# hugolatendresse/FlexFlow

Measured on AMD Instinct MI355X. Metric: decoded tokens/s (LLaMA-7B SpecInfer, LLaMA-68M SSM), higher is better.
Workload: dtype f16; 1 GPU; llama7b_specinfer_llama68m_b8_p128_d128; model=LLaMA-7B (random init), ssm=LLaMA-68M (random init), global_batch=8, prefill=128, decode=128, seq_len=256, parallelism=tp1, layers=32

## Files before the change

### flexflow_amd/csrc/api.cpp

```cpp
#include <rccl/rccl.h>
#include <stdio.h>
#include <stdlib.h>
#include <string.h>

#include <chrono>
#include <cmath>
#include <condition_variable>
#include <memory>
#include <mutex>
#include <string>
#include <vector>

#include <algorithm>
#include <climits>

#include "ffmi_internal.h"
#include "collective.h"

static thread_local std::string g_last_error;

void ffmi_set_last_error(const char *msg, const char *file, int line) {
  char buf[512];
  snprintf(buf, sizeof(buf), "%s (%s:%d)", msg, file, line);
  g_last_error = buf;
// ... 221 lines not shown
}

extern "C" ffmi_status ffmi_attn_create(const ffmi_attn_cfg *cfg, ffmi_attn **out) {
  FFMI_CHECK(cfg && out, FFMI_ERR_INVALID);
  FFMI_CHECK(cfg->head_dim == 64 || cfg->head_dim == 128 ||
                 (cfg->head_dim == 32 && cfg->mode == FFMI_ATTN_INC),
             FFMI_ERR_UNSUPPORTED);
  FFMI_CHECK(cfg->num_heads > 0 && cfg->max_requests > 0 && cfg->max_seq_len > 0 &&
                 cfg->max_tokens > 0,
             FFMI_ERR_INVALID);
  FFMI_CHECK(cfg->out_layout == 0 || cfg->out_layout == 1, FFMI_ERR_INVALID);
  FFMI_CHECK(cfg->out_layout == 0 || (cfg->num_heads * cfg->head_dim) % 32 == 0,
             FFMI_ERR_UNSUPPORTED);
  ffmi_attn *h = new ffmi_attn();
  h->cfg = *cfg;
  h->slots = (cfg->max_seq_len + cfg->max_tree_tokens + 31) & ~31;
  const size_t Hl = (size_t)cfg->num_heads * cfg->head_dim;
  const size_t kv = (size_t)cfg->max_requests * cfg->num_heads * h->slots * cfg->head_dim;
  const bool f32 = cfg->full_precision != 0;
  if (f32 && (cfg->out_layout != 0 || (size_t)(cfg->head_dim + 256 + h->slots) * 4 > 64 * 1024)) {
    delete h;
    ffmi_set_last_error("full precision: out_layout 0 and (head_dim + 256 + slots) * 4 <= 64 KiB",
                        __FILE__, __LINE__);
    return FFMI_ERR_UNSUPPORTED;
  }
  const size_t es = f32 ? 4 : 2, stage_halves = f32 ? 1 : 2;
  bool ok = hipMalloc((void **)&h->kc, kv * es) == hipSuccess &&
            hipMalloc((void **)&h->vc, kv * es) == hipSuccess &&
            hipMalloc((void **)&h->qbuf, (size_t)cfg->max_tokens * Hl * es) == hipSuccess;
  if (ok && cfg->mode == FFMI_ATTN_TREE)
    ok = hipMalloc((void **)&h->stage, (size_t)cfg->max_tokens * 2 * Hl * es * stage_halves) ==
         hipSuccess;
  std::vector<float> tab;
  rope_table(tab, h->slots, cfg->head_dim, cfg);
  if (ok) ok = hipMalloc((void **)&h->rope, tab.size() * sizeof(float)) == hipSuccess;
  if (!ok) {
    ffmi_attn_destroy(h);
    ffmi_set_last_error("attention cache alloc", __FILE__, __LINE__);
    return FFMI_ERR_OOM;
  }
  FFMI_HIP(hipMemset(h->kc, 0, kv * es));
  FFMI_HIP(hipMemset(h->vc, 0, kv * es));
  if (h->stage)
    FFMI_HIP(hipMemset(h->stage, 0, (size_t)cfg->max_tokens * 2 * Hl * es * stage_halves));
  FFMI_HIP(hipMemcpy(h->rope, tab.data(), tab.size() * sizeof(float), hipMemcpyHostToDevice));
  *out = h;
  return FFMI_OK;
}

namespace ffmi {
ffmi_status attn_rope_fault(ffmi_attn *h, int from_pos) {
  FFMI_CHECK(h, FFMI_ERR_INVALID);
  std::vector<float> tab;
  rope_table(tab, h->slots + 1, h->cfg.head_dim, &h->cfg);
  const size_t row = (size_t)h->cfg.head_dim;
  if (from_pos >= 0)
    for (int p = from_pos; p < h->slots; ++p)
      memcpy(&tab[(size_t)p * row], &tab[(size_t)(p + 1) * row], row * sizeof(float));
  FFMI_HIP(hipMemcpy(h->rope, tab.data(), (size_t)h->slots * row * sizeof(float),
                     hipMemcpyHostToDevice));
  return FFMI_OK;
}
}

extern "C" void ffmi_attn_destroy(ffmi_attn *h) {
  if (!h) return;
  (void)hipFree(h->kc);
  (void)hipFree(h->vc);
  (void)hipFree(h->qbuf);
  (void)hipFree(h->stage);
  (void)hipFree(h->rope);
  delete h;
}

extern "C" ffmi_status ffmi_attn_kv_ptrs(ffmi_attn *h, void **k, void **v, int *slots) {
  FFMI_CHECK(h, FFMI_ERR_INVALID);
  if (k) *k = h->kc;
  if (v) *v = h->vc;
  if (slots) *slots = h->slots;
  return FFMI_OK;
}

namespace ffmi {
ffmi_status attn_forward(ffmi_attn *h, const ffmi_batch_dev *b, const void *qkv, Partials qkvp,
                         void *out, ffmi_stream stream, int parity, OprojArgs *opa) {
  FFMI_CHECK(h && b && (qkv || qkvp.S > 0) && out, FFMI_ERR_INVALID);
  if (opa) opa->done = false;
  FFMI_CHECK(b->num_tokens <= h->cfg.max_tokens, FFMI_ERR_INVALID);
  const bool tree = h->cfg.mode == FFMI_ATTN_TREE;
  const hipStream_t s = (hipStream_t)stream;
  const int heads = h->cfg.num_heads, d = h->cfg.head_dim;
  if (h->cfg.full_precision) {
    FFMI_CHECK(qkv && qkvp.S == 0 && !(opa && opa->wo), FFMI_ERR_INVALID);
    FFMI_HIP(ffmi::launch_kv_update_f32(b->dev, b->num_tokens, tree ? b->num_commits : 0,
                                        (const float *)qkv, h->rope, h->slots, (float *)h->qbuf,
                                        (float *)h->kc, (float *)h->vc,
                                        tree ? (float *)h->stage : nullptr, heads, d, h->slots, s));
    FFMI_HIP(ffmi::launch_attention_f32(b->dev, b->num_tokens, (const float *)h->qbuf,
                                        (const float *)h->kc, (const float *)h->vc, (float *)out,
                                        heads, d, h->slots, h->cfg.qk_scale, s));
    return FFMI_OK;
  }
  uint16_t *stage_wr = nullptr, *stage_rd = nullptr;
  int C = 0;
  if (tree) {
    if (parity < 0) parity = h->parity, h->parity ^= 1;
    const size_t half = (size_t)h->cfg.max_tokens * 2 * heads * d;
    stage_wr = h->stage + (parity ? half : 0);
    stage_rd = h->stage + (parity ? 0 : half);
    C = b->num_commits;
  }
  const bool no_fuse = getenv("FFMI_ATTN_NO_FUSE") != nullptr;
  const bool fused = b->one_item_per_req && b->lds_tail && !no_fuse;
  if (C > 0 && b->commit_overlap) {
    FFMI_HIP(ffmi::launch_commit(b->dev, C, stage_rd, h->kc, h->vc, heads, d, h->slots, s));
    C = 0;
  }
  if (!fused) {
    FFMI_HIP(ffmi::launch_kv_update(b->dev, b->num_tokens, b->num_work, C,
                                    (const uint16_t *)qkv, qkvp, h->qbuf, h->kc, h->vc, stage_wr,
                                    stage_rd, h->rope, heads, d, h->slots, h->slots, s));
    C = 0;
  }
  const bool oproj = opa && opa->wo && opa->slab && fused && d == 64 && b->max_q <= 16 &&
                     opa->N % 16 == 0 && opa->N <= 1024 && b->num_tokens <= opa->max_T;
  FFMI_HIP(ffmi::launch_attention(b->dev, b->num_work, b->max_q, h->qbuf, h->kc, h->vc,
                                  (uint16_t *)out, heads, d, h->slots, h->cfg.qk_scale, s,
                                  h->cfg.out_layout == 1, fused, b->num_tokens, C,
                                  (const uint16_t *)qkv, qkvp, stage_wr, stage_rd, h->rope,
                                  h->slots, oproj ? opa : nullptr));
  if (oproj) opa->done = true;
  return FFMI_OK;
}
}

static ffmi_status attn_run(ffmi_attn *h, const ffmi_batch_dev *b, const void *qkv, void *out,
                            ffmi_stream stream, int mode) {
  FFMI_CHECK(h && qkv, FFMI_ERR_INVALID);
  FFMI_CHECK(h->cfg.mode == mode, FFMI_ERR_INVALID);
  return ffmi::attn_forward(h, b, qkv, ffmi::Partials(), out, stream);
}

extern "C" ffmi_status ffmi_attn_inc(ffmi_attn *h, const ffmi_batch_dev *b, const void *qkv,
                                     void *out, ffmi_stream stream) {
  return attn_run(h, b, qkv, out, stream, FFMI_ATTN_INC);
}
extern "C" ffmi_status ffmi_attn_spec(ffmi_attn *h, const ffmi_batch_dev *b, const void *qkv,
                                      void *out, ffmi_stream stream) {
  return attn_run(h, b, qkv, out, stream, FFMI_ATTN_SPEC);
}
extern "C" ffmi_status ffmi_attn_tree(ffmi_attn *h, const ffmi_batch_dev *b, const void *qkv,
                                      void *out, ffmi_stream stream) {
  FFMI_CHECK(h && h->stage, FFMI_ERR_INVALID);
  return attn_run(h, b, qkv, out, stream, FFMI_ATTN_TREE);
}

extern "C" size_t ffmi_linear_packed_bytes(int out_dim, int in_dim) {
  const size_t nt = (size_t)(out_dim + 15) / 16, kt = (size_t)(in_dim + 31) / 32;
  return nt * kt * 512 * 2;
}

extern "C" ffmi_status ffmi_linear_pack_weight(const void *W, int out_dim, int in_dim,
                                               void *W_packed, ffmi_stream stream) {
  FFMI_CHECK(W && W_packed && out_dim > 0 && in_dim > 0, FFMI_ERR_INVALID);
  FFMI_HIP(ffmi::launch_pack_weight((const uint16_t *)W, in_dim, 0, 0, out_dim, in_dim,
                                    (uint16_t *)W_packed, 1, 0, (out_dim + 15) / 16,
                                    (hipStream_t)stream));
  return FFMI_OK;
}

extern "C" ffmi_status ffmi_linear_pack_gate_up(const void *Wg, const void *Wu, int out_dim,
                                                int in_dim, void *W_packed, ffmi_stream stream) {
  FFMI_CHECK(Wg && Wu && W_packed && out_dim > 0 && in_dim > 0, FFMI_ERR_INVALID);
  const int pitch = 2 * ((out_dim + 15) / 16);
  FFMI_HIP(ffmi::launch_pack_weight((const uint16_t *)Wg, in_dim, 0, 0, out_dim, in_dim,
                                    (uint16_t *)W_packed, 2, 0, pitch, (hipStream_t)stream));
  FFMI_HIP(ffmi::launch_pack_weight((const uint16_t *)Wu, in_dim, 0, 0, out_dim, in_dim,
                                    (uint16_t *)W_packed, 2, 1, pitch, (hipStream_t)stream));
  return FFMI_OK;
}

extern "C" size_t ffmi_linear_workspace_bytes(int T, int out_dim, int in_dim, int epilogue) {
  if (T <= 0 || out_dim <= 0 || in_dim <= 0) return 0;
  return ffmi::gemm_workspace_bytes(T, out_dim, in_dim, epilogue);
}

extern "C" ffmi_status ffmi_linear_ws(const void *X, const void *W_packed, void *Y, int T,
                                      int out_dim, int in_dim, int epilogue, void *workspace,
                                      size_t workspace_bytes, ffmi_stream stream) {
  FFMI_CHECK(X && W_packed && Y && T >= 0 && out_dim > 0, FFMI_ERR_INVALID);
  FFMI_CHECK(in_dim > 0 && in_dim % 32 == 0, FFMI_ERR_UNSUPPORTED);
  const int epi = epilogue & ~(FFMI_X_PACKED | FFMI_W_STREAM);
  const int epi_base = epi & ~FFMI_Y_PACKED;
  FFMI_CHECK(epi_base == FFMI_EPI_NONE || epi_base == FFMI_EPI_SILU_MUL, FFMI_ERR_INVALID);
  FFMI_CHECK(!(epilogue & FFMI_Y_PACKED) || out_dim % 32 == 0, FFMI_ERR_UNSUPPORTED);
  FFMI_HIP(ffmi::launch_gemm((const uint16_t *)X, (const uint16_t *)W_packed, (uint16_t *)Y,
                             (float *)workspace, workspace_bytes, T, out_dim, in_dim, epilogue,
                             (hipStream_t)stream));
  return FFMI_OK;
}

static std::mutex g_ws_mu;
static void *g_ws = nullptr;
static size_t g_ws_bytes = 0;

extern "C" ffmi_status ffmi_linear(const void *X, const void *W_packed, void *Y, int T,
                                   int out_dim, int in_dim, int epilogue, ffmi_stream stream) {
  FFMI_CHECK(X && W_packed && Y && T >= 0 && out_dim > 0, FFMI_ERR_INVALID);
  FFMI_CHECK(in_dim > 0 && in_dim % 32 == 0, FFMI_ERR_UNSUPPORTED);
  const size_t need = ffmi_linear_workspace_bytes(T, out_dim, in_dim, epilogue);
  void *ws = nullptr;
  {
    std::lock_guard<std::mutex> lk(g_ws_mu);
    if (need > g_ws_bytes) {
      if (g_ws) {
        FFMI_HIP(hipDeviceSynchronize());
        (void)hipFree(g_ws);
        g_ws = nullptr;
        g_ws_bytes = 0;
      }
      if (hipMalloc(&g_ws, need) != hipSuccess) return FFMI_ERR_OOM;
      g_ws_bytes = need;
    }
    ws = g_ws;
  }
  return ffmi_linear_ws(X, W_packed, Y, T, out_dim, in_dim, epilogue, ws, g_ws_bytes, stream);
}

extern "C" ffmi_status ffmi_rmsnorm(const void *x, const void *w, void *out, int T, int H,
                                    float eps, ffmi_stream stream) {
  FFMI_CHECK(x && w && out && H % 8 == 0 && H <= 16384, FFMI_ERR_INVALID);
  FFMI_HIP(ffmi::launch_rmsnorm((const uint16_t *)x, nullptr, (const uint16_t *)w, nullptr,
                                (uint16_t *)out, T, H, eps, (hipStream_t)stream));
  return FFMI_OK;
}

extern "C" ffmi_status ffmi_residual_rmsnorm(const void *x1, const void *x2, const void *w,
                                             void *residual_out, void *out, int T, int H,
                                             float eps, ffmi_stream stream) {
  FFMI_CHECK(x1 && x2 && w && residual_out && out && H % 8 == 0 && H <= 16384, FFMI_ERR_INVALID);
  FFMI_HIP(ffmi::launch_rmsnorm((const uint16_t *)x1, (const uint16_t *)x2, (const uint16_t *)w,
                                (uint16_t *)residual_out, (uint16_t *)out, T, H, eps,
                                (hipStream_t)stream));
  return FFMI_OK;
}

extern "C" ffmi_status ffmi_rmsnorm_ex(const void *x1, const void *x2, const void *w,
                                       void *residual_out, void *out, int T, int H, float eps,
                                       int flags, ffmi_stream stream) {
  FFMI_CHECK(x1 && w && out && T >= 0 && H > 0 && H % 8 == 0, FFMI_ERR_INVALID);
  FFMI_CHECK(!x2 || residual_out, FFMI_ERR_INVALID);
  FFMI_CHECK((flags & ~FFMI_Y_PACKED) == 0, FFMI_ERR_INVALID);
  const bool packed = (flags & FFMI_Y_PACKED) != 0;
  FFMI_CHECK(!packed || H % 32 == 0, FFMI_ERR_UNSUPPORTED);
  FFMI_HIP(ffmi::launch_rmsnorm((const uint16_t *)x1, (const uint16_t *)x2, (const uint16_t *)w,
                                (uint16_t *)residual_out, (uint16_t *)out, T, H, eps,
                                (hipStream_t)stream, packed));
  return FFMI_OK;
}

extern "C" ffmi_status ffmi_embedding(const ffmi_batch_dev *b, const void *table, void *out,
                                      int H, ffmi_stream stream) {
  FFMI_CHECK(b && table && out && H % 8 == 0, FFMI_ERR_INVALID);
  FFMI_HIP(ffmi::launch_embedding(b->dev, b->num_tokens, (const uint16_t *)table,
                                  (uint16_t *)out, H, (hipStream_t)stream));
  return FFMI_OK;
}

extern "C" ffmi_status ffmi_silu_mul(const void *a, const void *b, void *out, size_t n,
                                     ffmi_stream stream) {
  FFMI_CHECK(a && b && out, FFMI_ERR_INVALID);
  FFMI_HIP(ffmi::launch_silu_mul((const uint16_t *)a, (const uint16_t *)b, (uint16_t *)out, n,
                                 (hipStream_t)stream));
  return FFMI_OK;
}

extern "C" ffmi_status ffmi_argmax(const void *logits, int T, int V, int32_t *ids, float *probs,
                                   ffmi_stream stream) {
  FFMI_CHECK(logits && ids && V > 0, FFMI_ERR_INVALID);
  FFMI_HIP(ffmi::launch_argmax((const uint16_t *)logits, T, V, 1, ids, probs,
                               (hipStream_t)stream));
  return FFMI_OK;
}

extern "C" ffmi_status ffmi_arg_topk(const void *logits, int T, int V, int k, int32_t *ids,
                                     float *probs, ffmi_stream stream) {
  FFMI_CHECK(logits && ids && V > 0 && k >= 1 && k <= 4 && k <= V, FFMI_ERR_INVALID);
  FFMI_HIP(ffmi::launch_argmax((const uint16_t *)logits, T, V, k, ids, probs,
                               (hipStream_t)stream));
  return FFMI_OK;
}

extern "C" size_t ffmi_arg_topk_workspace_bytes(int T) { return ffmi::argmax_workspace_bytes(T); }

extern "C" ffmi_status ffmi_arg_topk_ws(const void *logits, int T, int V, int k, int32_t *ids,
                                        float *probs, void *workspace, size_t workspace_bytes,
                                        ffmi_stream stream) {
  FFMI_CHECK(logits && ids && V > 0 && k >= 1 && k <= 4 && k <= V, FFMI_ERR_INVALID);
  FFMI_HIP(ffmi::launch_argmax((const uint16_t *)logits, T, V, k, ids, probs,
                               (hipStream_t)stream, workspace, workspace_bytes));
  return FFMI_OK;
}

extern "C" ffmi_status ffmi_debug_fused_residual_linear(const void *X, const void *W_packed,
                                                        void *residual, float *ss_out, int T,
                                                        int out_dim, int in_dim,
                                                        ffmi_stream stream) {
  FFMI_CHECK(X && W_packed && residual && ss_out && T > 0 && T <= 32, FFMI_ERR_INVALID);
  ffmi::FuseArgs fz;
  fz.kind = 1;
  fz.res_in = (const uint16_t *)residual;
  fz.ss_out = ss_out;
  FFMI_HIP(ffmi::launch_gemm((const uint16_t *)X, (const uint16_t *)W_packed, (uint16_t *)residual,
                             nullptr, 0, T, out_dim, in_dim, FFMI_EPI_NONE, (hipStream_t)stream,
                             nullptr, 0, &fz));
  return FFMI_OK;
}

extern "C" ffmi_status ffmi_debug_fused_norm_linear(const void *residual, const float *ss_in,
                                                    const void *norm_w, float eps,
                                                    const void *W_packed, void *Y, int T,
                                                    int out_dim, int in_dim, int epilogue,
                                                    ffmi_stream stream) {
  FFMI_CHECK(residual && ss_in && norm_w && W_packed && Y && T > 0 && T <= 32 &&
                 (epilogue == FFMI_EPI_NONE || epilogue == FFMI_EPI_SILU_MUL),
             FFMI_ERR_INVALID);
  ffmi::FuseArgs fz;
  fz.kind = 2;
  fz.ss_in = ss_in;
  fz.nss = in_dim / 16;
  fz.wnorm = (const uint16_t *)norm_w;
  fz.eps = eps;
  FFMI_HIP(ffmi::launch_gemm((const uint16_t *)residual, (const uint16_t *)W_packed, (uint16_t *)Y,
                             nullptr, 0, T, out_dim, in_dim, epilogue, (hipStream_t)stream,
                             nullptr, 0, &fz));
  return FFMI_OK;
}

extern "C" ffmi_status ffmi_fill_weight(void *dst_f16, size_t n, const char *name, uint64_t seed,
                                        int kind, ffmi_stream stream) {
  FFMI_CHECK(dst_f16 && name, FFMI_ERR_INVALID);
  FFMI_HIP(ffmi::launch_fill_weight((uint16_t *)dst_f16, n, ffmi::weight_key(name, seed), kind,
                                    (hipStream_t)stream));
  return FFMI_OK;
}

struct LocalGroup {
  int n = 0;
  ffmi_status sum_status = FFMI_OK;
  std::mutex mu;
  std::condition_variable cv;
  int arrived = 0;
  long gen = 0;
  bool broken = false;
  std::vector<const void *> bufs;
  void *tmp = nullptr;
  size_t tmp_bytes = 0;
  ~LocalGroup() {
    if (tmp) (void)hipFree(tmp);
  }
  bool barrier() {
    std::unique_lock<std::mutex> lk(mu);
    if (broken) return false;
    const long g = gen;
    if (++arrived == n) {
      arrived = 0;
      ++gen;
      cv.notify_all();
      return true;
    }
    if (!cv.wait_for(lk, std::chrono::seconds(120), [&] { return gen != g || broken; }) || broken) {
      broken = true;
      cv.notify_all();
      return false;
    }
    return true;
  }
};

struct PeerState {
  size_t cap = 0;
  char *own = nullptr;
  char *base[ffmi::kMaxPeers] = {};
  std::vector<void *> opened;
  int *err_h = nullptr, *err_d = nullptr;
  bool attached = false;
  uint64_t timeout_ticks = 1000000000ull;
  size_t two_shot_min = 256 << 10;
  ~PeerState() {
    for (void *p : opened) (void)hipIpcCloseMemHandle(p);
    if (own) (void)hipFree(own);
    if (err_h) (void)hipHostFree(err_h);
  }
};

struct ffmi_comm {
  ncclComm_t comm = nullptr;
  int nranks = 1, rank = 0;
  std::shared_ptr<LocalGroup> local;
  std::unique_ptr<PeerState> peer;
  float *xg = nullptr;
  size_t xg_cap = 0;
  hipStream_t xg_stream = nullptr;
};

extern "C" ffmi_status ffmi_comm_create_local(int nranks, ffmi_comm **out) {
  FFMI_CHECK(out && nranks >= 1 && nranks <= 8, FFMI_ERR_INVALID);
  auto g = std::make_shared<LocalGroup>();
  g->n = nranks;
  g->bufs.assign(nranks, nullptr);
  for (int r = 0; r < nranks; ++r) {
    out[r] = new ffmi_comm();
    out[r]->nranks = nranks;
    out[r]->rank = r;
    out[r]->local = g;
  }
  return FFMI_OK;
}

static ffmi_status local_allreduce(ffmi_comm *c, const void *in, void *out, size_t count,
                                   int dtype, hipStream_t s) {
  LocalGroup &g = *c->local;
  const size_t bytes = count * (dtype == FFMI_F16 ? 2 : 4);
  g.bufs[c->rank] = in;
  FFMI_HIP(hipStreamSynchronize(s));
  FFMI_CHECK(g.barrier(), FFMI_ERR_NCCL);
  ffmi_status st = FFMI_OK;
  if (c->rank == 0) {
    if (g.tmp_bytes < bytes) {
      if (g.tmp) (void)hipFree(g.tmp);
      g.tmp = nullptr;
      g.tmp_bytes = 0;
      if (hipMalloc(&g.tmp, bytes) == hipSuccess) g.tmp_bytes = bytes;
    }
    if (!g.tmp) {
      st = FFMI_ERR_OOM;
    } else if (ffmi::launch_group_sum(g.bufs.data(), g.n, g.tmp, count, dtype, s) != hipSuccess ||
               hipStreamSynchronize(s) != hipSuccess) {
      st = FFMI_ERR_HIP;
    }
  }
  if (c->rank == 0) g.sum_status = st;
  if (!g.barrier() || g.sum_status != FFMI_OK) {
    std::lock_guard<std::mutex> lk(g.mu);
    g.broken = true;
    g.cv.notify_all();
    return g.sum_status != FFMI_OK ? g.sum_status : FFMI_ERR_NCCL;
  }
  FFMI_HIP(hipMemcpyAsync(out, g.tmp, bytes, hipMemcpyDeviceToDevice, s));
  FFMI_HIP(hipStreamSynchronize(s));
  FFMI_CHECK(g.barrier(), FFMI_ERR_NCCL);
  return FFMI_OK;
}

extern "C" ffmi_status ffmi_comm_unique_id(void *id_out) {
  FFMI_CHECK(id_out, FFMI_ERR_INVALID);
  static_assert(sizeof(ncclUniqueId) == FFMI_UNIQUE_ID_BYTES, "unique id size");
  ncclUniqueId id;
  if (ncclGetUniqueId(&id) != ncclSuccess) return FFMI_ERR_NCCL;
  memcpy(id_out, &id, sizeof(id));
  return FFMI_OK;
}

extern "C" ffmi_status ffmi_comm_create(const void *id, int nranks, int rank, ffmi_comm **out) {
  FFMI_CHECK(id && out && nranks >= 1 && rank >= 0 && rank < nranks, FFMI_ERR_INVALID);
  ffmi_comm *c = new ffmi_comm();
  c->nranks = nranks;
  c->rank = rank;
  ncclUniqueId uid;
  memcpy(&uid, id, sizeof(uid));
  ncclResult_t r = ncclCommInitRank(&c->comm, nranks, uid, rank);
  if (r != ncclSuccess) {
    ffmi_set_last_error(ncclGetErrorString(r), __FILE__, __LINE__);
    delete c;
    return FFMI_ERR_NCCL;
  }
  *out = c;
  return FFMI_OK;
}

extern "C" void ffmi_comm_destroy(ffmi_comm *c) {
  if (!c) return;
  if (c->xg_stream) (void)hipStreamSynchronize(c->xg_stream);
  if (c->xg) (void)hipFree(c->xg);
  if (c->xg_stream) (void)hipStreamDestroy(c->xg_stream);
  if (c->comm) ncclCommDestroy(c->comm);
  delete c;
}

extern "C" ffmi_status ffmi_comm_allgather(ffmi_comm *c, const void *mine, size_t bytes,
                                           void *all) {
  FFMI_CHECK(c && (mine || !bytes) && (all || !bytes), FFMI_ERR_INVALID);
  const int n = c->nranks;
  if (n == 1) {
    if (bytes) memcpy(all, mine, bytes);
    return FFMI_OK;
  }
  const size_t words = (bytes + 1) / 2;
  const size_t count = words * n;
  if (c->xg_cap < count) {
    if (c->xg) FFMI_HIP(hipFree(c->xg));
    c->xg = nullptr;
    c->xg_cap = 0;
    FFMI_HIP(hipMalloc((void **)&c->xg, count * sizeof(float)));
    c->xg_cap = count;
  }
  if (!c->xg_stream) FFMI_HIP(hipStreamCreateWithFlags(&c->xg_stream, hipStreamNonBlocking));
  std::vector<float> h(count, 0.0f);
  std::vector<uint16_t> w(words, 0);
  memcpy(w.data(), mine, bytes);
  for (size_t i = 0; i < words; ++i) h[(size_t)c->rank * words + i] = (float)w[i];
  FFMI_HIP(hipMemcpyAsync(c->xg, h.data(), count * sizeof(float), hipMemcpyHostToDevice,
                          c->xg_stream));
  ffmi_status st = ffmi_allreduce(c, c->xg, c->xg, count, FFMI_F32, (ffmi_stream)c->xg_stream);
  if (st != FFMI_OK) return st;
  FFMI_HIP(hipMemcpyAsync(h.data(), c->xg, count * sizeof(float), hipMemcpyDeviceToHost,
                          c->xg_stream));
  FFMI_HIP(hipStreamSynchronize(c->xg_stream));
  if (c->peer && c->peer->attached) {
    st = ffmi_comm_peer_status(c);
    if (st != FFMI_OK) return st;
  }
  std::vector<uint16_t> out(words);
  for (int r = 0; r < n; ++r) {
    for (size_t i = 0; i < words; ++i) {
      const float v = h[(size_t)r * words + i];
      if (!(v >= 0.0f && v <= 65535.0f && v == (float)(uint16_t)v)) return FFMI_ERR_NCCL;
      out[i] = (uint16_t)v;
    }
    memcpy(static_cast<char *>(all) + (size_t)r * bytes, out.data(), bytes);
  }
  return FFMI_OK;
}

extern "C" ffmi_status ffmi_comm_create_peer(int nranks, int rank, ffmi_comm **out) {
  FFMI_CHECK(out && nranks >= 1 && nranks <= ffmi::kMaxPeers && rank >= 0 && rank < nranks,
             FFMI_ERR_INVALID);
  ffmi_comm *c = new ffmi_comm();
  c->nranks = nranks;
  c->rank = rank;
  *out = c;
  return FFMI_OK;
}

extern "C" ffmi_status ffmi_comm_peer_export(ffmi_comm *c, size_t max_bytes, void *handle_out) {
  FFMI_CHECK(c && handle_out && max_bytes > 0 && !c->local, FFMI_ERR_INVALID);
  FFMI_CHECK(c->nranks <= ffmi::kMaxPeers && !c->peer, FFMI_ERR_INVALID);
  static_assert(sizeof(hipIpcMemHandle_t) == FFMI_PEER_HANDLE_BYTES, "IPC handle size");
  auto p = std::make_unique<PeerState>();
  p->cap = (max_bytes + 255) & ~(size_t)255;
  if (const char *e = getenv("FFMI_PEER_TIMEOUT_S")) p->timeout_ticks = (uint64_t)(atof(e) * 1e8);
  if (c->nranks <= 2) p->two_shot_min = (size_t)-1;
  if (const char *e = getenv("FFMI_PEER_TWO_SHOT_MIN")) p->two_shot_min = (size_t)atoll(e);
  const size_t bytes = ffmi::peer_buffer_bytes(p->cap);
  const char *uc = getenv("FFMI_PEER_UNCACHED");
  if (uc && !atoi(uc)) FFMI_HIP(hipMalloc((void **)&p->own, bytes));
  else FFMI_HIP(hipExtMallocWithFlags((void **)&p->own, bytes, hipDeviceMallocUncached));
  FFMI_HIP(hipMemset(p->own, 0, ffmi::kDataOff));
  FFMI_HIP(hipDeviceSynchronize());
  FFMI_HIP(hipHostMalloc((void **)&p->err_h, sizeof(int), hipHostMallocMapped));
  *p->err_h = 0;
  FFMI_HIP(hipHostGetDevicePointer((void **)&p->err_d, p->err_h, 0));
  hipIpcMemHandle_t h;
  FFMI_HIP(hipIpcGetMemHandle(&h, p->own));
  memcpy(handle_out, &h, sizeof(h));
  c->peer = std::move(p);
  return FFMI_OK;
}

static ffmi_status peer_run(ffmi_comm *c, const void *in, void *out, size_t rows, size_t cols,
                            size_t ld, size_t col0, int dtype, hipStream_t s,
                            const ffmi::Partials *slabs = nullptr, int rs_row0 = -1,
                            int rs_row1 = -1, const ffmi::PeerNormArgs *norm = nullptr,
                            int two_shot = -1) {
  PeerState &p = *c->peer;
  const size_t esz = dtype == FFMI_F16 ? 2 : 4;
  const size_t bytes = rows * cols * esz;
  FFMI_CHECK(bytes <= p.cap, FFMI_ERR_INVALID);
  FFMI_CHECK((cols * esz) % 16 == 0 && ((size_t)in & 15) == 0 && ((size_t)out & 15) == 0 &&
                 (ld * esz) % 16 == 0 && (col0 * esz) % 16 == 0,
             FFMI_ERR_UNSUPPORTED);
  if (slabs && slabs->S > 0)
    FFMI_CHECK(dtype == FFMI_F16 && slabs->S <= 8 && slabs->NP >= (int)cols && slabs->NP % 4 == 0 &&
                   ((size_t)slabs->p & 15) == 0,
               FFMI_ERR_UNSUPPORTED);
  ffmi::PeerArgs a;
  for (int r = 0; r < ffmi::kMaxPeers; ++r) a.base[r] = p.base[r];
  a.nranks = c->nranks;
  a.rank = c->rank;
  a.cap = p.cap;
  a.in = in;
  a.out = out;
  a.nvec = bytes / 16;
  a.vec_elems = 16 / esz;
  a.cols = cols;
  a.ld = ld;
  a.col0 = col0;
  a.esz = esz;
  a.err = p.err_d;
  a.timeout_ticks = p.timeout_ticks;
  if (slabs && slabs->S > 0) a.slabs = slabs->p, a.S = slabs->S, a.NP = slabs->NP, a.rows = rows;
  const bool ts = two_shot >= 0 ? two_shot != 0 : bytes >= p.two_shot_min;
  if (norm) FFMI_HIP(ffmi::launch_peer_allreduce_norm(a, *norm, ts, s));
  else FFMI_HIP(ffmi::launch_peer_allreduce(a, ts, s, rs_row0, rs_row1));
  return FFMI_OK;
}
// ... 233 lines not shown
```

### flexflow_amd/csrc/ffmi_internal.h

```cpp
#pragma once
#include <hip/hip_runtime.h>
#include <hip/hip_fp16.h>
#include <stdint.h>

#include "../../include/ffmi.h"
#include "kernels/gemm_plan.h"

#define FFMI_HIP(expr)                                   \
  do {                                                   \
    hipError_t e_ = (expr);                              \
    if (e_ != hipSuccess) {                              \
      ffmi_set_last_error(hipGetErrorString(e_), __FILE__, __LINE__); \
      (void)hipGetLastError();  \
      return FFMI_ERR_HIP;                               \
    }                                                    \
  } while (0)

#define FFMI_CHECK(cond, code)                                         \
  do {                                                                 \
    if (!(cond)) {                                                     \
      ffmi_set_last_error(#cond, __FILE__, __LINE__);                  \
      return (code);                                                   \
    }                                                                  \
  } while (0)

void ffmi_set_last_error(const char *msg, const char *file, int line);

namespace ffmi {

typedef _Float16 h8 __attribute__((ext_vector_type(8)));
typedef _Float16 h4 __attribute__((ext_vector_type(4)));
typedef float f4 __attribute__((ext_vector_type(4)));

template <bool NT>
__device__ __forceinline__ h8 ld_weight(const uint16_t *p) {
  if constexpr (NT) return __builtin_nontemporal_load(reinterpret_cast<const h8 *>(p));
  else return *reinterpret_cast<const h8 *>(p);
}

__host__ __device__ __forceinline__ size_t act_packed_off(int m, int n, int K) {
  return ((((size_t)(m >> 4) * (size_t)(K >> 5) + (size_t)(n >> 5)) * 64 + (m & 15) +
           16 * ((n >> 3) & 3))
          << 3) +
         (n & 7);
}

struct BatchHeader {
  int32_t num_tokens, num_work, num_commits, num_mask_reqs;
  int32_t off_tokens, off_work, off_commits, off_masks;
};
constexpr int kBlobWorkOffset = 32;
static_assert(sizeof(BatchHeader) == kBlobWorkOffset, "work array follows the header");

constexpr int kTailSlots = 128;
constexpr int kItemCommits = 8;

struct WorkDev {
  ffmi_attn_work w;
  int32_t clean;
  int32_t tail0;
  int32_t ncommit;
  int32_t told;
  int16_t rope_pos[FFMI_ATTN_QTILE];
  int16_t cm_src[kItemCommits], cm_depth[kItemCommits];
};
static_assert(sizeof(WorkDev) % 16 == 0, "16-B aligned work items");

struct BatchView {
  const BatchHeader *hdr;
  const ffmi_token_info *tokens;
  const WorkDev *work;
  const ffmi_commit_info *commits;
  const uint64_t *masks;
};

__device__ __forceinline__ BatchView batch_view(const char *blob) {
  BatchView v;
  v.hdr = reinterpret_cast<const BatchHeader *>(blob);
  v.work = reinterpret_cast<const WorkDev *>(blob + kBlobWorkOffset);
  v.tokens = reinterpret_cast<const ffmi_token_info *>(blob + v.hdr->off_tokens);
  v.commits = reinterpret_cast<const ffmi_commit_info *>(blob + v.hdr->off_commits);
  v.masks = reinterpret_cast<const uint64_t *>(blob + v.hdr->off_masks);
  return v;
}

struct Partials {
  const float *p = nullptr;
  int S = 0, NP = 0;
};
__device__ __forceinline__ float partials_value(const float *p, int S, int NP, int T, int t,
                                                int n) {
  const size_t slab = (size_t)T * NP;
  const float *q = p + (size_t)t * NP + n;
  float acc = q[0];
  for (int s = 1; s < S; ++s) acc += q[s * slab];
  return __half2float(__float2half_rn(acc));
}

__host__ __device__ __forceinline__ void mid_xcd_map(int bx, int by, int nblk, int S, int &cb,
                                                     int &ks) {
  cb = bx, ks = by;
  if (S <= 1) return;
  const int l = bx + nblk * by, P = nblk * S;
  const int x = l & 7, q = P >> 3, r = P & 7;
  const int L = (x < r ? x * (q + 1) : r * (q + 1) + (x - r) * q) + (l >> 3);
  ks = L / nblk, cb = L - ks * nblk;
}

hipError_t launch_fill_weight(uint16_t *dst, size_t n, uint64_t key, int kind, hipStream_t s,
                              int cols = 0, uint64_t pa = 1, uint64_t pb = 0, float scale = 1.0f);
hipError_t launch_fill_weight_f32(float *dst, size_t n, uint64_t key, int kind, hipStream_t s,
                                  int cols = 0, uint64_t pa = 1, uint64_t pb = 0,
                                  float scale = 1.0f);
float weight_amp(int kind);
hipError_t launch_gemm_f32(const float *X, const float *W, float *Y, int T, int N, int K,
                           hipStream_t s);
hipError_t launch_rmsnorm_f32(const float *x1, const float *x2, const float *w, float *res_out,
                              float *out, int T, int H, float eps, hipStream_t s,
                              const char *gather = nullptr);
hipError_t launch_silu_mul_f32(const float *A, const float *B, float *out, int T, int F,
                               size_t lda, size_t ldb, hipStream_t s);
hipError_t launch_kv_update_f32(const char *blob, int T, int C, const float *qkv, const float *rope,
                                int max_rope_pos, float *qbuf, float *kc, float *vc,
                                float *stage, int heads, int d, int slots, hipStream_t s);
hipError_t launch_attention_f32(const char *blob, int T, const float *qbuf, const float *kc,
                                const float *vc, float *out, int heads, int d, int slots,
                                float scale, hipStream_t s);
hipError_t launch_softmax_topk_f32(const float *logits, int T, int V, int k, int32_t *ids,
                                   float *probs, hipStream_t s);
ffmi_status attn_rope_fault(ffmi_attn *h, int from_pos);
bool weights_kmajor();
inline size_t w_tile_stride(int KT) { return weights_kmajor() ? 512 : (size_t)KT * 512; }
inline size_t w_k_stride(int pitch) { return weights_kmajor() ? (size_t)pitch * 512 : 512; }
hipError_t launch_pack_weight(const uint16_t *src, int ld, int row0, int col0,
                              int N, int K, uint16_t *dst, int tile_step,
                              int tile_offset, int pitch, hipStream_t s);
struct FuseArgs {
  int kind = 0;
  const uint16_t *res_in = nullptr;
  float *ss_out = nullptr;
  const float *ss_in = nullptr;
  int nss = 0;
  const uint16_t *wnorm = nullptr;
  float eps = 0.f;
};
hipError_t launch_gemm(const uint16_t *X, const uint16_t *Wp, uint16_t *Y, float *ws,
                       size_t ws_bytes, int T, int N, int K, int epilogue, hipStream_t s,
                       Partials *defer = nullptr, int wpitch = 0, const FuseArgs *fuse = nullptr);
hipError_t launch_partials_reduce(const Partials &p, uint16_t *Y, int T, int N, hipStream_t s);
long attn_debug_stamps(long long *dst, long max_waves);
hipError_t launch_marker(int i, hipStream_t s);
void attn_stamp_gate(bool open);
long debug_markers(long long *dst, long n);
long gemm_debug_stamps(long long *dst, long max_waves);
size_t packed_act_bytes(int T, int K);
hipError_t launch_pack_act(const uint16_t *X, uint16_t *Xp, int T, int K, hipStream_t s);
hipError_t launch_rmsnorm(const uint16_t *x1, const uint16_t *x2, const uint16_t *w,
                          uint16_t *res_out, uint16_t *out, int T, int H, float eps,
                          hipStream_t s, bool out_packed = false, Partials x2p = {}, const char *gather = nullptr,
                          char *blob_dst = nullptr, size_t blob_bytes = 0,
                          const int32_t *gather_prev = nullptr);
void set_norm_fault(bool on);
hipError_t launch_embedding(const char *blob, int T, const uint16_t *table,
                            uint16_t *out, int H, hipStream_t s);
hipError_t launch_silu_mul(const uint16_t *a, const uint16_t *b, uint16_t *out,
                           size_t n, hipStream_t s);
hipError_t launch_argmax(const uint16_t *logits, int T, int V, int k, int32_t *ids,
                         float *probs, hipStream_t s, void *ws = nullptr, size_t ws_bytes = 0,
                         int32_t *ids2 = nullptr);
size_t argmax_workspace_bytes(int T);
hipError_t launch_vshard(const uint16_t *logits, int T, int Vl, int P, int rank, int k,
                         int phase, float *xch, int W, int32_t *ids, float *probs,
                         hipStream_t s);
hipError_t launch_group_sum(const void *const *bufs, int n, void *out, size_t count, int dtype,
                            hipStream_t s);

hipError_t launch_kv_update(const char *blob, int T, int W, int C, const uint16_t *qkv,
                            Partials qkvp, uint16_t *qbuf, uint16_t *kc, uint16_t *vc,
                            uint16_t *stage_wr, const uint16_t *stage_rd, const float *rope,
                            int heads, int d, int slots, int max_rope_pos, hipStream_t s);
hipError_t launch_commit(const char *blob, int C, const uint16_t *stage,
                         uint16_t *kc, uint16_t *vc, int heads, int d, int slots,
                         hipStream_t s);
struct OprojArgs {
  const uint16_t *wo = nullptr;
  float *slab = nullptr;
  int N = 0, max_T = 0;
  size_t wts = 0, wks = 0;
  bool done = false;
};
hipError_t launch_attention(const char *blob, int W, int max_q, uint16_t *qbuf, uint16_t *kc,
                            uint16_t *vc, uint16_t *out, int heads, int d, int slots, float scale,
                            hipStream_t s, bool out_packed, bool fused, int T, int C,
                            const uint16_t *qkv, Partials qkvp, uint16_t *stage_wr,
                            const uint16_t *stage_rd, const float *rope, int max_rope_pos,
                            const OprojArgs *opa = nullptr);

uint64_t weight_key(const char *name, uint64_t seed);

}

struct ffmi_batch_dev {
  char *host = nullptr;
  char *dev = nullptr;
  size_t cap = 0;
  int max_tokens = 0, max_requests = 0;
  int num_tokens = 0, num_work = 0, num_commits = 0, num_mask_reqs = 0;
  bool commit_overlap = false;
  bool one_item_per_req = false;
  bool lds_tail = false;
  int max_q = 0;
  hipEvent_t uploaded = nullptr;
};

namespace ffmi {
ffmi_status batch_stage(ffmi_batch_dev *b, const ffmi_batch_desc *d, size_t *bytes);
ffmi_status batch_copy(ffmi_batch_dev *b, size_t bytes, hipStream_t s, bool record_event);
bool comm_has_peer(const ffmi_comm *c, size_t bytes);
int comm_size(const ffmi_comm *c);
int comm_rank(const ffmi_comm *c);
bool comm_peer_attached(const ffmi_comm *c);
bool comm_has_fallback(const ffmi_comm *c);
bool comm_is_rccl(const ffmi_comm *c);
ffmi_status comm_allreduce_cols(ffmi_comm *c, const void *in, void *out, int rows, int cols,
                                int ld, int col0, int dtype, hipStream_t s,
                                const Partials *slabs = nullptr);
bool comm_two_shot(const ffmi_comm *c, size_t bytes);
ffmi_status comm_reduce_rows(ffmi_comm *c, const void *in, void *out, int rows, int cols, int ld,
                             int col0, int row0, int row1, hipStream_t s,
                             const Partials *slabs = nullptr);
ffmi_status comm_allreduce_norm(ffmi_comm *c, const void *in, int T, int H, int col0,
                                const uint16_t *prev, uint16_t *res, const uint16_t *w, float eps,
                                uint16_t *h, bool packed, bool two_shot, hipStream_t s,
                                const Partials *slabs = nullptr);
ffmi_status comm_status(ffmi_comm *c);
ffmi_status attn_forward(ffmi_attn *h, const ffmi_batch_dev *b, const void *qkv, Partials qkvp,
                         void *out, ffmi_stream stream, int parity = -1,
                         OprojArgs *opa = nullptr);
}
```

### flexflow_amd/csrc/kernels/norm.hip

```cpp
#include <algorithm>

#include "../ffmi_internal.h"
#include "expf_ref.h"

namespace ffmi {

__device__ __forceinline__ float h2f_(uint16_t v) { return __half2float(__ushort_as_half(v)); }
__device__ __forceinline__ uint16_t f2h_(float v) { return __half_as_ushort(__float2half_rn(v)); }

template <int NW, typename T>
__device__ __forceinline__ T block_sum(T v, T *scratch) {
#pragma unroll
  for (int o = 32; o > 0; o >>= 1) v += __shfl_xor(v, o);
  const int wave = threadIdx.x >> 6;
  if ((threadIdx.x & 63) == 0) scratch[wave] = v;
  __syncthreads();
  T r = scratch[0];
#pragma unroll
  for (int q = 1; q < NW; ++q) r += scratch[q];
  return r;
}

template <int NT, int MAXC, int MAXS, int SRC>
__global__ __launch_bounds__(NT) void rmsnorm_kernel(
    const uint16_t *__restrict__ x1, const uint16_t *__restrict__ x2,
    const uint16_t *__restrict__ w, uint16_t *__restrict__ res_out,
    uint16_t *__restrict__ out, int H, float eps, int out_packed,
    const float *__restrict__ x2p, int pS, int pNP, const char *__restrict__ gather,
    uint4 *__restrict__ blob_dst, int blob_n16, const int32_t *__restrict__ gprev) {
  __shared__ double scratch[NT / 64];
  const int row = blockIdx.x;
  const int T = gridDim.x;
  const int nchunk = H >> 3;
  constexpr bool FAULT = SRC >= 4;
  constexpr int S = FAULT ? SRC - 3 : SRC;
  int gid = 0;
  if (S == 3) {
    gid = batch_view(gather).tokens[row].token_id;
    if (gid < 0) gid = gprev[-1 - gid];
  }
  const uint16_t *a = S == 3 ? x1 + (size_t)gid * H : x1 + (size_t)row * H;
  if (S == 3 && blob_dst) {
    const uint4 *src = reinterpret_cast<const uint4 *>(gather);
    for (int i = row * NT + threadIdx.x; i < blob_n16; i += T * NT) blob_dst[i] = src[i];
  }
  uint4 v[MAXC], wv[MAXC];
  uint4 xb[MAXC];
  f4 slo[MAXS], shi[MAXS];
  auto fold = [&]() {
    f4 lo = slo[0], hi = shi[0];
#pragma unroll
    for (int sl = 1; sl < MAXS; ++sl)
      if (sl < pS) lo += slo[sl], hi += shi[sl];
    uint16_t hb[8];
#pragma unroll
    for (int q4 = 0; q4 < 4; ++q4) {
      hb[q4] = f2h_(lo[q4]);
      hb[q4 + 4] = f2h_(hi[q4]);
    }
    return *reinterpret_cast<uint4 *>(hb);
  };
#pragma unroll
  for (int c = 0; c < MAXC; ++c) {
    const int ch = min((int)threadIdx.x + c * NT, nchunk - 1);
    if (S == 2) {
      const float *q = x2p + (size_t)row * pNP + ch * 8;
#pragma unroll
      for (int sl = 0; sl < MAXS; ++sl) {
        const float *qs = q + (size_t)min(sl, pS - 1) * T * pNP;
        slo[sl] = *reinterpret_cast<const f4 *>(qs);
        shi[sl] = *reinterpret_cast<const f4 *>(qs + 4);
      }
    }
    if (S == 1) xb[c] = *reinterpret_cast<const uint4 *>(x2 + (size_t)row * H + ch * 8);
    v[c] = *reinterpret_cast<const uint4 *>(a + ch * 8);
    wv[c] = *reinterpret_cast<const uint4 *>(w + ch * 8);
    if (S == 2 && MAXC > 1) xb[c] = fold();
  }
  if (S == 2 && MAXC == 1) xb[0] = fold();
  double ss = 0.0;
#pragma unroll
  for (int c = 0; c < MAXC; ++c) {
    const int ch = threadIdx.x + c * NT;
    if (ch < nchunk) {
      uint4 xa = v[c];
      if (S == 1 || S == 2) {
        const uint4 xbb = xb[c];
        const __half2 *pa = reinterpret_cast<const __half2 *>(&xa);
        const __half2 *pb = reinterpret_cast<const __half2 *>(&xbb);
        if (FAULT) {
          const uint16_t *ea = reinterpret_cast<const uint16_t *>(&xa);
          const uint16_t *eb = reinterpret_cast<const uint16_t *>(&xbb);
#pragma unroll
          for (int q = 0; q < 8; ++q) {
            const float f = h2f_(ea[q]) + h2f_(eb[q]);
            ss += (double)f * (double)f;
          }
        }
        __half2 r[4];
#pragma unroll
        for (int q = 0; q < 4; ++q) r[q] = __hadd2(pa[q], pb[q]);
        xa = *reinterpret_cast<uint4 *>(r);
        *reinterpret_cast<uint4 *>(res_out + (size_t)row * H + ch * 8) = xa;
      } else if (S == 3) {
        *reinterpret_cast<uint4 *>(res_out + (size_t)row * H + ch * 8) = xa;
      }
      v[c] = xa;
      const uint16_t *e = reinterpret_cast<const uint16_t *>(&xa);
      if (!FAULT) {
#pragma unroll
        for (int q = 0; q < 8; ++q) {
          const float f = h2f_(e[q]);
          ss += (double)f * (double)f;
        }
      }
    }
  }
  const float sum = (float)block_sum<NT / 64>(ss, scratch);
  const float rms_f = __fdiv_rn(1.0f, sqrtf(__fadd_rn(__fdiv_rn(sum, (float)H), eps)));
  const float rms = h2f_(f2h_(rms_f));
#pragma unroll
  for (int c = 0; c < MAXC; ++c) {
    const int ch = threadIdx.x + c * NT;
    if (ch < nchunk) {
      const uint16_t *e = reinterpret_cast<const uint16_t *>(&v[c]);
      const uint16_t *we = reinterpret_cast<const uint16_t *>(&wv[c]);
      uint16_t o8[8];
#pragma unroll
      for (int q = 0; q < 8; ++q) {
        float y = h2f_(f2h_(__fmul_rn(h2f_(e[q]), rms)));
        o8[q] = f2h_(__fmul_rn(y, h2f_(we[q])));
      }
      uint16_t *dst = out_packed ? out + act_packed_off(row, ch * 8, H) : out + (size_t)row * H + ch * 8;
      *reinterpret_cast<uint4 *>(dst) = *reinterpret_cast<uint4 *>(o8);
    }
  }
}

static bool g_norm_fault = false;
void set_norm_fault(bool on) { g_norm_fault = on; }

hipError_t launch_rmsnorm(const uint16_t *x1, const uint16_t *x2, const uint16_t *w,
                          uint16_t *res_out, uint16_t *out, int T, int H, float eps,
                          hipStream_t s, bool out_packed, Partials x2p, const char *gather,
                          char *blob_dst, size_t blob_bytes, const int32_t *gather_prev) {
  if (gather && (x2 || x2p.S > 0 || !res_out)) return hipErrorInvalidValue;
  if (blob_dst && (!gather || blob_bytes > (size_t)1 << 30 || (uintptr_t)gather % 16 ||
                   (uintptr_t)blob_dst % 16))
    return hipErrorInvalidValue;
  const int blob_n16 = blob_dst ? (int)((blob_bytes + 15) / 16) : 0;
  if (T <= 0) return hipSuccess;
  if (out_packed && H % 32) return hipErrorInvalidValue;
  const int op = out_packed ? 1 : 0;
  const int nchunk = H / 8;
  if (nchunk > 4096) return hipErrorInvalidValue;
  const float *pp = x2p.S > 0 ? x2p.p : nullptr;
  if (pp && (x2p.S > 16 || (x2p.S > 8 && nchunk > 128))) return hipErrorInvalidValue;
  if ((x2 || pp) && !res_out) return hipErrorInvalidValue;
  if (pp && nchunk > 1024) return hipErrorInvalidValue;
  const int src = gather ? 3 : pp ? 2 : x2 ? 1 : 0;
  const int ms = !pp || x2p.S <= 1 ? 1 : x2p.S <= 2 ? 2 : x2p.S <= 4 ? 4 : x2p.S <= 8 ? 8
               : x2p.S <= 12 ? 12 : 16;
#define FFMI_RMS3(NT, MC, MS, SR)                                                              \
  hipLaunchKernelGGL((rmsnorm_kernel<NT, MC, MS, SR>), dim3(T), dim3(NT), 0, s, x1, x2, w,    \
                     res_out, out, H, eps, op, pp, x2p.S, x2p.NP, gather,               \
                     reinterpret_cast<uint4 *>(blob_dst), blob_n16, gather_prev)
#define FFMI_RMS(NT, MC)                                   \
  do {                                                     \
    if (src == 0) FFMI_RMS3(NT, MC, 1, 0);                 \
    else if (src == 1) FFMI_RMS3(NT, MC, 1, 1);            \
    else if (src == 3) FFMI_RMS3(NT, MC, 1, 3);            \
    else if (ms == 1) FFMI_RMS3(NT, MC, 1, 2);             \
    else if (ms == 2) FFMI_RMS3(NT, MC, 2, 2);             \
    else if (ms == 4) FFMI_RMS3(NT, MC, 4, 2);             \
    else FFMI_RMS3(NT, MC, 8, 2);                          \
  } while (0)
#define FFMI_RMS_NOSLAB(NT, MC)                            \
  do {                                                     \
    if (src == 0) FFMI_RMS3(NT, MC, 1, 0);                 \
    else if (src == 1) FFMI_RMS3(NT, MC, 1, 1);            \
    else FFMI_RMS3(NT, MC, 1, 3);                          \
  } while (0)
  if (g_norm_fault && (src == 1 || src == 2)) {
#define FFMI_RMSF(NT)                                      \
  do {                                                     \
    if (src == 1) FFMI_RMS3(NT, 1, 1, 4);                  \
    else if (ms == 1) FFMI_RMS3(NT, 1, 1, 5);              \
    else if (ms == 2) FFMI_RMS3(NT, 1, 2, 5);              \
    else if (ms == 4) FFMI_RMS3(NT, 1, 4, 5);              \
    else if (ms == 8) FFMI_RMS3(NT, 1, 8, 5);              \
    else return hipErrorInvalidValue;                      \
  } while (0)
    if (nchunk <= 128) FFMI_RMSF(128);
    else if (nchunk <= 256) FFMI_RMSF(256);
    else if (nchunk <= 512) FFMI_RMSF(512);
    else if (nchunk <= 1024) FFMI_RMSF(1024);
    else return hipErrorInvalidValue;
#undef FFMI_RMSF
    return hipGetLastError();
  }
  if (nchunk <= 128 && ms == 12) FFMI_RMS3(128, 1, 12, 2);
  else if (nchunk <= 128 && ms == 16) FFMI_RMS3(128, 1, 16, 2);
  else if (nchunk <= 128) FFMI_RMS(128, 1);
  else if (nchunk <= 256) FFMI_RMS(256, 1);
  else if (nchunk <= 512) FFMI_RMS(512, 1);
  else if (nchunk <= 1024) FFMI_RMS(1024, 1);
  else if (nchunk <= 2048) FFMI_RMS_NOSLAB(1024, 2);
  else FFMI_RMS_NOSLAB(1024, 4);
#undef FFMI_RMS_NOSLAB
#undef FFMI_RMS
#undef FFMI_RMS3
  return hipGetLastError();
}

__global__ void embedding_kernel(const char *__restrict__ blob,
                                 const uint16_t *__restrict__ table,
                                 uint16_t *__restrict__ out, int H) {
  const BatchView bv = batch_view(blob);
  const int t = blockIdx.x;
  const int tok = bv.tokens[t].token_id;
  const uint4 *src = reinterpret_cast<const uint4 *>(table + (size_t)tok * H);
  uint4 *dst = reinterpret_cast<uint4 *>(out + (size_t)t * H);
  for (int c = threadIdx.x; c < H / 8; c += blockDim.x) dst[c] = src[c];
}

hipError_t launch_embedding(const char *blob, int T, const uint16_t *table, uint16_t *out,
                            int H, hipStream_t s) {
  if (T <= 0) return hipSuccess;
  if (H % 8 != 0) return hipErrorInvalidValue;
  hipLaunchKernelGGL(embedding_kernel, dim3(T), dim3(256), 0, s, blob, table, out, H);
  return hipGetLastError();
}

__global__ void silu_mul_kernel(const uint16_t *__restrict__ a, const uint16_t *__restrict__ b,
                                uint16_t *__restrict__ out, size_t n) {
  for (size_t i = blockIdx.x * (size_t)blockDim.x + threadIdx.x; i < n;
       i += (size_t)gridDim.x * blockDim.x) {
    const float g = h2f_(a[i]);
    const float sg = __fdiv_rn(1.0f, __fadd_rn(1.0f, expf(-g)));
    const float t = h2f_(f2h_(__fmul_rn(g, h2f_(f2h_(sg)))));
    out[i] = f2h_(__fmul_rn(t, h2f_(b[i])));
  }
}

hipError_t launch_silu_mul(const uint16_t *a, const uint16_t *b, uint16_t *out, size_t n,
                           hipStream_t s) {
  if (n == 0) return hipSuccess;
  size_t blocks = (n + 255) / 256;
  if (blocks > 16384) blocks = 16384;
  hipLaunchKernelGGL(silu_mul_kernel, dim3((unsigned)blocks), dim3(256), 0, s, a, b, out, n);
  return hipGetLastError();
}

extern "C" __device__ float __ockl_wfred_max_f32(float);
extern "C" __device__ double __ockl_wfred_add_f64(double);
extern "C" __device__ unsigned long long __ockl_wfred_max_u64(unsigned long long);

template <int TPB, int NV, int G>
__global__ __launch_bounds__(TPB) void softmax_topk_reg_kernel(
    const uint16_t *__restrict__ logits, int V, int k, int32_t *__restrict__ ids,
    float *__restrict__ probs, double *__restrict__ part, unsigned *__restrict__ cnt,
    int32_t *__restrict__ ids2) {
  constexpr int NW = TPB / 64;
  constexpr int kCand = 128;
  static_assert(G == 1 || ((NV * 8) % G == 0 && NV * 8 / G >= 2),
                "split: whole dwords of a thread's elements per workgroup");
  constexpr int E = NV * 8 / G;
  __shared__ double sh[NW + 2];
  __shared__ unsigned long long cand[kCand];
  __shared__ unsigned ncand;
  __shared__ int last_arrival;
  float *fsh = reinterpret_cast<float *>(sh);
  unsigned long long *ksh = reinterpret_cast<unsigned long long *>(sh);
  const int row = G == 1 ? blockIdx.x : blockIdx.y, chunk = G == 1 ? 0 : blockIdx.x;
  const int tid = threadIdx.x, lane = tid & 63, wv = tid >> 6;
  const int nvec = V >> 3;
  const uint4 *x = reinterpret_cast<const uint4 *>(logits + (size_t)row * V);
  constexpr int EPV = E < 8 ? 8 / E : 1;
  const int vrot = G == 1 ? 0 : (E >= 8 ? chunk * (E / 8) : chunk / EPV);
  const int eo = E >= 8 ? 0 : (chunk % EPV) * E;
  auto gv = [&](int v) -> int { return (G == 1 ? v : (v + vrot) % NV) * TPB + tid; };
  uint4 r[NV];
#pragma unroll
  for (int v = 0; v < NV; ++v) {
    const int i = gv(v);
    r[v] = i < nvec ? x[i] : make_uint4(0xfc00fc00u, 0xfc00fc00u, 0xfc00fc00u, 0xfc00fc00u);
  }
  if (tid == 0) ncand = 0;
  auto elem = [&](int v, int e) -> float {
    const uint32_t w = (&r[v].x)[e >> 1];
    return h2f_((uint16_t)((e & 1) ? (w >> 16) : (w & 0xffffu)));
  };
  float mx = -INFINITY;
#pragma unroll
  for (int v = 0; v < NV; ++v)
#pragma unroll
    for (int e = 0; e < 8; ++e) mx = fmaxf(mx, elem(v, e));
  mx = __ockl_wfred_max_f32(mx);
  if (lane == 0) fsh[wv] = mx;
  __syncthreads();
  float wmax[NW];
#pragma unroll
  for (int q = 0; q < NW; ++q) wmax[q] = fsh[q];
  __syncthreads();
  float M = wmax[0];
#pragma unroll
  for (int q = 1; q < NW; ++q) M = fmaxf(M, wmax[q]);
  float L = -INFINITY;
  {
    float top[4] = {-INFINITY, -INFINITY, -INFINITY, -INFINITY};
#pragma unroll
    for (int q = 0; q < NW; ++q) {
      float v = wmax[q];
#pragma unroll
      for (int j = 0; j < 4; ++j) {
        const float hi = fmaxf(top[j], v), lo = fminf(top[j], v);
        top[j] = hi, v = lo;
      }
    }
#pragma unroll
    for (int j = 0; j < 4; ++j)
      if (j == k - 1) L = top[j];
  }
  double se = 0.0;
  if constexpr (E >= 8) {
#pragma unroll
    for (int v = 0; v < E / 8; ++v)
      if (gv(v) < nvec)
#pragma unroll
        for (int e = 0; e < 8; ++e) se += (double)expf_ref(elem(v, e) - M);
  } else {
    const int d0 = eo >> 1;
    auto dw = [&](int d) -> uint32_t {
      const uint32_t lo = (d & 1) ? r[0].y : r[0].x, hi = (d & 1) ? r[0].w : r[0].z;
      return (d & 2) ? hi : lo;
    };
    if (gv(0) < nvec)
#pragma unroll
      for (int q = 0; q < E / 2; ++q) {
        const uint32_t w = dw(d0 + q);
        se += (double)expf_ref(h2f_((uint16_t)(w & 0xffffu)) - M);
        se += (double)expf_ref(h2f_((uint16_t)(w >> 16)) - M);
      }
  }
  se = __ockl_wfred_add_f64(se);
  if (lane == 0) sh[wv] = se;
  __syncthreads();
  double sd = 0.0;
#pragma unroll
  for (int q = 0; q < NW; ++q) sd += sh[q];
  if constexpr (G > 1) {
    if (wv == 0) {
      unsigned before = 0;
      if (lane == 0) {
        __hip_atomic_store(&part[(size_t)row * G + chunk], sd, __ATOMIC_RELAXED,
                           __HIP_MEMORY_SCOPE_AGENT);
        asm volatile("s_waitcnt vmcnt(0)" ::: "memory");
        before = __hip_atomic_fetch_add(&cnt[row], 1u, __ATOMIC_RELAXED, __HIP_MEMORY_SCOPE_AGENT);
      }
      const int last = __shfl(before, 0) == (unsigned)(G - 1);
      if (last) {
        double pq = 0.0;
        if (lane < G)
          pq = __hip_atomic_load(&part[(size_t)row * G + lane], __ATOMIC_RELAXED,
                                 __HIP_MEMORY_SCOPE_AGENT);
        double tot = 0.0;
#pragma unroll
        for (int q = 0; q < G; ++q) tot += __shfl(pq, q);
        if (lane == 0) {
          __hip_atomic_store(&cnt[row], 0u, __ATOMIC_RELAXED, __HIP_MEMORY_SCOPE_AGENT);
          sh[NW] = tot;
        }
      }
      if (lane == 0) last_arrival = last;
    }
    __syncthreads();
    if (!last_arrival) return;
    sd = sh[NW];
  }
  const float S = (float)sd;
  float thr = -3.402823466e38f;
  {
    const uint16_t pL = f2h_(__fdiv_rn(expf_ref(L - M), S));
    if (pL > 1) {
      const float lo = 0.5f * (h2f_(pL) + h2f_((uint16_t)(pL - 1)));
      thr = M + logf(lo * S) - 0.0009765625f * fmaxf(1.0f, fabsf(M));
    }
  }
  auto key_of = [&](float xv, unsigned i) -> unsigned long long {
    const uint16_t p = f2h_(__fdiv_rn(expf_ref(xv - M), S));
    return ((unsigned long long)(p + 1u) << 32) | (unsigned long long)(0xffffffffu - i);
  };
  auto emit = [&](int rd, unsigned long long b) {
    ids[(size_t)row * k + rd] = (int)(0xffffffffu - (unsigned)(b & 0xffffffffu));
    if (ids2) ids2[(size_t)row * k + rd] = (int)(0xffffffffu - (unsigned)(b & 0xffffffffu));
    if (probs) probs[(size_t)row * k + rd] = h2f_((uint16_t)((b >> 32) - 1u));
  };
#pragma unroll
  for (int v = 0; v < NV; ++v)
#pragma unroll
    for (int e = 0; e < 8; ++e) {
      const float xv = elem(v, e);
      const unsigned i = (unsigned)(gv(v) * 8 + e);
      if (xv >= thr && (int)i < V) {
        const unsigned slot = atomicAdd(&ncand, 1u);
        if (slot < (unsigned)kCand) cand[slot] = key_of(xv, i);
      }
    }
  __syncthreads();
  const unsigned n = ncand;
  if (n <= (unsigned)kCand) {
    if (wv == 0) {
      unsigned long long a = (unsigned)lane < n ? cand[lane] : 0ull;
      unsigned long long b = (unsigned)(lane + 64) < n ? cand[lane + 64] : 0ull;
      for (int rd = 0; rd < k; ++rd) {
        const unsigned long long best = __ockl_wfred_max_u64(a > b ? a : b);
        if (lane == 0) emit(rd, best);
        if (a == best) a = 0ull;
        if (b == best) b = 0ull;
      }
    }
    return;
  }
  for (int rd = 0; rd < k; ++rd) {
    unsigned long long best = 0;
#pragma unroll
    for (int v = 0; v < NV; ++v)
#pragma unroll
      for (int e = 0; e < 8; ++e) {
        const float xv = elem(v, e);
        const unsigned i = (unsigned)(gv(v) * 8 + e);
        if (xv >= thr && (int)i < V) {
          const unsigned long long key = key_of(xv, i);
          best = key > best ? key : best;
        }
      }
    best = __ockl_wfred_max_u64(best);
    if (lane == 0) ksh[wv] = best;
    __syncthreads();
    unsigned long long b = ksh[0];
#pragma unroll
    for (int q = 1; q < NW; ++q) b = ksh[q] > b ? ksh[q] : b;
    __syncthreads();
    const unsigned idx = 0xffffffffu - (unsigned)(b & 0xffffffffu);
    if (tid == 0) emit(rd, b);
    if (rd + 1 < k && (idx >> 3) % TPB == (unsigned)tid) {
#pragma unroll
      for (int v = 0; v < NV; ++v)
        if ((unsigned)gv(v) == (idx >> 3)) {
#pragma unroll
          for (int e = 0; e < 8; ++e) {
            uint32_t &w = (&r[v].x)[e >> 1];
            const uint32_t m = (e & 1) ? 0xffff0000u : 0x0000ffffu;
            if ((unsigned)e == (idx & 7)) w = (w & ~m) | (0xfc00fc00u & m);
          }
        }
    }
  }
}

template <int TPB>
__global__ __launch_bounds__(TPB) void softmax_topk_kernel(
    const uint16_t *__restrict__ logits, int V, int k, int32_t *__restrict__ ids,
    float *__restrict__ probs, int32_t *__restrict__ ids2) {
  constexpr int NW = TPB / 64;
  constexpr int kCand = 128;
  __shared__ double sh[NW + 2];
  __shared__ unsigned long long cand[kCand];
  __shared__ unsigned ncand;
  float *fsh = reinterpret_cast<float *>(sh);
  unsigned long long *ksh = reinterpret_cast<unsigned long long *>(sh);
  const int row = blockIdx.x, tid = threadIdx.x, lane = tid & 63, wv = tid >> 6;
  const uint16_t *x = logits + (size_t)row * V;
  if (tid == 0) ncand = 0;
  float mx = -INFINITY;
  for (int i = tid; i < V; i += TPB) mx = fmaxf(mx, h2f_(x[i]));
  mx = __ockl_wfred_max_f32(mx);
  if (lane == 0) fsh[wv] = mx;
  __syncthreads();
  float wmax[NW];
#pragma unroll
  for (int q = 0; q < NW; ++q) wmax[q] = fsh[q];
  __syncthreads();
  float M = wmax[0];
#pragma unroll
  for (int q = 1; q < NW; ++q) M = fmaxf(M, wmax[q]);
  float L = -INFINITY;
  {
    float top[4] = {-INFINITY, -INFINITY, -INFINITY, -INFINITY};
#pragma unroll
    for (int q = 0; q < NW; ++q) {
      float v = wmax[q];
#pragma unroll
      for (int j = 0; j < 4; ++j) {
        const float hi = fmaxf(top[j], v), lo = fminf(top[j], v);
        top[j] = hi, v = lo;
      }
    }
#pragma unroll
    for (int j = 0; j < 4; ++j)
      if (j == k - 1) L = top[j];
  }
  double se = 0.0;
  for (int i = tid; i < V; i += TPB) se += (double)expf_ref(h2f_(x[i]) - M);
  se = __ockl_wfred_add_f64(se);
  if (lane == 0) sh[wv] = se;
  __syncthreads();
  double sd = 0.0;
#pragma unroll
  for (int q = 0; q < NW; ++q) sd += sh[q];
  const float S = (float)sd;
  float thr = -3.402823466e38f;
  {
    const uint16_t pL = f2h_(__fdiv_rn(expf_ref(L - M), S));
    if (pL > 1) {
      const float lo = 0.5f * (h2f_(pL) + h2f_((uint16_t)(pL - 1)));
      thr = M + logf(lo * S) - 0.0009765625f * fmaxf(1.0f, fabsf(M));
    }
  }
  auto key_of = [&](float xv, unsigned i) -> unsigned long long {
    const uint16_t p = f2h_(__fdiv_rn(expf_ref(xv - M), S));
    return ((unsigned long long)(p + 1u) << 32) | (unsigned long long)(0xffffffffu - i);
  };
  auto emit = [&](int rd, unsigned long long b) {
    ids[(size_t)row * k + rd] = (int)(0xffffffffu - (unsigned)(b & 0xffffffffu));
    if (ids2) ids2[(size_t)row * k + rd] = (int)(0xffffffffu - (unsigned)(b & 0xffffffffu));
    if (probs) probs[(size_t)row * k + rd] = h2f_((uint16_t)((b >> 32) - 1u));
  };
  for (int i = tid; i < V; i += TPB) {
    const float xv = h2f_(x[i]);
    if (xv >= thr) {
      const unsigned slot = atomicAdd(&ncand, 1u);
      if (slot < (unsigned)kCand) cand[slot] = key_of(xv, (unsigned)i);
    }
  }
  __syncthreads();
  const unsigned n = ncand;
  if (n <= (unsigned)kCand) {
    if (wv == 0) {
      unsigned long long a = (unsigned)lane < n ? cand[lane] : 0ull;
      unsigned long long b = (unsigned)(lane + 64) < n ? cand[lane + 64] : 0ull;
      for (int rd = 0; rd < k; ++rd) {
        const unsigned long long best = __ockl_wfred_max_u64(a > b ? a : b);
        if (lane == 0) emit(rd, best);
        if (a == best) a = 0ull;
        if (b == best) b = 0ull;
      }
    }
    return;
  }
  int chosen[4] = {-1, -1, -1, -1};
  for (int rd = 0; rd < k; ++rd) {
    unsigned long long best = 0;
    for (int i = tid; i < V; i += TPB) {
      const float xv = h2f_(x[i]);
      if (xv < thr) continue;
      bool taken = false;
#pragma unroll
      for (int q = 0; q < 4; ++q) taken |= (q < rd && chosen[q] == i);
      if (taken) continue;
      const unsigned long long key = key_of(xv, (unsigned)i);
      best = key > best ? key : best;
    }
    best = __ockl_wfred_max_u64(best);
    if (lane == 0) ksh[wv] = best;
    __syncthreads();
    unsigned long long b = ksh[0];
#pragma unroll
    for (int q = 1; q < NW; ++q) b = ksh[q] > b ? ksh[q] : b;
    __syncthreads();
    chosen[rd] = (int)(0xffffffffu - (unsigned)(b & 0xffffffffu));
    if (tid == 0) emit(rd, b);
  }
}

constexpr int kSplitRows = 256;
constexpr size_t kSplitPartOff = kSplitRows * 4;
size_t argmax_workspace_bytes(int T) {
  return T <= 0 ? 0 : kSplitPartOff + (size_t)std::min(T, kSplitRows) * 16 * 8;
}

hipError_t launch_argmax(const uint16_t *logits, int T, int V, int k, int32_t *ids,
                         float *probs, hipStream_t s, void *ws, size_t ws_bytes, int32_t *ids2) {
  if (T <= 0) return hipSuccess;
  if (k < 1 || k > 4) return hipErrorInvalidValue;
  static const int split_env = getenv("FFMI_TOPK_SPLIT") ? atoi(getenv("FFMI_TOPK_SPLIT")) : -1;
  static const bool split2 = getenv("FFMI_TOPK_SPLIT2") && atoi(getenv("FFMI_TOPK_SPLIT2"));
  int G = T <= 32 ? 8 : T <= 64 ? 4 : T <= 128 ? 2 : (T <= kSplitRows && split2) ? 2 : 1;
  if (split_env >= 0) G = split_env;
  if (!ws || ws_bytes < argmax_workspace_bytes(T) || T > kSplitRows) G = 1;
  unsigned *cnt = reinterpret_cast<unsigned *>(ws);
  double *part = ws ? reinterpret_cast<double *>(static_cast<char *>(ws) + kSplitPartOff) : nullptr;
  static const int tpb = [] {
    const char *e = getenv("FFMI_TOPK_TPB");
    const int v = e ? atoi(e) : 1024;
    return v == 256 || v == 512 ? v : 1024;
  }();
  const int nv = (V / 8 + tpb - 1) / tpb;
  if (V % 8 == 0 && ((uintptr_t)logits & 15) == 0 && nv * tpb <= 4096) {
#define FFMI_SMR(TPB, NV)                                                                  \
  hipLaunchKernelGGL((softmax_topk_reg_kernel<TPB, NV, 1>), dim3(T), dim3(TPB), 0, s, logits, V, \
                     k, ids, probs, nullptr, nullptr, ids2)
#define FFMI_SMG(NV, GG)                                                                     \
  hipLaunchKernelGGL((softmax_topk_reg_kernel<1024, NV, GG>), dim3(GG, T), dim3(1024), 0, s, \
                     logits, V, k, ids, probs, part, cnt, ids2)
    const int gmax = 4 * std::max(1, nv);
    while (G > 1 && (G > gmax || (G & (G - 1)))) G >>= 1;
    if (tpb == 1024 && G > 1) {
      if (nv <= 1) {
        if (G >= 4) FFMI_SMG(1, 4);
        else FFMI_SMG(1, 2);
      } else if (nv <= 2) {
        if (G >= 8) FFMI_SMG(2, 8);
        else if (G == 4) FFMI_SMG(2, 4);
        else FFMI_SMG(2, 2);
      } else {
        if (G >= 16) FFMI_SMG(4, 16);
        else if (G == 8) FFMI_SMG(4, 8);
        else if (G == 4) FFMI_SMG(4, 4);
        else FFMI_SMG(4, 2);
      }
    } else if (tpb == 256) {
      if (nv <= 4) FFMI_SMR(256, 4);
      else if (nv <= 8) FFMI_SMR(256, 8);
      else FFMI_SMR(256, 16);
    } else if (tpb == 512) {
      if (nv <= 2) FFMI_SMR(512, 2);
      else if (nv <= 4) FFMI_SMR(512, 4);
      else FFMI_SMR(512, 8);
    } else {
      if (nv <= 1) FFMI_SMR(1024, 1);
      else if (nv <= 2) FFMI_SMR(1024, 2);
      else FFMI_SMR(1024, 4);
    }
#undef FFMI_SMR
#undef FFMI_SMG
  } else {
    hipLaunchKernelGGL(softmax_topk_kernel<1024>, dim3(T), dim3(1024), 0, s, logits, V, k, ids, probs,
                       ids2);
  }
  return hipGetLastError();
}

template <int TPB>
__global__ __launch_bounds__(TPB) void vshard_kernel(const uint16_t *__restrict__ logits, int T,
                                                      int Vl, int P, int rank, int k, int phase,
                                                      float *__restrict__ xch, int W,
                                                      int32_t *__restrict__ ids,
                                                      float *__restrict__ probs) {
  constexpr int NW = TPB / 64;
  constexpr int kCand = 128;
  __shared__ double dsh[NW];
  __shared__ float fsh[NW];
  __shared__ unsigned long long ksh[NW];
  __shared__ unsigned long long cand[kCand];
  __shared__ unsigned ncand;
  const int t = blockIdx.x, tid = threadIdx.x, lane = tid & 63, wv = tid >> 6;
  const uint16_t *x = logits + (size_t)t * Vl;
  auto slot = [&](int r) { return xch + ((size_t)r * T + t) * W; };
  if (phase == 3) {
    if (tid == 0) {
      int taken[4] = {-1, -1, -1, -1};
      for (int rd = 0; rd < k; ++rd) {
        unsigned long long best = 0;
        int bq = -1;
        for (int r = 0; r < P; ++r)
          for (int j = 0; j < k; ++j) {
            const float pv = slot(r)[2 * j], iv = slot(r)[2 * j + 1];
            if (iv < 0.f) continue;
            const int q = r * k + j;
            bool used = false;
            for (int z = 0; z < rd; ++z) used |= taken[z] == q;
            if (used) continue;
            const unsigned long long key =
                ((unsigned long long)(f2h_(pv) + 1u) << 32) |
                (unsigned long long)(0xffffffffu - (unsigned)iv);
            if (key > best) best = key, bq = q;
          }
        taken[rd] = bq;
        ids[(size_t)t * k + rd] = (int)(0xffffffffu - (unsigned)(best & 0xffffffffu));
        if (probs) probs[(size_t)t * k + rd] = h2f_((uint16_t)((best >> 32) - 1u));
      }
    }
    return;
  }
  float *own = slot(rank);
  if (phase == 0) {
    float m = -INFINITY;
    for (int i = tid; i < Vl; i += TPB) m = fmaxf(m, h2f_(x[i]));
    m = __ockl_wfred_max_f32(m);
    if (lane == 0) fsh[wv] = m;
    __syncthreads();
#pragma unroll
    for (int q = 0; q < NW; ++q) m = fmaxf(m, fsh[q]);
    if (tid < P * W) {
      const int r = tid / W, w = tid % W;
      slot(r)[w] = (r == rank && w == 0) ? m : 0.f;
    }
    return;
  }
  float M = -INFINITY;
  for (int r = 0; r < P; ++r) M = fmaxf(M, xch[((size_t)r * T + t) * W]);
  if (phase == 1) {
    double se = 0.0;
    for (int i = tid; i < Vl; i += TPB) se += (double)expf_ref(h2f_(x[i]) - M);
    se = __ockl_wfred_add_f64(se);
    if (lane == 0) dsh[wv] = se;
    __syncthreads();
    se = 0.0;
#pragma unroll
    for (int q = 0; q < NW; ++q) se += dsh[q];
    if (tid < P * W) {
      const int r = tid / W, w = tid % W;
      const float hi = (float)se, lo = (float)(se - (double)hi);
      slot(r)[w] = r != rank ? 0.f : (w == 0 ? M : w == 1 ? hi : w == 2 ? lo : 0.f);
    }
    return;
  }
  double sd = 0.0;
  for (int r = 0; r < P; ++r) {
    const float *q = xch + ((size_t)r * T + t) * W;
    sd += (double)q[1] + (double)q[2];
  }
  const float S = (float)sd;
  if (tid == 0) ncand = 0;
  float wm = -INFINITY;
  for (int i = tid; i < Vl; i += TPB) wm = fmaxf(wm, h2f_(x[i]));
  wm = __ockl_wfred_max_f32(wm);
  if (lane == 0) fsh[wv] = wm;
  __syncthreads();
  float L = -INFINITY;
  {
    float top[4] = {-INFINITY, -INFINITY, -INFINITY, -INFINITY};
#pragma unroll
    for (int q = 0; q < NW; ++q) {
      float v = fsh[q];
#pragma unroll
      for (int j = 0; j < 4; ++j) {
        const float hi = fmaxf(top[j], v), lo = fminf(top[j], v);
        top[j] = hi, v = lo;
      }
    }
#pragma unroll
    for (int j = 0; j < 4; ++j)
      if (j == k - 1) L = top[j];
  }
  float thr = -3.402823466e38f;
  {
    const uint16_t pL = f2h_(__fdiv_rn(expf_ref(L - M), S));
    if (pL > 1) {
      const float lo = 0.5f * (h2f_(pL) + h2f_((uint16_t)(pL - 1)));
      thr = M + logf(lo * S) - 0.0009765625f * fmaxf(1.0f, fabsf(M));
    }
  }
  auto key_of = [&](float xv, int i) -> unsigned long long {
    const uint16_t p = f2h_(__fdiv_rn(expf_ref(xv - M), S));
    const unsigned gi = (unsigned)(rank * Vl + i);
    return ((unsigned long long)(p + 1u) << 32) | (unsigned long long)(0xffffffffu - gi);
  };
  auto emit = [&](int rd, unsigned long long b) {
    own[2 * rd] = b ? h2f_((uint16_t)((b >> 32) - 1u)) : 0.f;
    own[2 * rd + 1] = b ? (float)(0xffffffffu - (unsigned)(b & 0xffffffffu)) : -1.f;
  };
  for (int i = tid; i < Vl; i += TPB) {
    const float xv = h2f_(x[i]);
    if (xv >= thr) {
      const unsigned sl = atomicAdd(&ncand, 1u);
      if (sl < (unsigned)kCand) cand[sl] = key_of(xv, i);
    }
  }
  __syncthreads();
  const unsigned n = ncand;
  if (n <= (unsigned)kCand) {
    if (wv == 0) {
      unsigned long long a = (unsigned)lane < n ? cand[lane] : 0ull;
      unsigned long long b = (unsigned)(lane + 64) < n ? cand[lane + 64] : 0ull;
      for (int rd = 0; rd < k; ++rd) {
        const unsigned long long best = __ockl_wfred_max_u64(a > b ? a : b);
        if (lane == 0) emit(rd, best);
        if (best) {
          if (a == best) a = 0ull;
          if (b == best) b = 0ull;
        }
      }
    }
  } else {
    int chosen[4] = {-1, -1, -1, -1};
    for (int rd = 0; rd < k; ++rd) {
      unsigned long long best = 0;
      for (int i = tid; i < Vl; i += TPB) {
        const float xv = h2f_(x[i]);
        if (xv < thr) continue;
        bool used = false;
#pragma unroll
        for (int z = 0; z < 4; ++z) used |= (z < rd && chosen[z] == i);
        if (used) continue;
        const unsigned long long key = key_of(xv, i);
        best = key > best ? key : best;
      }
      best = __ockl_wfred_max_u64(best);
      if (lane == 0) ksh[wv] = best;
      __syncthreads();
      unsigned long long b = ksh[0];
#pragma unroll
      for (int q = 1; q < NW; ++q) b = ksh[q] > b ? ksh[q] : b;
      __syncthreads();
      chosen[rd] = b ? (int)(0xffffffffu - (unsigned)(b & 0xffffffffu)) - rank * Vl : -1;
      if (tid == 0) emit(rd, b);
    }
  }
  if (tid < P * W) {
    const int r = tid / W, w = tid % W;
    if (r != rank) slot(r)[w] = 0.f;
    else if (w >= 2 * k) own[w] = 0.f;
  }
}

hipError_t launch_vshard(const uint16_t *logits, int T, int Vl, int P, int rank, int k,
                         int phase, float *xch, int W, int32_t *ids, float *probs,
                         hipStream_t s) {
  if (T <= 0) return hipSuccess;
  if (k < 1 || k > 4 || P * W > 256 || W < 2 * k || W < 4) return hipErrorInvalidValue;
  hipLaunchKernelGGL((vshard_kernel<1024>), dim3(T), dim3(1024), 0, s, logits, T, Vl, P, rank, k,
                     phase, xch, W, ids, probs);
  return hipGetLastError();
}

struct GroupBufs {
  const void *p[8];
};
__global__ void group_sum_kernel(GroupBufs b, int n, void *__restrict__ out, size_t count,
                                 int dtype) {
  for (size_t i = blockIdx.x * (size_t)blockDim.x + threadIdx.x; i < count;
       i += (size_t)gridDim.x * blockDim.x) {
    if (dtype == FFMI_F16) {
      float a = 0.f;
      for (int r = 0; r < n; ++r) a += h2f_(reinterpret_cast<const uint16_t *>(b.p[r])[i]);
      reinterpret_cast<uint16_t *>(out)[i] = f2h_(a);
    } else if (dtype == FFMI_F32) {
      float a = 0.f;
      for (int r = 0; r < n; ++r) a += reinterpret_cast<const float *>(b.p[r])[i];
      reinterpret_cast<float *>(out)[i] = a;
    } else {
      int a = 0;
      for (int r = 0; r < n; ++r) a += reinterpret_cast<const int *>(b.p[r])[i];
      reinterpret_cast<int *>(out)[i] = a;
    }
  }
}

hipError_t launch_group_sum(const void *const *bufs, int n, void *out, size_t count, int dtype,
                            hipStream_t s) {
  if (n < 1 || n > 8) return hipErrorInvalidValue;
  if (count == 0) return hipSuccess;
  GroupBufs b;
  for (int r = 0; r < 8; ++r) b.p[r] = bufs[r < n ? r : 0];
  size_t blocks = (count + 255) / 256;
  if (blocks > 4096) blocks = 4096;
  hipLaunchKernelGGL(group_sum_kernel, dim3((unsigned)blocks), dim3(256), 0, s, b, n, out, count,
                     dtype);
  return hipGetLastError();
}

}
```

### flexflow_amd/csrc/runtime/llama_gpu.cpp

```cpp
#include <stdio.h>
#include <string.h>

#include <algorithm>
#include <cmath>

#include <string>
#include <map>
#include <tuple>
#include <vector>

#include "model.h"
#include "request_manager.h"

namespace ffmi {

namespace {

struct Layer {
  uint16_t *in_norm = nullptr, *post_norm = nullptr;
  uint16_t *wqkv = nullptr, *wo = nullptr, *wgu = nullptr, *wd = nullptr;
  ffmi_attn *attn = nullptr;
};

struct LlamaGPU : public ffmi_model {
  ffmi_llama_config c{};
  ffmi_model_opts o{};
  int token_capacity() const override { return o.max_tokens; }
  bool uses_collectives() const override { return o.tp_size > 1; }
  std::string weights_folder;
  int Hl = 0, Fl = 0, d = 0, heads_l = 0, slots = 0;
  bool packed = false;
  int wstream = 0;
  hipStream_t stream = nullptr;
  std::vector<Layer> layers;
  uint16_t *embed = nullptr, *final_norm = nullptr, *lm = nullptr;
  uint16_t *res = nullptr, *h = nullptr, *qkv = nullptr, *att = nullptr, *proj = nullptr,
           *mlp = nullptr, *logits = nullptr;
  int32_t *ids_d = nullptr;
  void *topk_ws = nullptr;
  size_t topk_ws_bytes = 0;
  int Vl = 0;
  float *xch = nullptr;
  bool peer = false;
  bool rccl = false;
  bool solo = false;
  int fuse_norms = getenv("FFMI_FUSE_NORM") ? atoi(getenv("FFMI_FUSE_NORM")) : 1;
  float *ss_o = nullptr, *ss_d = nullptr;
  bool fuse_ao = false;
  float *oslab = nullptr;
  int oslab_T = 0;
  int tp_fuse_norm = getenv("FFMI_TP_FUSED_NORM") ? atoi(getenv("FFMI_TP_FUSED_NORM")) : 1;
  int tp_chunks = 1;
  hipStream_t comm_stream = nullptr;
  uint16_t *chunk_buf = nullptr;
  std::vector<hipEvent_t> ev_chunk;
  hipEvent_t ev_comm_done = nullptr;
  float *ws = nullptr;
  size_t ws_bytes = 0;
  size_t ws_chunk = 0;
  bool ar_slabs = !getenv("FFMI_AR_SLABS") || atoi(getenv("FFMI_AR_SLABS")) != 0;
  int32_t *ids_h = nullptr;
  static constexpr int kChain = BeamSearchBatchConfig::MAX_BEAM_DEPTH;
  ffmi_batch_dev *chain_batch[kChain] = {};
  int32_t *ids_dev = nullptr;
  int cur_slot = 0;
  size_t slot_results[kChain] = {};
  std::vector<int> slot_map[kChain];
  hipEvent_t slot_ev[kChain] = {};
  hipEvent_t chain_t0 = nullptr;
  bool slot_ev_live[kChain] = {};
  int last_slot = -1;
  bool chain_ok = !getenv("FFMI_SSM_CHAIN") || atoi(getenv("FFMI_SSM_CHAIN")) != 0;
  size_t slot_ints() const { return (size_t)((o.max_tokens + 15) & ~15) * 4 * 2; }
  bool result_copy = getenv("FFMI_RESULT_COPY") && atoi(getenv("FFMI_RESULT_COPY")) != 0;
  float *probs_h = nullptr;
  ffmi_batch_dev *batch = nullptr;
  PackedStep ps;
  std::vector<void *> allocs;

  enum Cat { GEMM_QKV, GEMM_O, GEMM_GATE_UP, GEMM_DOWN, GEMM_LM_HEAD, ATTENTION, NORM,
             ALLREDUCE, SAMPLING, EMBED, NCAT };
  struct ProfRec {
    int cat;
    hipEvent_t a, b;
    double bytes, flops;
  };
  struct OpStat {
    long launches = 0;
    double ms = 0, bytes = 0, flops = 0;
  };
  int prof_level = 0;
  int prof_every = getenv("FFMI_PROF_EVERY") ? std::max(1, atoi(getenv("FFMI_PROF_EVERY"))) : 4;
  long prof_steps = 0;
  bool prof_this_step = true;
  std::vector<hipEvent_t> ev_pool;
  size_t ev_used = 0;
  std::vector<ProfRec> recs;
  OpStat opstat[NCAT];

  hipEvent_t next_event() {
    if (ev_used == ev_pool.size()) {
      hipEvent_t e;
      (void)hipEventCreate(&e);
      ev_pool.push_back(e);
    }
    return ev_pool[ev_used++];
  }
  bool prof_on(int layer, int T) const {
    if (prof_level == 2) return true;
    if (prof_level == 1)
      return prof_this_step && T <= 256 && (layer == 0 || layer == c.num_layers / 2);
    return false;
  }
  int prof_begin(bool on) {
    if (!on) return -1;
    ProfRec r;
    r.a = next_event();
    r.b = next_event();
    (void)hipEventRecord(r.a, stream);
    recs.push_back(r);
    return (int)recs.size() - 1;
  }
  void prof_end(int idx, int cat, double bytes, double flops) {
    if (idx < 0) return;
    ProfRec &r = recs[idx];
    r.cat = cat;
    r.bytes = bytes;
    r.flops = flops;
    (void)hipEventRecord(r.b, stream);
  }
  void prof_collect() {
    for (auto &r : recs) {
      float ms = 0;
      if (hipEventElapsedTime(&ms, r.a, r.b) != hipSuccess) continue;
      OpStat &o = opstat[r.cat];
      o.launches++;
      o.ms += ms;
      o.bytes += r.bytes;
      o.flops += r.flops;
    }
    recs.clear();
    ev_used = 0;
  }
  ffmi_status set_profiling(int level) override {
    prof_level = level;
    prof_steps = 0;
    for (auto &o : opstat) o = OpStat();
    return FFMI_OK;
  }
  int op_stats(ffmi_op_stat *out, int cap) override {
    static const char *names[NCAT] = {"gemm_qkv", "gemm_o_proj", "gemm_gate_up_silu",
                                      "gemm_down", "gemm_lm_head", "attention", "rmsnorm",
                                      "rowpar_gemm_allreduce", "softmax_argmax", "embedding"};
    int n = 0;
    for (int i = 0; i < NCAT; ++i) {
      if (opstat[i].launches == 0) continue;
      if (out && n < cap) {
        snprintf(out[n].name, sizeof(out[n].name), "%s", names[i]);
        out[n].launches = opstat[i].launches;
        out[n].total_ms = opstat[i].ms;
        out[n].bytes = opstat[i].bytes;
        out[n].flops = opstat[i].flops;
      }
      ++n;
    }
    return n;
  }
  static double gemm_bytes(int T, int N_w, int N_out, int K) {
    return 2.0 * ((double)N_w * K + (double)T * K + (double)T * N_out);
  }
  double attn_bytes() const {
    std::vector<int> kv(o.max_requests, 0);
    for (const auto &w : ps.work) kv[w.req] = std::max(kv[w.req], w.kv_len);
    double b = 0;
    for (int r : kv) b += (double)r * Hl * 2 * 2;
    return b + (double)ps.tokens.size() * (3 * Hl + Hl) * 2;
  }

  static constexpr int kDbgKinds = 10;
  int dbg = 0;
  uint16_t *dbg_buf = nullptr;
  size_t dbg_off[kDbgKinds] = {};
  int dbg_T = -1;
  long debug_width(int k) const override {
    switch (k) {
      case FFMI_DBG_LOGITS: return Vl;
      case FFMI_DBG_QKV: return 3L * Hl;
      case FFMI_DBG_ATTN_OUT: return Hl;
      case FFMI_DBG_MLP_ACT: return Fl;
      case FFMI_DBG_HIDDEN: case FFMI_DBG_ATTN_NORM: case FFMI_DBG_O_PROJ:
      case FFMI_DBG_FFN_NORM: case FFMI_DBG_DOWN: case FFMI_DBG_EMBED: return c.hidden;
    }
    return -1;
  }
  int dbg_layers(int k) const {
    return k == FFMI_DBG_LOGITS ? 0 : k == FFMI_DBG_EMBED ? 1
                                    : k == FFMI_DBG_HIDDEN ? c.num_layers + 1 : c.num_layers;
  }
  bool dbg_is_packed(int k, int layer) const {
    if (!packed) return false;
    return k == FFMI_DBG_ATTN_NORM || k == FFMI_DBG_FFN_NORM || k == FFMI_DBG_ATTN_OUT ||
           k == FFMI_DBG_MLP_ACT || (k == FFMI_DBG_HIDDEN && layer == c.num_layers);
  }
  size_t dbg_tm() const { return (size_t)((o.max_tokens + 15) & ~15); }
  ffmi_status set_debug(int enable) override {
    if (enable && !dbg_buf) {
      size_t total = 0;
      for (int k = 0; k < kDbgKinds; ++k) {
        dbg_off[k] = total;
        total += (size_t)dbg_layers(k) * dbg_tm() * std::max(0L, debug_width(k));
      }
      if (alloc(&dbg_buf, total) != FFMI_OK) return FFMI_ERR_OOM;
    }
    dbg = enable ? 1 : 0;
    dbg_T = -1;
    return FFMI_OK;
  }
  uint16_t *dbg_slot(int k, int l) const {
    return dbg_buf + dbg_off[k] + (size_t)l * dbg_tm() * debug_width(k);
  }
  ffmi_status dbg_copy(int k, int l, const uint16_t *src, int T) {
    const size_t rows = dbg_is_packed(k, l) ? (size_t)((T + 15) & ~15) : (size_t)T;
    FFMI_HIP(hipMemcpyAsync(dbg_slot(k, l), src, rows * debug_width(k) * 2,
                            hipMemcpyDeviceToDevice, stream));
    return FFMI_OK;
  }
  ffmi_status dbg_gemm_out(int k, int l, const uint16_t *Y, const ffmi::Partials &p, int T) {
    if (p.S > 0) {
      FFMI_HIP(ffmi::launch_partials_reduce(p, dbg_slot(k, l), T, (int)debug_width(k), stream));
      return FFMI_OK;
    }
    return dbg_copy(k, l, Y, T);
  }
  long debug_tensor(int which, int layer, float *out, long cap) override {
    if (dbg_T < 0 || (stream && hipStreamSynchronize(stream) != hipSuccess)) return -1;
    if (which < 0 || which >= kDbgKinds) return -1;
    const int T = dbg_T;
    const long width = debug_width(which);
    if (which != FFMI_DBG_LOGITS && (layer < 0 || layer >= dbg_layers(which))) return -1;
    if (cap < (long)T * width) return -1;
    const uint16_t *src = which == FFMI_DBG_LOGITS ? logits : dbg_slot(which, layer);
    const bool pk = which != FFMI_DBG_LOGITS && dbg_is_packed(which, layer);
    const size_t n = (size_t)(pk ? (T + 15) & ~15 : T) * width;
    std::vector<uint16_t> raw(n);
    if (hipMemcpy(raw.data(), src, n * 2, hipMemcpyDeviceToHost) != hipSuccess) return -1;
    for (int t = 0; t < T; ++t)
      for (long j = 0; j < width; ++j) {
        const uint16_t b = raw[pk ? act_packed_off(t, (int)j, (int)width) : (size_t)t * width + j];
        _Float16 v;
        memcpy(&v, &b, 2);
        out[(size_t)t * width + j] = (float)v;
      }
    return T;
  }

  int ar_drop_layer = -1, ar_drop_which = 0;
  bool ar_drop_now = false;
  std::vector<int> head_swapped;

  ffmi_status pack_q_heads(int l, bool swap) {
    const int H = c.hidden, s = o.tp_rank;
    uint16_t *tmp = nullptr;
    FFMI_HIP(hipMalloc((void **)&tmp, (size_t)H * H * 2));
    const std::string p = "model.layers." + std::to_string(l) + ".self_attn.q_proj.weight";
    ffmi_status st = FFMI_OK;
    if (!weights_folder.empty()) {
      st = load_tensor(tmp, (size_t)H * H, p);
    } else if (launch_fill_weight(tmp, (size_t)H * H, ffmi::weight_key(p.c_str(), o.weight_seed),
                                  0, stream) != hipSuccess) {
      st = FFMI_ERR_HIP;
    }
    if (st == FFMI_OK) {
      const int pitch = 3 * (Hl / 16);
      const hipError_t e0 = launch_pack_weight(tmp, H, s * Hl + (swap ? d : 0), 0, d, H,
                                               layers[l].wqkv, 1, 0, pitch, stream);
      const hipError_t e1 = launch_pack_weight(tmp, H, s * Hl + (swap ? 0 : d), 0, d, H,
                                               layers[l].wqkv, 1, d / 16, pitch, stream);
      if (e0 != hipSuccess || e1 != hipSuccess || hipStreamSynchronize(stream) != hipSuccess)
        st = FFMI_ERR_HIP;
    }
    (void)hipFree(tmp);
    return st;
  }

  ffmi_status debug_fault(int kind, int layer, int arg) override {
    if (stream) FFMI_HIP(hipStreamSynchronize(stream));
    if (kind == FFMI_FAULT_TP_HEAD_SWAP) {
      FFMI_CHECK(layer >= -1 && layer < c.num_layers && heads_l >= 2 && d % 16 == 0,
                 FFMI_ERR_INVALID);
      for (int l = 0; l < c.num_layers; ++l)
        if ((layer < 0 || l == layer) &&
            std::find(head_swapped.begin(), head_swapped.end(), l) == head_swapped.end()) {
          ffmi_status st = pack_q_heads(l, true);
          if (st != FFMI_OK) return st;
          head_swapped.push_back(l);
        }
      clear_graphs();
      return FFMI_OK;
    }
    if (kind == FFMI_FAULT_TP_AR_DROP) {
      FFMI_CHECK(o.tp_size > 1 && layer >= 0 && layer < c.num_layers && (arg == 0 || arg == 1),
                 FFMI_ERR_INVALID);
      ar_drop_layer = layer;
      ar_drop_which = arg;
      clear_graphs();
      return FFMI_OK;
    }
    if (kind == FFMI_FAULT_NONE) {
      for (int l : head_swapped) {
        ffmi_status st = pack_q_heads(l, false);
        if (st != FFMI_OK) return st;
      }
      head_swapped.clear();
      ar_drop_layer = -1;
      clear_graphs();
    }
    if (kind == FFMI_FAULT_RESID_ROUND || kind == FFMI_FAULT_NONE) {
      ffmi::set_norm_fault(kind == FFMI_FAULT_RESID_ROUND);
      clear_graphs();
      if (kind == FFMI_FAULT_RESID_ROUND) return FFMI_OK;
    }
    if (kind == FFMI_FAULT_NONE) {
      for (auto &L : layers) {
        ffmi_status st = ffmi::attn_rope_fault(L.attn, -1);
        if (st != FFMI_OK) return st;
      }
      return FFMI_OK;
    }
    FFMI_CHECK(kind == FFMI_FAULT_ROPE_POS && layer >= -1 && layer < c.num_layers,
               FFMI_ERR_INVALID);
    for (int l = 0; l < c.num_layers; ++l)
      if (layer < 0 || l == layer) {
        ffmi_status st = ffmi::attn_rope_fault(layers[l].attn, arg);
        if (st != FFMI_OK) return st;
      }
    return FFMI_OK;
  }

  ~LlamaGPU() override {
    if (stream) (void)hipStreamSynchronize(stream);
    for (auto &kv : st_sum) {
      if (kv.first < 0) {
        fprintf(stderr, "[ffmi step timing] H=%d chain of %d steps: %ld chains, gpu span %.1f us "
                "(%.1f us per step)\n", c.hidden, -kv.first, kv.second.n,
                kv.second.gpu / kv.second.n, kv.second.gpu / kv.second.n / -kv.first);
        continue;
      }
      fprintf(stderr, "[ffmi step timing] H=%d T=%d steps=%ld launch=%.1f gpu=%.1f wait=%.1f total=%.1f us\n",
              c.hidden, kv.first, kv.second.n, kv.second.launch / kv.second.n, kv.second.gpu / kv.second.n,
              kv.second.wait / kv.second.n, kv.second.total / kv.second.n);
    }
    for (auto e : st_ev)
      if (e) (void)hipEventDestroy(e);
    for (auto e : slot_ev)
      if (e) (void)hipEventDestroy(e);
    if (chain_t0) (void)hipEventDestroy(chain_t0);
    clear_graphs();
    for (auto &L : layers) ffmi_attn_destroy(L.attn);
    for (auto e : ev_pool) (void)hipEventDestroy(e);
    for (auto e : ev_chunk) (void)hipEventDestroy(e);
    if (ev_comm_done) (void)hipEventDestroy(ev_comm_done);
    if (comm_stream) (void)hipStreamDestroy(comm_stream);
    for (void *p : allocs) (void)hipFree(p);
    if (ids_h) (void)hipHostFree(ids_h);
    for (int i = 1; i < kChain; ++i) ffmi_batch_destroy(chain_batch[i]);
    ffmi_batch_destroy(batch);
    if (stream) (void)hipStreamDestroy(stream);
  }

  template <typename T>
  ffmi_status alloc(T **p, size_t elems) {
    if (hipMalloc((void **)p, elems * sizeof(T)) != hipSuccess) {
      ffmi_set_last_error("model alloc", __FILE__, __LINE__);
      return FFMI_ERR_OOM;
    }
    allocs.push_back(*p);
    return FFMI_OK;
  }

  ffmi_status load_tensor(uint16_t *dst, size_t n, const std::string &hf_name) {
    std::string file = hf_name.rfind("model.", 0) == 0 ? hf_name.substr(6) : hf_name;
    const bool kv = file.find("self_attn.k_proj") != std::string::npos ||
                    file.find("self_attn.v_proj") != std::string::npos;
    const int group = kv ? c.num_heads / c.num_kv_heads : 1;
    const size_t n_file = n / group;
    const std::string path = weights_folder + "/" + file;
    FILE *f = fopen(path.c_str(), "rb");
    if (!f) {
      ffmi_set_last_error(("weight file not found: " + path).c_str(), __FILE__, __LINE__);
      return FFMI_ERR_INVALID;
    }
    fseek(f, 0, SEEK_END);
    const long bytes = ftell(f);
    fseek(f, 0, SEEK_SET);
    std::vector<uint16_t> h16(n_file);
    bool ok = false;
    if (bytes == (long)(n_file * 2)) {
      ok = fread(h16.data(), 2, n_file, f) == n_file;
    } else if (bytes == (long)(n_file * 4)) {
      std::vector<float> h32(n_file);
      ok = fread(h32.data(), 4, n_file, f) == n_file;
      for (size_t i = 0; ok && i < n_file; ++i) {
        const _Float16 v = (_Float16)h32[i];
        memcpy(&h16[i], &v, 2);
      }
    }
    fclose(f);
    if (!ok) {
      ffmi_set_last_error(("weight file has the wrong size: " + path).c_str(), __FILE__, __LINE__);
      return FFMI_ERR_INVALID;
    }
    if (group > 1) {
      const size_t row_block = n_file / c.num_kv_heads;
      std::vector<uint16_t> rep(n);
      for (int i = 0; i < c.num_heads; ++i)
        memcpy(rep.data() + (size_t)i * row_block, h16.data() + (size_t)(i / group) * row_block,
               row_block * 2);
      h16.swap(rep);
    }
    FFMI_HIP(hipMemcpy(dst, h16.data(), n * 2, hipMemcpyHostToDevice));
    return FFMI_OK;
  }

  ffmi_status init() {
    const int H = c.hidden, F = c.intermediate, V = c.vocab_size, P = o.tp_size;
    FFMI_CHECK(c.num_kv_heads == c.num_heads ||
                   (!weights_folder.empty() && c.num_kv_heads > 0 &&
                    c.num_heads % c.num_kv_heads == 0),
               FFMI_ERR_UNSUPPORTED);
    FFMI_CHECK(H % c.num_heads == 0 && c.num_heads % P == 0 && F % P == 0, FFMI_ERR_INVALID);
    d = H / c.num_heads;
    FFMI_CHECK(d == 64 || d == 128 || (d == 32 && mode == FFMI_MODEL_INC), FFMI_ERR_UNSUPPORTED);
    heads_l = c.num_heads / P;
    Hl = heads_l * d;
    Fl = F / P;
    FFMI_CHECK(H % 32 == 0 && Hl % 32 == 0 && Fl % 32 == 0, FFMI_ERR_UNSUPPORTED);
    FFMI_HIP(hipStreamCreateWithFlags(&stream, hipStreamNonBlocking));
    const int Tm = (o.max_tokens + 15) & ~15;
    packed = H % 32 == 0 && Hl % 32 == 0 && Fl % 32 == 0;
    {
      const double wbytes = 2.0 * c.num_layers * ((double)4 * Hl * H + 3.0 * Fl * H) +
                            2.0 * V * H;
      wstream = wbytes > 192.0 * (1 << 20) ? FFMI_W_STREAM : 0;
      if (const char *e = getenv("FFMI_W_STREAM"))
        wstream = atoi(e) ? FFMI_W_STREAM : 0;
    }
    ffmi_status st;
#define TRY(x) \
  do { if ((st = (x)) != FFMI_OK) return st; } while (0)
    TRY(ffmi_batch_create(Tm, o.max_requests, &batch));
    TRY(alloc(&res, (size_t)Tm * H));
    TRY(alloc(&h, (size_t)Tm * H));
    TRY(alloc(&qkv, (size_t)Tm * 3 * Hl));
    TRY(alloc(&att, (size_t)Tm * Hl));
    TRY(alloc(&proj, (size_t)Tm * H));
    TRY(alloc(&ss_o, (size_t)2 * 32 * (H / 16)));
    ss_d = ss_o + (size_t)32 * (H / 16);
    TRY(alloc(&mlp, (size_t)Tm * Fl));
    fuse_ao = P == 1 && d == 64 && H <= 1024 && H % 16 == 0 &&
              !(getenv("FFMI_FUSE_AO") && atoi(getenv("FFMI_FUSE_AO")) == 0);
    if (fuse_ao) {
      oslab_T = std::min(Tm, 64);
      TRY(alloc(&oslab, (size_t)heads_l * oslab_T * H));
    }
    Vl = P > 1 && V % P == 0 && (V / P) % 16 == 0 ? V / P : V;
    if (const char *e = getenv("FFMI_VOCAB_SHARD"))
      if (!atoi(e)) Vl = V;
    TRY(alloc(&logits, (size_t)Tm * Vl));
    if (Vl != V) TRY(alloc(&xch, (ffmi_vocab_shard_scratch_bytes(P, Tm) + 3) / 4));
    TRY(alloc(&ids_d, (size_t)Tm * 4 * 2));
    topk_ws_bytes = ffmi::argmax_workspace_bytes(std::min(Tm, 256));
    TRY(alloc((char **)&topk_ws, topk_ws_bytes));
    FFMI_HIP(hipMemsetAsync(topk_ws, 0, topk_ws_bytes, stream));
    peer = P > 1 && ffmi::comm_has_peer(o.comm, (size_t)Tm * H * 2);
    if (P > 1 && !peer && ffmi::comm_peer_attached(o.comm) && !ffmi::comm_has_fallback(o.comm)) {
      ffmi_set_last_error("xGMI exchange buffer smaller than max_tokens x hidden fp16 and no "
                          "RCCL communicator", __FILE__, __LINE__);
      return FFMI_ERR_INVALID;
    }
    rccl = P > 1 && !peer && ffmi::comm_is_rccl(o.comm);
    solo = P > 1 && !peer && !rccl && ffmi::comm_size(o.comm) == 1;
    if (peer || rccl) {
      tp_chunks = 2;
      if (const char *e = getenv("FFMI_TP_OVERLAP")) tp_chunks = atoi(e) ? 2 : 1;
      if ((H / tp_chunks) % 32 != 0) tp_chunks = 1;
      FFMI_HIP(hipStreamCreateWithFlags(&comm_stream, hipStreamNonBlocking));
      ev_chunk.resize(tp_chunks);
      for (auto &e : ev_chunk) FFMI_HIP(hipEventCreateWithFlags(&e, hipEventDisableTiming));
      FFMI_HIP(hipEventCreateWithFlags(&ev_comm_done, hipEventDisableTiming));
      if (tp_chunks > 1) TRY(alloc(&chunk_buf, (size_t)Tm * H));
    }
    {
      for (int t = 16; t <= Tm; t += 16) {
        const size_t w1 = ffmi_linear_workspace_bytes(t, 3 * Hl, H, FFMI_EPI_NONE);
        const size_t w2 = ffmi_linear_workspace_bytes(t, H, Hl, FFMI_EPI_NONE);
        const size_t w3 = ffmi_linear_workspace_bytes(t, Fl, H, FFMI_EPI_SILU_MUL);
        const size_t w4 = ffmi_linear_workspace_bytes(t, H, Fl, FFMI_EPI_NONE);
        const size_t w5 = ffmi_linear_workspace_bytes(t, Vl, H, FFMI_EPI_NONE);
        ws_bytes = std::max(ws_bytes, std::max(std::max(std::max(w1, w2), std::max(w3, w4)), w5));
      }
      if (peer && ar_slabs && tp_chunks > 1) {
        const int Hc = H / tp_chunks;
        for (int t = 16; t <= Tm; t += 16)
          ws_chunk = std::max(ws_chunk, std::max(ffmi_linear_workspace_bytes(t, Hc, Hl, FFMI_EPI_NONE),
                                                 ffmi_linear_workspace_bytes(t, Hc, Fl, FFMI_EPI_NONE)));
        ws_chunk = (ws_chunk + 255) & ~(size_t)255;
        ws_bytes = std::max(ws_bytes, ws_chunk * tp_chunks);
      }
      if (ws_bytes) TRY(alloc(&ws, (ws_bytes + 3) / 4));
    }
    FFMI_HIP(hipHostMalloc((void **)&ids_h, (size_t)kChain * Tm * 4 * 2 * sizeof(int32_t),
                           hipHostMallocCoherent | hipHostMallocMapped));
    if (mode == FFMI_MODEL_BEAM) TRY(alloc(&ids_dev, (size_t)kChain * Tm * 4));
    chain_batch[0] = batch;
    if (mode == FFMI_MODEL_BEAM && o.tp_size == 1)
      for (int i = 1; i < kChain; ++i)
        TRY(ffmi_batch_create((o.max_tokens + 15) & ~15, o.max_requests, &chain_batch[i]));
    uint16_t *tmp = nullptr;
    size_t tmp_elems = std::max((size_t)V * H, std::max((size_t)F * H, (size_t)H * H));
    TRY(alloc(&tmp, tmp_elems));
    FFMI_CHECK(o.weight_init >= 0 && o.weight_init <= 2, FFMI_ERR_INVALID);
    const int kres = o.weight_init == 1 ? (FFMI_WKIND_DEPTH | c.num_layers) : 0;
    auto fill = [&](uint16_t *dst, size_t n, const std::string &name, int kind, int cols = 0,
                    uint64_t pa = 1, float scale = 1.0f) -> ffmi_status {
      if (!weights_folder.empty()) return load_tensor(dst, n, name);
      FFMI_CHECK(dst, FFMI_ERR_INVALID);
      FFMI_HIP(ffmi::launch_fill_weight(dst, n, ffmi::weight_key(name.c_str(), o.weight_seed), kind,
                                        stream, cols, pa, 17, scale));
      return FFMI_OK;
    };
    const bool chain = o.weight_init == 2 && weights_folder.empty();
    float chain_scale = 128.0f;
    for (long long f2 = 1; f2 * 32LL * (4096 + 2 * 11008) <
                           (long long)c.num_layers * (c.hidden + 2LL * c.intermediate);
         f2 *= 4)
      chain_scale *= 2.0f;
    TRY(alloc(&embed, (size_t)V * H));
    TRY(fill(embed, (size_t)V * H, "model.embed_tokens.weight", 0, 0, 1, chain ? chain_scale : 1.0f));
    TRY(alloc(&final_norm, H));
    TRY(fill(final_norm, H, "model.norm.weight", 1));
    TRY(alloc(&lm, ffmi_linear_packed_bytes(Vl, H) / 2));
    if (chain)
      TRY(fill(tmp, (size_t)V * H, "model.embed_tokens.weight", 0, H, 7919));
    else
      TRY(fill(tmp, (size_t)V * H, "lm_head.weight", 0));
    FFMI_HIP(launch_pack_weight(tmp, H, Vl == V ? 0 : o.tp_rank * Vl, 0, Vl, H, lm, 1, 0,
                                (Vl + 15) / 16, stream));
    slots = 0;
    layers.resize(c.num_layers);
    const int s = o.tp_rank;
    for (int l = 0; l < c.num_layers; ++l) {
      Layer &L = layers[l];
      const std::string p = "model.layers." + std::to_string(l) + ".";
      TRY(alloc(&L.in_norm, H));
      TRY(fill(L.in_norm, H, p + "input_layernorm.weight", 1));
      TRY(alloc(&L.post_norm, H));
      TRY(fill(L.post_norm, H, p + "post_attention_layernorm.weight", 1));
      const size_t qkv_tiles_bytes = ffmi_linear_packed_bytes(Hl, H);
      TRY(alloc(&L.wqkv, 3 * qkv_tiles_bytes / 2));
      const char *names[3] = {"self_attn.q_proj.weight", "self_attn.k_proj.weight",
                              "self_attn.v_proj.weight"};
      for (int q = 0; q < 3; ++q) {
        TRY(fill(tmp, (size_t)H * H, p + names[q], 0));
        FFMI_HIP(launch_pack_weight(tmp, H, s * Hl, 0, Hl, H, L.wqkv, 1, q * (Hl / 16),
                                    3 * (Hl / 16), stream));
      }
      TRY(alloc(&L.wo, ffmi_linear_packed_bytes(H, Hl) / 2));
      TRY(fill(tmp, (size_t)H * H, p + "self_attn.o_proj.weight", kres));
      FFMI_HIP(launch_pack_weight(tmp, H, 0, s * Hl, H, Hl, L.wo, 1, 0, H / 16, stream));
      TRY(alloc(&L.wgu, 2 * ffmi_linear_packed_bytes(Fl, H) / 2));
      TRY(fill(tmp, (size_t)F * H, p + "mlp.gate_proj.weight", 0));
      FFMI_HIP(launch_pack_weight(tmp, H, s * Fl, 0, Fl, H, L.wgu, 2, 0, 2 * ((Fl + 15) / 16),
                                  stream));
      TRY(fill(tmp, (size_t)F * H, p + "mlp.up_proj.weight", 0));
      FFMI_HIP(launch_pack_weight(tmp, H, s * Fl, 0, Fl, H, L.wgu, 2, 1, 2 * ((Fl + 15) / 16),
                                  stream));
      TRY(alloc(&L.wd, ffmi_linear_packed_bytes(H, Fl) / 2));
      TRY(fill(tmp, (size_t)H * F, p + "mlp.down_proj.weight", kres));
      FFMI_HIP(launch_pack_weight(tmp, F, 0, s * Fl, H, Fl, L.wd, 1, 0, H / 16, stream));
      ffmi_attn_cfg ac{};
      ac.mode = mode == FFMI_MODEL_TREE ? FFMI_ATTN_TREE
                                        : (mode == FFMI_MODEL_BEAM ? FFMI_ATTN_SPEC : FFMI_ATTN_INC);
      ac.num_heads = heads_l;
      ac.head_dim = d;
      ac.max_requests = o.max_requests;
      ac.max_seq_len = o.max_seq_len;
      ac.max_tree_tokens = mode == FFMI_MODEL_INC ? 0 : o.max_tree_tokens;
      ac.max_tokens = Tm;
      ac.qk_scale = 1.0f / sqrtf((float)d);
      ac.rope_theta = c.rope_theta;
      ac.rope_llama3 = c.rope_llama3;
      ac.rope_factor = c.rope_factor;
      ac.rope_low_freq_factor = c.rope_low_freq_factor;
      ac.rope_high_freq_factor = c.rope_high_freq_factor;
      ac.rope_original_max_pos = c.rope_original_max_pos;
      ac.out_layout = packed ? 1 : 0;
      TRY(ffmi_attn_create(&ac, &L.attn));
      int sl = 0;
      ffmi_attn_kv_ptrs(L.attn, nullptr, nullptr, &sl);
      slots = sl;
    }
    FFMI_HIP(hipStreamSynchronize(stream));
    for (auto it = allocs.begin(); it != allocs.end(); ++it)
      if (*it == tmp) {
        (void)hipFree(tmp);
        allocs.erase(it);
        break;
      }
#undef TRY
    return FFMI_OK;
  }

  ffmi_status allreduce(uint16_t *buf, size_t n) {
    if (o.tp_size <= 1) return FFMI_OK;
    return ffmi_allreduce(o.comm, buf, buf, n, FFMI_F16, (ffmi_stream)stream);
  }

  ffmi_status rowpar_gemm_allreduce(const uint16_t *X, const uint16_t *W, int K, uint16_t *out,
                                    int T, int XP) {
    const int H = c.hidden;
    const bool drop = ar_drop_now;
    if (!(peer || rccl) || tp_chunks == 1) {
      ffmi::Partials part;
      FFMI_HIP(ffmi::launch_gemm(X, W, out, ws, ws_bytes, T, H, K, XP, stream,
                                 peer && ar_slabs && !drop ? &part : nullptr));
      if (drop) FFMI_HIP(hipMemsetAsync(out, 0, (size_t)T * H * 2, stream));
      if (peer)
        return ffmi::comm_allreduce_cols(o.comm, out, out, T, H, H, 0, FFMI_F16, stream,
                                         part.S > 0 ? &part : nullptr);
      return allreduce(out, (size_t)T * H);
    }
    const int Hc = H / tp_chunks;
    const size_t tiles = (size_t)(Hc / 16) * ffmi::w_tile_stride((K + 31) / 32);
    for (int ch = 0; ch < tp_chunks; ++ch) {
      uint16_t *cb = chunk_buf + (size_t)ch * T * Hc;
      ffmi::Partials part;
      const bool def = peer && ar_slabs && !drop;
      FFMI_HIP(ffmi::launch_gemm(X, W + ch * tiles, cb,
                                 def ? (float *)((char *)ws + ch * ws_chunk) : ws,
                                 def ? ws_chunk : ws_bytes, T, Hc, K, XP, stream,
                                 def ? &part : nullptr, H / 16));
      if (drop) FFMI_HIP(hipMemsetAsync(cb, 0, (size_t)T * Hc * 2, stream));
      FFMI_HIP(hipEventRecord(ev_chunk[ch], stream));
      FFMI_HIP(hipStreamWaitEvent(comm_stream, ev_chunk[ch], 0));
      if (peer) {
        ffmi_status st = ffmi::comm_allreduce_cols(o.comm, cb, out, T, Hc, H, ch * Hc, FFMI_F16,
                                                   comm_stream, part.S > 0 ? &part : nullptr);
        if (st != FFMI_OK) return st;
      } else {
        ffmi_status st = ffmi_allreduce(o.comm, cb, cb, (size_t)T * Hc, FFMI_F16,
                                        (ffmi_stream)comm_stream);
        if (st != FFMI_OK) return st;
        FFMI_HIP(hipMemcpy2DAsync(out + (size_t)ch * Hc, (size_t)H * 2, cb, (size_t)Hc * 2,
                                  (size_t)Hc * 2, T, hipMemcpyDeviceToDevice, comm_stream));
      }
    }
    FFMI_HIP(hipEventRecord(ev_comm_done, comm_stream));
    FFMI_HIP(hipStreamWaitEvent(stream, ev_comm_done, 0));
    return FFMI_OK;
  }

  ffmi_status rowpar_gemm_allreduce_norm(const uint16_t *X, const uint16_t *W, int K, int T, int XP,
                                         const uint16_t *wnorm) {
    const int H = c.hidden;
    const float eps = c.rms_eps;
    const bool drop = ar_drop_now;
    const bool two = ffmi::comm_two_shot(o.comm, (size_t)T * H * 2);
    if (tp_chunks == 1) {
      ffmi::Partials part;
      FFMI_HIP(ffmi::launch_gemm(X, W, proj, ws, ws_bytes, T, H, K, XP, stream,
                                 ar_slabs && !drop ? &part : nullptr));
      if (drop) FFMI_HIP(hipMemsetAsync(proj, 0, (size_t)T * H * 2, stream));
      return ffmi::comm_allreduce_norm(o.comm, proj, T, H, 0, nullptr, res, wnorm, eps, h, packed,
                                       two, stream, part.S > 0 ? &part : nullptr);
    }
    const int Hc = H / tp_chunks;
    const size_t tiles = (size_t)(Hc / 16) * ffmi::w_tile_stride((K + 31) / 32);
    const int nr = ffmi::comm_size(o.comm), rk = ffmi::comm_rank(o.comm);
    for (int ch = 0; ch < tp_chunks; ++ch) {
      uint16_t *cb = chunk_buf + (size_t)ch * T * Hc;
      ffmi::Partials part;
      const bool def = ar_slabs && !drop;
      FFMI_HIP(ffmi::launch_gemm(X, W + ch * tiles, cb,
                                 def ? (float *)((char *)ws + ch * ws_chunk) : ws,
                                 def ? ws_chunk : ws_bytes, T, Hc, K, XP, stream,
                                 def ? &part : nullptr, H / 16));
      if (drop) FFMI_HIP(hipMemsetAsync(cb, 0, (size_t)T * Hc * 2, stream));
      FFMI_HIP(hipEventRecord(ev_chunk[ch], stream));
      FFMI_HIP(hipStreamWaitEvent(comm_stream, ev_chunk[ch], 0));
      const ffmi::Partials *sl = part.S > 0 ? &part : nullptr;
      ffmi_status st;
      if (ch + 1 < tp_chunks) {
        st = two ? ffmi::comm_reduce_rows(o.comm, cb, proj, T, Hc, H, ch * Hc,
                                          (int)((long)T * rk / nr), (int)((long)T * (rk + 1) / nr),
                                          comm_stream, sl)
                 : ffmi::comm_allreduce_cols(o.comm, cb, proj, T, Hc, H, ch * Hc, FFMI_F16,
                                             comm_stream, sl);
      } else {
        st = ffmi::comm_allreduce_norm(o.comm, cb, T, H, ch * Hc, proj, res, wnorm, eps, h, packed,
                                       two, comm_stream, sl);
      }
      if (st != FFMI_OK) return st;
    }
    FFMI_HIP(hipEventRecord(ev_comm_done, comm_stream));
    FFMI_HIP(hipStreamWaitEvent(stream, ev_comm_done, 0));
    return FFMI_OK;
  }

  struct GraphKey {
    int T, W, C, k, parity, overlap, fused, max_q, slot;
    size_t bytes;
    bool operator<(const GraphKey &o) const {
      return std::tie(T, W, C, k, parity, overlap, fused, max_q, slot, bytes) <
             std::tie(o.T, o.W, o.C, o.k, o.parity, o.overlap, o.fused, o.max_q, o.slot, o.bytes);
    }
  };
  int tree_parity = 0;
  std::map<GraphKey, hipGraphExec_t> graphs;
  int chain_group = getenv("FFMI_CHAIN_GROUP") ? atoi(getenv("FFMI_CHAIN_GROUP")) : kChain - 2;
  struct PendingSlot {
    int slot, T, k;
    size_t bytes;
    GraphKey key;
  };
  std::vector<PendingSlot> pend;
  std::map<std::vector<GraphKey>, hipGraphExec_t> group_graphs;
  bool use_graphs = getenv("FFMI_NO_GRAPHS") == nullptr;
  bool blob_fetch = !getenv("FFMI_BLOB_FETCH") || atoi(getenv("FFMI_BLOB_FETCH")) != 0;
  int graph_max_t = getenv("FFMI_GRAPH_MAXT") ? atoi(getenv("FFMI_GRAPH_MAXT")) : 1024;

  bool inflight = false;
  bool step_timing = getenv("FFMI_STEP_TIMING") && atoi(getenv("FFMI_STEP_TIMING")) != 0;
  hipEvent_t st_ev[2] = {nullptr, nullptr};
  double st_t0 = 0, st_t1 = 0;
  struct StepTime { long n = 0; double launch = 0, gpu = 0, wait = 0, total = 0; };
  std::map<int, StepTime> st_sum;
  int st_T = 0;
  ffmi_status forward(int k) {
    ffmi_status st = forward_launch(k);
    if (st != FFMI_OK) return st;
    return forward_finish();
  }

  ffmi_status forward_launch(int k) {
    inflight = false;
    const int T = (int)ps.tokens.size();
    if (step_timing) {
      if (!st_ev[0]) {
        FFMI_HIP(hipEventCreate(&st_ev[0]));
        FFMI_HIP(hipEventCreate(&st_ev[1]));
      }
      st_t0 = now_us();
      st_T = T;
    }
    prof_this_step = prof_level == 1 && (prof_steps++ % prof_every) == 0;
    ffmi_batch_desc desc;
    ps.desc(&desc);
    const long prev_n = cur_slot > 0 ? (long)slot_results[cur_slot - 1] : 0;
    for (int t = 0; t < T; ++t)
      FFMI_CHECK((desc.tokens[t].token_id >= 0 && desc.tokens[t].token_id < c.vocab_size) ||
                     (desc.tokens[t].token_id < 0 && -1L - desc.tokens[t].token_id < prev_n),
                 FFMI_ERR_INVALID);
    size_t bytes = 0;
    ffmi_status st = ffmi::batch_stage(batch, &desc, &bytes);
    if (st != FFMI_OK) return st;
    if (T == 0) return FFMI_OK;
    probs_h = reinterpret_cast<float *>(ids_h + cur_slot * slot_ints() + (size_t)T * k);
    const bool graph = use_graphs && !dbg && (T <= 64 || (batch->one_item_per_req && T <= graph_max_t)) &&
                       (o.tp_size == 1 || peer || rccl || ffmi::comm_size(o.comm) == 1) &&
                       !prof_on(0, T) &&
                       !prof_on(c.num_layers / 2, T);
    if (graph) {
      const GraphKey key{T, batch->num_work, batch->num_commits, k, tree_parity,
                         batch->commit_overlap ? 1 : 0,
                         (batch->one_item_per_req ? 1 : 0) | (batch->lds_tail ? 2 : 0),
                         batch->max_q, cur_slot, bytes};
      auto it = graphs.find(key);
      if (it == graphs.end()) {
        if (graphs.size() >= 512) clear_graphs();
        hipGraph_t g = nullptr;
        FFMI_HIP(hipStreamBeginCapture(stream, hipStreamCaptureModeThreadLocal));
        st = enqueue(k, bytes, false, T);
        const hipError_t ce = hipStreamEndCapture(stream, &g);
        if (st != FFMI_OK || ce != hipSuccess) {
          if (g) (void)hipGraphDestroy(g);
          if (st != FFMI_OK) return st;
          FFMI_HIP(ce);
        }
        hipGraphExec_t ex = nullptr;
        const hipError_t ie = hipGraphInstantiate(&ex, g, nullptr, nullptr, 0);
        (void)hipGraphDestroy(g);
        FFMI_HIP(ie);
        it = graphs.emplace(key, ex).first;
      }
      if (step_timing) FFMI_HIP(hipEventRecord(st_ev[0], stream));
      FFMI_HIP(hipGraphLaunch(it->second, stream));
    } else {
      if (step_timing) FFMI_HIP(hipEventRecord(st_ev[0], stream));
      st = enqueue(k, bytes, true, T);
      if (st != FFMI_OK) return st;
    }
    if (step_timing) {
      FFMI_HIP(hipEventRecord(st_ev[1], stream));
      st_t1 = now_us();
    }
    inflight = true;
    return FFMI_OK;
  }

  ffmi_status stage_pending(int k, int slot) {
    const int T = (int)ps.tokens.size();
    ffmi_batch_desc desc;
    ps.desc(&desc);
    const long prev_n = slot > 0 ? (long)slot_results[slot - 1] : 0;
    for (int t = 0; t < T; ++t)
      FFMI_CHECK((desc.tokens[t].token_id >= 0 && desc.tokens[t].token_id < c.vocab_size) ||
                     (desc.tokens[t].token_id < 0 && -1L - desc.tokens[t].token_id < prev_n),
                 FFMI_ERR_INVALID);
    size_t bytes = 0;
    ffmi_status st = ffmi::batch_stage(batch, &desc, &bytes);
    if (st != FFMI_OK) return st;
    pend.push_back({slot, T, k, bytes,
                    GraphKey{T, batch->num_work, batch->num_commits, k, tree_parity,
                             batch->commit_overlap ? 1 : 0,
                             (batch->one_item_per_req ? 1 : 0) | (batch->lds_tail ? 2 : 0),
                             batch->max_q, slot, bytes}});
    return FFMI_OK;
  }
  ffmi_status flush_pending() {
    if (pend.empty()) return FFMI_OK;
    std::vector<GraphKey> keys;
    for (const auto &q : pend) keys.push_back(q.key);
    auto it = group_graphs.find(keys);
    if (it == group_graphs.end()) {
      if (group_graphs.size() >= 256) clear_graphs();
      hipGraph_t g = nullptr;
      ffmi_status st = FFMI_OK;
      FFMI_HIP(hipStreamBeginCapture(stream, hipStreamCaptureModeThreadLocal));
      for (const auto &q : pend) {
        cur_slot = q.slot;
        batch = chain_batch[q.slot];
        st = enqueue(q.k, q.bytes, false, q.T);
        if (st != FFMI_OK) break;
      }
      cur_slot = 0;
      batch = chain_batch[0];
      const hipError_t ce = hipStreamEndCapture(stream, &g);
      if (st != FFMI_OK || ce != hipSuccess) {
        if (g) (void)hipGraphDestroy(g);
        pend.clear();
        if (st != FFMI_OK) return st;
        FFMI_HIP(ce);
      }
      hipGraphExec_t ex = nullptr;
      const hipError_t ie = hipGraphInstantiate(&ex, g, nullptr, nullptr, 0);
      (void)hipGraphDestroy(g);
      if (ie != hipSuccess) pend.clear();
      FFMI_HIP(ie);
      it = group_graphs.emplace(keys, ex).first;
    }
    pend.clear();
    FFMI_HIP(hipGraphLaunch(it->second, stream));
    inflight = true;
    return FFMI_OK;
  }

  ffmi_status forward_finish() {
    if (!inflight) return FFMI_OK;
    inflight = false;
    ffmi_status st;
    const double tw = step_timing ? now_us() : 0;
    FFMI_HIP(hipStreamSynchronize(stream));
    if (step_timing) {
      const double te = now_us();
      float ms = 0;
      (void)hipEventElapsedTime(&ms, st_ev[0], st_ev[1]);
      StepTime &q = st_sum[st_T];
      q.n++;
      q.launch += st_t1 - st_t0;
      q.gpu += ms * 1e3;
      q.wait += te - tw;
      q.total += te - st_t0;
    }
    if ((peer || (o.comm && ffmi::comm_peer_attached(o.comm))) &&
        (st = ffmi::comm_status(o.comm)) != FFMI_OK)
      return st;
    if (mode == FFMI_MODEL_TREE) tree_parity ^= 1;
    if (!recs.empty()) prof_collect();
    return FFMI_OK;
  }

  void clear_graphs() {
    for (auto &kv : graphs) (void)hipGraphExecDestroy(kv.second);
    graphs.clear();
    for (auto &kv : group_graphs) (void)hipGraphExecDestroy(kv.second);
    group_graphs.clear();
  }

  ffmi_status enqueue(int k, size_t blob_bytes, bool record_upload, int T) {
    const int H = c.hidden, V = c.vocab_size;
    const float eps = c.rms_eps;
    const ffmi_stream s = (ffmi_stream)stream;
    ffmi_status st;
#define TRY(x) \
  do { if ((st = (x)) != FFMI_OK) return st; } while (0)
    if (!blob_fetch) TRY(ffmi::batch_copy(batch, blob_bytes, stream, record_upload));
    const bool ptail = prof_on(0, T);
    int pr = 0;
    ffmi::Partials down_part;
    static const int marker_h = getenv("FFMI_MARKERS") ? atoi(getenv("FFMI_MARKERS")) : 0;
    static const int marker_t = getenv("FFMI_MARKERS_T") ? atoi(getenv("FFMI_MARKERS_T")) : 0;
    int mark_i = 0;
    const bool fuse = (fuse_norms == 2 || (fuse_norms == 1 && H >= 2048)) && !dbg &&
                      o.tp_size == 1 && T <= 32 && H % 32 == 0 && Hl % 32 == 0 && H <= 4096;
    const bool arn = peer && !solo && o.tp_size > 1 && (tp_fuse_norm == 2 || (tp_fuse_norm == 1 && !dbg));
    for (int l = 0; l < c.num_layers; ++l) {
      Layer &L = layers[l];
      const bool on = prof_on(l, T);
      const bool mark_on = marker_h == c.hidden && l == c.num_layers - 1 && (!marker_t || T == marker_t);
      if (marker_h) ffmi::attn_stamp_gate(mark_on);
      auto mk = [&]() {
        if (mark_on) (void)ffmi::launch_marker(mark_i++, stream);
      };
      if (marker_h && l == 0 && record_upload) (void)ffmi::launch_marker(63, stream);
      mk();
      const int XP = (packed ? FFMI_X_PACKED : 0) | wstream;
      const bool fz_in = fuse && l > 0;
      ffmi::FuseArgs fz_qkv, fz_o, fz_gu, fz_d;
      if (fuse) {
        fz_o.kind = fz_d.kind = 1;
        fz_o.res_in = fz_d.res_in = res;
        fz_o.ss_out = ss_o, fz_d.ss_out = ss_d;
        fz_qkv.kind = fz_gu.kind = 2;
        fz_qkv.ss_in = ss_d, fz_gu.ss_in = ss_o;
        fz_qkv.nss = fz_gu.nss = H / 16;
        fz_qkv.wnorm = L.in_norm, fz_gu.wnorm = L.post_norm;
        fz_qkv.eps = fz_gu.eps = eps;
      }
      if (!fz_in && !(arn && l > 0)) {
        pr = prof_begin(on);
        FFMI_HIP(ffmi::launch_rmsnorm(l == 0 ? embed : res, l == 0 ? nullptr : proj, L.in_norm, res,
                                      h, T, H, eps, stream, packed,
                                      l == 0 ? ffmi::Partials() : down_part,
                                      l == 0 ? (blob_fetch ? batch->host : batch->dev) : nullptr,
                                      l == 0 && blob_fetch ? batch->dev : nullptr, blob_bytes,
                                      cur_slot > 0 ? ids_dev + (size_t)(cur_slot - 1) * (slot_ints() / 2)
                                                   : nullptr));
        if (l == 0 && blob_fetch && record_upload) FFMI_HIP(hipEventRecord(batch->uploaded, stream));
        prof_end(pr, NORM, (double)T * H * 2 * (l == 0 ? 3 : 4), 0);
        mk();
      }
      if (dbg) {
        if (l == 0 || !arn) TRY(dbg_copy(l == 0 ? FFMI_DBG_EMBED : FFMI_DBG_HIDDEN, l == 0 ? 0 : l - 1, res, T));
        TRY(dbg_copy(FFMI_DBG_ATTN_NORM, l, h, T));
      }
      pr = prof_begin(on);
      ffmi::Partials qkv_part;
      FFMI_HIP(ffmi::launch_gemm(fz_in ? res : h, L.wqkv, qkv, (float *)ws, ws_bytes, T, 3 * Hl, H,
                                 fz_in ? wstream : XP, stream, &qkv_part, 0,
                                 fz_in ? &fz_qkv : nullptr));
      prof_end(pr, GEMM_QKV, gemm_bytes(T, 3 * Hl, 3 * Hl, H), 2.0 * T * 3 * Hl * H);
      mk();
      if (dbg) TRY(dbg_gemm_out(FFMI_DBG_QKV, l, qkv, qkv_part, T));
      pr = prof_begin(on);
      ffmi::OprojArgs oa;
      if (fuse_ao && !fuse) {
        oa.wo = L.wo, oa.slab = oslab, oa.N = H, oa.max_T = oslab_T;
        oa.wts = ffmi::w_tile_stride(Hl / 32), oa.wks = ffmi::w_k_stride(H / 16);
      }
      TRY(ffmi::attn_forward(L.attn, batch, qkv, qkv_part, att, s,
                             mode == FFMI_MODEL_TREE ? tree_parity : -1,
                             oa.wo ? &oa : nullptr));
      prof_end(pr, ATTENTION, on ? attn_bytes() : 0, 0);
      mk();
      if (dbg) TRY(dbg_copy(FFMI_DBG_ATTN_OUT, l, att, T));
      ffmi::Partials o_part;
      if (oa.done) {
        o_part.p = oslab, o_part.S = heads_l, o_part.NP = H;
      } else if (fuse) {
        pr = prof_begin(on);
        FFMI_HIP(ffmi::launch_gemm(att, L.wo, res, (float *)ws, ws_bytes, T, H, Hl, XP, stream,
                                   nullptr, 0, &fz_o));
        prof_end(pr, GEMM_O, gemm_bytes(T, H, H, Hl), 2.0 * T * H * Hl);
        mk();
      } else if (o.tp_size == 1 || solo) {
        pr = prof_begin(on);
        FFMI_HIP(ffmi::launch_gemm(att, L.wo, proj, (float *)ws, ws_bytes, T, H, Hl, XP, stream,
                                   H <= 8192 ? &o_part : nullptr));
        prof_end(pr, GEMM_O, gemm_bytes(T, H, H, Hl), 2.0 * T * H * Hl);
        mk();
      } else {
        pr = prof_begin(on);
        ar_drop_now = l == ar_drop_layer && ar_drop_which == 0;
        if (arn) TRY(rowpar_gemm_allreduce_norm(att, L.wo, Hl, T, XP, L.post_norm));
        else TRY(rowpar_gemm_allreduce(att, L.wo, Hl, proj, T, XP));
        ar_drop_now = false;
        prof_end(pr, ALLREDUCE, gemm_bytes(T, H, H, Hl), 2.0 * T * H * Hl);
        mk();
      }
      if (dbg && !arn) TRY(dbg_gemm_out(FFMI_DBG_O_PROJ, l, proj, o_part, T));
      if (!fuse && !arn) {
        pr = prof_begin(on);
        FFMI_HIP(ffmi::launch_rmsnorm(res, proj, L.post_norm, res, h, T, H, eps, stream, packed,
                                      o_part));
        prof_end(pr, NORM, (double)T * H * 2 * 4, 0);
        mk();
      }
      if (dbg) TRY(dbg_copy(FFMI_DBG_FFN_NORM, l, h, T));
      pr = prof_begin(on);
      const int YP = packed ? FFMI_Y_PACKED : 0;
      if (fuse)
        FFMI_HIP(ffmi::launch_gemm(res, L.wgu, mlp, (float *)ws, ws_bytes, T, Fl, H,
                                   FFMI_EPI_SILU_MUL | YP | wstream, stream, nullptr, 0, &fz_gu));
      else
        TRY(ffmi_linear_ws(h, L.wgu, mlp, T, Fl, H, FFMI_EPI_SILU_MUL | XP | YP, ws, ws_bytes, s));
      prof_end(pr, GEMM_GATE_UP, gemm_bytes(T, 2 * Fl, Fl, H), 2.0 * T * 2 * Fl * H);
      mk();
      if (dbg) TRY(dbg_copy(FFMI_DBG_MLP_ACT, l, mlp, T));
      if (fuse) {
        pr = prof_begin(on);
        FFMI_HIP(ffmi::launch_gemm(mlp, L.wd, res, (float *)ws, ws_bytes, T, H, Fl, XP, stream,
                                   nullptr, 0, &fz_d));
        prof_end(pr, GEMM_DOWN, gemm_bytes(T, H, H, Fl), 2.0 * T * H * Fl);
        mk();
        mk();
      } else if (o.tp_size == 1 || solo) {
        pr = prof_begin(on);
        FFMI_HIP(ffmi::launch_gemm(mlp, L.wd, proj, (float *)ws, ws_bytes, T, H, Fl, XP, stream,
                                   H <= 8192 ? &down_part : nullptr));
        prof_end(pr, GEMM_DOWN, gemm_bytes(T, H, H, Fl), 2.0 * T * H * Fl);
        mk();
        mk();
      } else {
        pr = prof_begin(on);
        ar_drop_now = l == ar_drop_layer && ar_drop_which == 1;
        if (arn)
          TRY(rowpar_gemm_allreduce_norm(mlp, L.wd, Fl, T, XP,
                                         l + 1 < c.num_layers ? layers[l + 1].in_norm : final_norm));
        else TRY(rowpar_gemm_allreduce(mlp, L.wd, Fl, proj, T, XP));
        ar_drop_now = false;
        prof_end(pr, ALLREDUCE, gemm_bytes(T, H, H, Fl), 2.0 * T * H * Fl);
        mk();
      }
      if (dbg && !arn) TRY(dbg_gemm_out(FFMI_DBG_DOWN, l, proj, down_part, T));
    }
    const int XP = (packed ? FFMI_X_PACKED : 0) | wstream;
    const bool tail_mark = marker_h == c.hidden && (!marker_t || T == marker_t);
    auto mkt = [&]() {
      if (tail_mark) (void)ffmi::launch_marker(mark_i++, stream);
    };
    if (!arn) {
      pr = prof_begin(ptail);
      if (fuse)
        FFMI_HIP(ffmi::launch_rmsnorm(res, nullptr, final_norm, nullptr, h, T, H, eps, stream, packed));
      else
        FFMI_HIP(ffmi::launch_rmsnorm(res, proj, final_norm, res, h, T, H, eps, stream, packed,
                                      down_part));
      prof_end(pr, NORM, (double)T * H * 2 * 4, 0);
    }
    mkt();
    if (dbg) {
      if (!arn) TRY(dbg_copy(FFMI_DBG_HIDDEN, c.num_layers - 1, res, T));
      TRY(dbg_copy(FFMI_DBG_HIDDEN, c.num_layers, h, T));
      dbg_T = T;
    }
    pr = prof_begin(ptail);
    TRY(ffmi_linear_ws(h, lm, logits, T, Vl, H, FFMI_EPI_NONE | XP, ws, ws_bytes, s));
    prof_end(pr, GEMM_LM_HEAD, gemm_bytes(T, Vl, Vl, H), 2.0 * T * Vl * H);
    mkt();
    pr = prof_begin(ptail);
    TRY(enqueue_sampling(k, T));
    prof_end(pr, SAMPLING, (double)T * V * 2, 0);
    mkt();
#undef TRY
    return FFMI_OK;
  }

  ffmi_status enqueue_sampling(int k, int T) {
    const int V = c.vocab_size;
    const ffmi_stream s = (ffmi_stream)stream;
    ffmi_status st;
#define TRY(x) \
  do { if ((st = (x)) != FFMI_OK) return st; } while (0)
    int32_t *ids_o = result_copy ? ids_d : ids_h + cur_slot * slot_ints();
    float *probs_o = reinterpret_cast<float *>(ids_o + (size_t)T * k);
    if (Vl != V) {
      TRY(ffmi_vocab_shard_topk(o.comm, logits, T, Vl, k, ids_o, probs_o, xch, s));
    } else {
      FFMI_CHECK(k >= 1 && k <= 4 && k <= V, FFMI_ERR_INVALID);
      FFMI_HIP(ffmi::launch_argmax(logits, T, V, k, ids_o, probs_o, stream, topk_ws, topk_ws_bytes,
                                   mode == FFMI_MODEL_BEAM
                                       ? ids_dev + (size_t)cur_slot * (slot_ints() / 2)
                                       : nullptr));
    }
    if (result_copy)
      FFMI_HIP(hipMemcpyAsync(ids_h + cur_slot * slot_ints(), ids_d, (size_t)T * k * 8,
                              hipMemcpyDeviceToHost, stream));
#undef TRY
    return FFMI_OK;
  }

  ffmi_status run_inc(const BatchConfig &bc, InferenceResult *ir) override {
    if (mode != FFMI_MODEL_INC) return FFMI_ERR_INVALID;
    FFMI_CHECK(bc.num_tokens <= o.max_tokens, FFMI_ERR_INVALID);
    pack_inc(bc, o.max_requests, slots, &ps);
    cur_slot = 0;
    ffmi_status st = forward(1);
    if (st != FFMI_OK) return st;
    memcpy(ir->token_ids, ids_h, bc.num_tokens * sizeof(int32_t));
    return FFMI_OK;
  }
  ffmi_status run_tree(const TreeVerifyBatchConfig &bc, InferenceResult *ir) override {
    if (mode != FFMI_MODEL_TREE) return FFMI_ERR_INVALID;
    FFMI_CHECK(bc.num_tokens <= o.max_tokens, FFMI_ERR_INVALID);
    pack_tree(bc, o.max_requests, slots, &ps);
    cur_slot = 0;
    ffmi_status st = forward(1);
    if (st != FFMI_OK) return st;
    memcpy(ir->token_ids, ids_h, bc.num_tokens * sizeof(int32_t));
    return FFMI_OK;
  }
  ffmi_status run_beam(const BeamSearchBatchConfig &bc, BeamInferenceResult *ir) override {
    ffmi_status st = beam_launch(bc);
    if (st != FFMI_OK) return st;
    return beam_collect(ir);
  }
  ffmi_status beam_launch(const BeamSearchBatchConfig &bc) override {
    return beam_launch_chained(bc, 0);
  }
  ffmi_status beam_collect(BeamInferenceResult *ir) override { return beam_collect_chained(0, ir); }
  bool can_chain_beam() const override {
    return chain_ok && mode == FFMI_MODEL_BEAM && o.tp_size == 1 && !dbg && !result_copy;
  }
  ffmi_status beam_launch_chained(const BeamSearchBatchConfig &bc, int slot) override {
    if (mode != FFMI_MODEL_BEAM) return FFMI_ERR_INVALID;
    FFMI_CHECK(bc.num_tokens <= o.max_tokens && slot >= 0 && slot < kChain, FFMI_ERR_INVALID);
    FFMI_CHECK(slot == 0 || can_chain_beam(), FFMI_ERR_INVALID);
    if (!chain_batch[slot]) {
      ffmi_batch_dev *b = nullptr;
      ffmi_status st = ffmi_batch_create((o.max_tokens + 15) & ~15, o.max_requests, &b);
      if (st != FFMI_OK) return st;
      chain_batch[slot] = b;
    }
    pack_beam(bc, o.max_requests, slots, &ps);
    for (auto &ti : ps.tokens)
      if (ti.token_id < 0) {
        const long i = -1L - ti.token_id;
        FFMI_CHECK(slot > 0 && i < (long)slot_map[slot - 1].size(), FFMI_ERR_INVALID);
        ti.token_id = -1 - slot_map[slot - 1][i];
      }
    const int k = ps.topk;
    if (step_timing && slot == 0) {
      if (!chain_t0) FFMI_HIP(hipEventCreate(&chain_t0));
      FFMI_HIP(hipEventRecord(chain_t0, stream));
    }
    cur_slot = slot;
    batch = chain_batch[slot];
    slot_results[slot] = (size_t)bc.num_tokens * k;
    beam_result_layout(bc, &slot_map[slot]);
    const int Ts = (int)ps.tokens.size();
    const bool grp = chain_group >= 2 && slot >= 1 && slot <= kChain - 2 && use_graphs && !dbg &&
                     prof_level == 0 && Ts > 0 && Ts <= 64;
    ffmi_status st;
    if (grp) {
      st = stage_pending(k, slot);
      if (st == FFMI_OK && ((slot - 1) % chain_group == chain_group - 1 || slot == kChain - 2)) {
        cur_slot = 0;
        batch = chain_batch[0];
        st = flush_pending();
      }
    } else {
      cur_slot = 0;
      batch = chain_batch[0];
      st = flush_pending();
      cur_slot = slot;
      batch = chain_batch[slot];
      if (st == FFMI_OK) st = forward_launch(k);
    }
    batch = chain_batch[0];
    cur_slot = 0;
    static const int slot_events =
        getenv("FFMI_CHAIN_EVENTS") ? atoi(getenv("FFMI_CHAIN_EVENTS")) : 2;
    const bool record = slot_events == 1 || (slot_events == 2 && slot == kChain - 2);
    if (st == FFMI_OK) last_slot = slot;
    if (st == FFMI_OK && record) {
      if (!slot_ev[slot])
        FFMI_HIP(hipEventCreateWithFlags(&slot_ev[slot], step_timing ? 0 : hipEventDisableTiming));
      FFMI_HIP(hipEventRecord(slot_ev[slot], stream));
      slot_ev_live[slot] = true;
      last_slot = slot;
    }
    return st;
  }
  ffmi_status beam_collect_chained(int slot, BeamInferenceResult *ir) override {
    FFMI_CHECK(slot >= 0 && slot < kChain, FFMI_ERR_INVALID);
    {
      ffmi_status st = flush_pending();
      if (st != FFMI_OK) return st;
    }
    int ev = -1;
    for (int e = slot; e < last_slot && ev < 0; ++e)
      if (slot_ev_live[e] && slot_ev[e]) ev = e;
    if (ev >= 0) {
      FFMI_HIP(hipEventSynchronize(slot_ev[ev]));
    } else {
      const int ls = last_slot;
      ffmi_status st = forward_finish();
      if (st != FFMI_OK) return st;
      for (bool &b : slot_ev_live) b = false;
      if (step_timing && ls > 0 && chain_t0) {
        float ms = 0;
        if (hipEventElapsedTime(&ms, chain_t0, slot_ev[ls]) == hipSuccess) {
          StepTime &q = st_sum[-(ls + 1)];
          q.n++;
          q.gpu += ms * 1e3;
        }
      }
      last_slot = -1;
    }
    const size_t n = slot_results[slot];
    const int32_t *ids = ids_h + slot * slot_ints();
    const float *pr = reinterpret_cast<const float *>(ids + n);
    const std::vector<int> &map = slot_map[slot];
    for (size_t i = 0; i < map.size(); ++i) {
      ir->token_ids[i] = ids[map[i]];
      ir->probs[i] = pr[map[i]];
      ir->parent_id[i] = 0;
    }
    return FFMI_OK;
  }
};

}

ffmi_status create_llama_gpu(const ffmi_llama_config *cfg, const ffmi_model_opts *o,
                             ffmi_model **out) {
  FFMI_CHECK(cfg && o && out, FFMI_ERR_INVALID);
  FFMI_CHECK(o->tp_size >= 1 && o->tp_rank >= 0 && o->tp_rank < o->tp_size, FFMI_ERR_INVALID);
  FFMI_CHECK(o->tp_size == 1 || o->comm, FFMI_ERR_INVALID);
  FFMI_CHECK(o->max_tokens > 0 && o->max_tokens <= BatchConfig::MAX_NUM_TOKENS, FFMI_ERR_INVALID);
  FFMI_CHECK(o->max_requests > 0 && o->max_requests <= BatchConfig::MAX_NUM_REQUESTS,
             FFMI_ERR_INVALID);
  int ndev = 0;
  if (hipGetDeviceCount(&ndev) != hipSuccess || ndev == 0) return FFMI_ERR_NO_DEVICE;
  LlamaGPU *m = new LlamaGPU();
  m->mode = o->mode;
  m->c = *cfg;
  m->o = *o;
  if (o->weights_folder && o->weights_folder[0]) m->weights_folder = o->weights_folder;
  m->o.weights_folder = nullptr;
  ffmi_status st = m->init();
  if (st != FFMI_OK) {
    delete m;
    return st;
  }
  *out = m;
  return FFMI_OK;
}

}
```

### flexflow_amd/ffmi.py

```python
import ctypes
import os

_HERE = os.path.dirname(os.path.abspath(__file__))
_VARIANT = os.environ.get("FFMI_LIB_VARIANT", "")
LIB_PATH = os.path.join(_HERE, f"libffmi_{_VARIANT}.so" if _VARIANT else "libffmi.so")

c_int, c_float, c_void_p, c_size_t, c_uint64, c_int64, c_double, c_long = (
    ctypes.c_int, ctypes.c_float, ctypes.c_void_p, ctypes.c_size_t, ctypes.c_uint64,
    ctypes.c_int64, ctypes.c_double, ctypes.c_long)

FFMI_OK = 0
STATUS = {0: "ok", 1: "invalid argument", 2: "hip error", 3: "rccl error", 4: "oom",
          5: "unsupported", 6: "no gfx950 device"}
ATTN_INC, ATTN_SPEC, ATTN_TREE = 0, 1, 2
MODEL_INC, MODEL_BEAM, MODEL_TREE = 0, 1, 2
DBG_KINDS = {"hidden": 0, "logits": 1, "attn_norm": 2, "qkv": 3, "attn_out": 4, "o_proj": 5,
             "ffn_norm": 6, "mlp_act": 7, "down": 8, "embed": 9}
DBG_HIDDEN, DBG_LOGITS = DBG_KINDS["hidden"], DBG_KINDS["logits"]
EPI_NONE, EPI_SILU_MUL = 0, 1
X_PACKED = 0x10
Y_PACKED = 0x20
W_STREAM = 0x40
F16, F32, I32 = 0, 1, 2
WEIGHT_INITS = {"uniform": 0, "depth_scaled": 1, "token_chain": 2}
FAULT_NONE, FAULT_ROPE_POS, FAULT_RESID_ROUND, FAULT_TP_HEAD_SWAP, FAULT_TP_AR_DROP = 0, 1, 2, 3, 4
SPEC_EXT_WIDTH4, SPEC_EXT_MULTI_SSM = 1, 2
ATTN_QTILE = 32
MAX_TREE = 64


class TokenInfo(ctypes.Structure):
    _fields_ = [(n, ctypes.c_int32) for n in
                ("token_id", "pos", "req", "store_slot", "prefix_len", "tree_base",
                 "tree_len", "tree_bit")] + [("tree_vis", ctypes.c_uint64)]


class AttnWork(ctypes.Structure):
    _fields_ = [(n, ctypes.c_int32) for n in ("req", "q_start", "q_count", "kv_len")]


class CommitInfo(ctypes.Structure):
    _fields_ = [(n, ctypes.c_int32) for n in ("src_token", "req", "depth", "pad")]


class BatchDesc(ctypes.Structure):
    _fields_ = [("num_tokens", ctypes.c_int32), ("num_work", ctypes.c_int32),
                ("num_commits", ctypes.c_int32), ("num_mask_reqs", ctypes.c_int32),
                ("tokens", ctypes.POINTER(TokenInfo)), ("work", ctypes.POINTER(AttnWork)),
                ("commits", ctypes.POINTER(CommitInfo)),
                ("masks", ctypes.POINTER(ctypes.c_uint64))]


class AttnCfg(ctypes.Structure):
    _fields_ = [("mode", c_int), ("num_heads", c_int), ("head_dim", c_int),
                ("max_requests", c_int), ("max_seq_len", c_int), ("max_tree_tokens", c_int),
                ("max_tokens", c_int), ("qk_scale", c_float), ("rope_theta", c_float),
                ("out_layout", c_int), ("rope_llama3", c_int), ("rope_factor", c_float),
                ("rope_low_freq_factor", c_float), ("rope_high_freq_factor", c_float),
                ("rope_original_max_pos", c_int), ("full_precision", c_int)]


class LlamaConfig(ctypes.Structure):
    _fields_ = [("num_layers", c_int), ("vocab_size", c_int), ("num_heads", c_int),
                ("num_kv_heads", c_int), ("hidden", c_int), ("intermediate", c_int),
                ("rms_eps", c_float), ("rope_theta", c_float), ("rope_llama3", c_int),
                ("rope_factor", c_float), ("rope_low_freq_factor", c_float),
                ("rope_high_freq_factor", c_float), ("rope_original_max_pos", c_int)]

    @classmethod
    def from_dict(cls, d):
        return cls(d["num_layers"], d["vocab_size"], d["num_heads"],
                   d.get("num_kv_heads", d["num_heads"]), d["hidden"], d["intermediate"],
                   d.get("rms_eps", 1e-6), d.get("rope_theta", 10000.0),
                   d.get("rope_llama3", 0), d.get("rope_factor", 1.0),
                   d.get("rope_low_freq_factor", 1.0), d.get("rope_high_freq_factor", 4.0),
                   d.get("rope_original_max_pos", 8192))


class ModelOpts(ctypes.Structure):
    _fields_ = [("mode", c_int), ("tp_rank", c_int), ("tp_size", c_int), ("comm", c_void_p),
                ("max_requests", c_int), ("max_tokens", c_int), ("max_seq_len", c_int),
                ("max_tree_tokens", c_int), ("weight_seed", c_uint64), ("use_graphs", c_int),
                ("weights_folder", ctypes.c_char_p), ("weight_init", c_int),
                ("full_precision", c_int)]


class RMConfig(ctypes.Structure):
    _fields_ = [("max_requests_per_batch", c_int), ("max_tokens_per_batch", c_int),
                ("max_spec_tree_token_num", c_int), ("max_sequence_length", c_int),
                ("bos_token_id", c_int), ("eos_token_ids", ctypes.POINTER(c_int)),
                ("num_eos", c_int), ("spec_tree_width", ctypes.POINTER(c_int)),
                ("num_tree_width", c_int), ("verbose", c_int), ("spec_extensions", c_int)]


class Profile(ctypes.Structure):
    _fields_ = [("llm_decoding_steps", c_int), ("ssm_decoding_steps", c_int),
                ("start_us", c_double), ("finish_us", c_double),
                ("registration_us", c_double), ("first_token_us", c_double),
                ("input_len", c_int), ("output_len", c_int)]


class OpStat(ctypes.Structure):
    _fields_ = [("name", ctypes.c_char * 32), ("launches", c_long), ("total_ms", c_double),
                ("bytes", c_double), ("flops", c_double)]


class ServeStats(ctypes.Structure):
    _fields_ = [("llm_steps", c_long), ("ssm_steps", c_long), ("tokens_committed", c_long),
                ("tree_tokens_verified", c_long), ("request_verifies", c_long),
                ("wall_us", c_double), ("llm_us", c_double), ("ssm_us", c_double),
                ("ssm_phases_chained", c_long), ("ssm_exchange_us", c_double)]


ALLGATHER_FN = ctypes.CFUNCTYPE(c_int, c_void_p, c_void_p, c_size_t, c_void_p)

SIGNATURES = {
    "ffmi_batch_create": (c_int, [c_int, c_int, ctypes.POINTER(c_void_p)]),
    "ffmi_batch_destroy": (None, [c_void_p]),
    "ffmi_batch_upload": (c_int, [c_void_p, ctypes.POINTER(BatchDesc), c_void_p]),
    "ffmi_attn_create": (c_int, [ctypes.POINTER(AttnCfg), ctypes.POINTER(c_void_p)]),
    "ffmi_attn_destroy": (None, [c_void_p]),
    "ffmi_attn_inc": (c_int, [c_void_p] * 5),
    "ffmi_attn_spec": (c_int, [c_void_p] * 5),
    "ffmi_attn_tree": (c_int, [c_void_p] * 5),
    "ffmi_attn_kv_ptrs": (c_int, [c_void_p, ctypes.POINTER(c_void_p), ctypes.POINTER(c_void_p),
                                  ctypes.POINTER(c_int)]),
    "ffmi_linear_packed_bytes": (c_size_t, [c_int, c_int]),
    "ffmi_linear_pack_weight": (c_int, [c_void_p, c_int, c_int, c_void_p, c_void_p]),
    "ffmi_linear_pack_gate_up": (c_int, [c_void_p, c_void_p, c_int, c_int, c_void_p, c_void_p]),
    "ffmi_linear": (c_int, [c_void_p, c_void_p, c_void_p, c_int, c_int, c_int, c_int, c_void_p]),
    "ffmi_linear_f32": (c_int, [c_void_p, c_void_p, c_void_p, c_int, c_int, c_int, c_void_p]),
    "ffmi_rmsnorm_f32": (c_int, [c_void_p, c_void_p, c_void_p, c_int, c_int, c_float, c_void_p]),
    "ffmi_residual_rmsnorm_f32": (c_int, [c_void_p, c_void_p, c_void_p, c_void_p, c_void_p, c_int,
                                          c_int, c_float, c_void_p]),
    "ffmi_silu_mul_f32": (c_int, [c_void_p, c_void_p, c_void_p, c_size_t, c_void_p]),
    "ffmi_arg_topk_f32": (c_int, [c_void_p, c_int, c_int, c_int, c_void_p, c_void_p, c_void_p]),
    "ffmi_linear_workspace_bytes": (c_size_t, [c_int, c_int, c_int, c_int]),
    "ffmi_linear_ws": (c_int, [c_void_p, c_void_p, c_void_p, c_int, c_int, c_int, c_int, c_void_p,
                               c_size_t, c_void_p]),
    "ffmi_rmsnorm": (c_int, [c_void_p, c_void_p, c_void_p, c_int, c_int, c_float, c_void_p]),
    "ffmi_residual_rmsnorm": (c_int, [c_void_p] * 5 + [c_int, c_int, c_float, c_void_p]),
    "ffmi_comm_unique_id": (c_int, [c_void_p]),
    "ffmi_comm_create": (c_int, [c_void_p, c_int, c_int, ctypes.POINTER(c_void_p)]),
    "ffmi_comm_create_local": (c_int, [c_int, ctypes.POINTER(c_void_p)]),
    "ffmi_comm_destroy": (None, [c_void_p]),
    "ffmi_comm_create_peer": (c_int, [c_int, c_int, ctypes.POINTER(c_void_p)]),
    "ffmi_comm_peer_export": (c_int, [c_void_p, c_size_t, c_void_p]),
    "ffmi_comm_peer_attach": (c_int, [c_void_p, c_void_p]),
    "ffmi_comm_peer_status": (c_int, [c_void_p]),
    "ffmi_comm_peer_detach": (c_int, [c_void_p]),
    "ffmi_vocab_shard_scratch_bytes": (c_size_t, [c_int, c_int]),
    "ffmi_vocab_shard_topk": (c_int, [c_void_p, c_void_p, c_int, c_int, c_int, c_void_p,
                                      c_void_p, c_void_p, c_void_p]),
    "ffmi_allreduce": (c_int, [c_void_p, c_void_p, c_void_p, c_size_t, c_int, c_void_p]),
    "ffmi_allreduce_rmsnorm": (c_int, [c_void_p, c_void_p, c_int, c_int, c_int, c_void_p, c_void_p,
                                       c_void_p, c_float, c_void_p, c_int, c_void_p, c_void_p]),
    "ffmi_embedding": (c_int, [c_void_p, c_void_p, c_void_p, c_int, c_void_p]),
    "ffmi_silu_mul": (c_int, [c_void_p, c_void_p, c_void_p, c_size_t, c_void_p]),
    "ffmi_argmax": (c_int, [c_void_p, c_int, c_int, c_void_p, c_void_p, c_void_p]),
    "ffmi_arg_topk": (c_int, [c_void_p, c_int, c_int, c_int, c_void_p, c_void_p, c_void_p]),
    "ffmi_arg_topk_workspace_bytes": (c_size_t, [c_int]),
    "ffmi_arg_topk_ws": (c_int, [c_void_p, c_int, c_int, c_int, c_void_p, c_void_p, c_void_p,
                                 c_size_t, c_void_p]),
    "ffmi_fill_weight": (c_int, [c_void_p, c_size_t, ctypes.c_char_p, c_uint64, c_int, c_void_p]),
    "ffmi_model_create": (c_int, [ctypes.POINTER(LlamaConfig), ctypes.POINTER(ModelOpts),
                                  ctypes.POINTER(c_void_p)]),
    "ffmi_model_destroy": (None, [c_void_p]),
    "ffmi_model_set_profiling": (c_int, [c_void_p, c_int]),
    "ffmi_model_op_stats": (c_int, [c_void_p, ctypes.POINTER(OpStat), c_int]),
    "ffmi_model_set_debug": (c_int, [c_void_p, c_int]),
    "ffmi_model_debug_tensor": (ctypes.c_long, [c_void_p, c_int, c_int, c_void_p, ctypes.c_long]),
    "ffmi_model_debug_width": (ctypes.c_long, [c_void_p, c_int]),
    "ffmi_model_debug_fault": (c_int, [c_void_p, c_int, c_int, c_int]),
    "ffmi_set_device": (c_int, [c_int]),
    "ffmi_rm_create": (c_int, [ctypes.POINTER(RMConfig), ctypes.POINTER(c_void_p)]),
    "ffmi_rm_destroy": (None, [c_void_p]),
    "ffmi_rm_register_ssm": (c_int, [c_void_p, c_void_p]),
    "ffmi_rm_register_remote_ssm": (c_int, [c_void_p]),
    "ffmi_rm_set_ssm_exchange": (c_int, [c_void_p, c_int, c_int, c_void_p, c_void_p]),
    "ffmi_rm_set_ssm_exchange_comm": (c_int, [c_void_p, c_void_p]),
    "ffmi_comm_allgather": (c_int, [c_void_p, c_void_p, c_size_t, c_void_p]),
    "ffmi_rm_register_output_filepath": (c_int, [c_void_p, ctypes.c_char_p]),
    "ffmi_rm_register_detokenizer": (c_int, [c_void_p, c_void_p, c_void_p]),
    "ffmi_rm_set_old_llama_tokenizer": (c_int, [c_void_p, c_int]),
    "ffmi_rm_register_request": (c_int64, [c_void_p, ctypes.POINTER(c_int), c_int, c_int, c_int,
                                           c_int]),
    "ffmi_rm_serve_incr_decoding": (c_int, [c_void_p, c_void_p]),
    "ffmi_rm_serve_spec_infer": (c_int, [c_void_p, c_void_p]),
    "ffmi_rm_get_output": (c_int, [c_void_p, c_int64, ctypes.POINTER(c_int), c_int]),
    "ffmi_rm_get_profile": (c_int, [c_void_p, c_int64, ctypes.POINTER(Profile)]),
    "ffmi_rm_get_stats": (c_int, [c_void_p, ctypes.POINTER(ServeStats)]),
    "ffmi_status_str": (ctypes.c_char_p, [c_int]),
    "ffmi_version": (ctypes.c_char_p, []),
    "ffmi_last_error": (ctypes.c_char_p, []),
    "ffmi_packed_activation_bytes": (ctypes.c_size_t, [c_int, c_int]),
    "ffmi_rmsnorm_ex": (c_int, [c_void_p, c_void_p, c_void_p, c_void_p, c_void_p, c_int, c_int,
                                c_float, c_int, c_void_p]),
    "ffmi_pack_activations": (c_int, [c_void_p, c_int, c_int, c_void_p, c_void_p]),
    "ffmi_debug_gemm_stamps": (ctypes.c_long, [c_void_p, ctypes.c_long]),
    "ffmi_debug_gemm_plan": (c_int, [c_int, c_int, c_int, c_int, ctypes.POINTER(c_int)]),
    "ffmi_debug_fused_residual_linear": (c_int, [c_void_p, c_void_p, c_void_p, c_void_p, c_int,
                                                 c_int, c_int, c_void_p]),
    "ffmi_debug_fused_norm_linear": (c_int, [c_void_p, c_void_p, c_void_p, c_float, c_void_p,
                                             c_void_p, c_int, c_int, c_int, c_int, c_void_p]),
    "ffmi_debug_attn_stamps": (ctypes.c_long, [c_void_p, ctypes.c_long]),
    "ffmi_debug_markers": (ctypes.c_long, [c_void_p, ctypes.c_long]),
}

TEST_SIGNATURES = {
    "ffmi_test_hash_model_create": (c_int, [c_int, c_int, c_int, c_int, c_int, c_uint64, c_int,
                                            ctypes.POINTER(c_void_p)]),
    "ffmi_test_hash_model_set_capacity": (c_int, [c_void_p, c_int]),
}
TEST_LIB_PATH = os.path.join(os.path.dirname(LIB_PATH), "libffmi_testmodel.so")

_lib = None
_test_lib = None


def test_lib():
    global _test_lib
    if _test_lib is None:
        lib()
        L = ctypes.CDLL(TEST_LIB_PATH, mode=ctypes.RTLD_GLOBAL)
        for name, (res, args) in TEST_SIGNATURES.items():
            fn = getattr(L, name)
            fn.restype = res
            fn.argtypes = args
        _test_lib = L
    return _test_lib


def lib():
    global _lib
    if _lib is None:
        if not os.path.exists(LIB_PATH):
            raise ImportError(f"libffmi.so not built at {LIB_PATH}; run "
                              "`python -c 'import __graft_entry__ as g; g.build()'`")
        L = ctypes.CDLL(LIB_PATH, mode=ctypes.RTLD_GLOBAL)
        for name, (res, args) in SIGNATURES.items():
            fn = getattr(L, name)
            fn.restype = res
            fn.argtypes = args
        _lib = L
    return _lib


DETOKENIZE_FN = ctypes.CFUNCTYPE(c_int, ctypes.POINTER(c_int), c_int, ctypes.c_void_p, c_int,
                                 c_void_p)


class FFMIError(RuntimeError):
    pass


def check(st, what=""):
    if st != FFMI_OK:
        msg = lib().ffmi_last_error().decode(errors="replace")
        raise FFMIError(f"{what}: {STATUS.get(st, st)} [{msg}]")


def int_array(vals):
    arr = (c_int * max(1, len(vals)))(*vals)
    return arr
```

### include/ffmi.h

```cpp
#ifndef FFMI_H_
#define FFMI_H_

#include <stddef.h>
#include <stdint.h>

#ifdef __cplusplus
extern "C" {
#endif

typedef struct ihipStream_t *ffmi_stream;

typedef enum {
  FFMI_OK = 0,
  FFMI_ERR_INVALID = 1,
  FFMI_ERR_HIP = 2,
  FFMI_ERR_NCCL = 3,
  FFMI_ERR_OOM = 4,
  FFMI_ERR_UNSUPPORTED = 5,
  FFMI_ERR_NO_DEVICE = 6
} ffmi_status;

typedef enum { FFMI_F16 = 0, FFMI_F32 = 1, FFMI_I32 = 2 } ffmi_dtype;

typedef enum {
  FFMI_ATTN_INC = 0,
  FFMI_ATTN_SPEC = 1,
  FFMI_ATTN_TREE = 2
} ffmi_attn_mode;


typedef struct {
  int32_t token_id;
  int32_t pos;
  int32_t req;
  int32_t store_slot;
  int32_t prefix_len;
  int32_t tree_base;
  int32_t tree_len;
  int32_t tree_bit;
  uint64_t tree_vis;
} ffmi_token_info;

typedef struct {
  int32_t req;
  int32_t q_start;
  int32_t q_count;
  int32_t kv_len;
} ffmi_attn_work;

typedef struct {
  int32_t src_token;
  int32_t req;
  int32_t depth;
  int32_t pad;
} ffmi_commit_info;

#define FFMI_ATTN_QTILE 32
#define FFMI_MAX_TREE 64

typedef struct {
  int32_t num_tokens;
  int32_t num_work;
  int32_t num_commits;
  int32_t num_mask_reqs;
  const ffmi_token_info *tokens;
  const ffmi_attn_work *work;
  const ffmi_commit_info *commits;
  const uint64_t *masks;
} ffmi_batch_desc;

typedef struct ffmi_batch_dev ffmi_batch_dev;

ffmi_status ffmi_batch_create(int max_tokens, int max_requests, ffmi_batch_dev **out);
void ffmi_batch_destroy(ffmi_batch_dev *b);
ffmi_status ffmi_batch_upload(ffmi_batch_dev *b, const ffmi_batch_desc *desc,
                              ffmi_stream stream);

typedef struct {
  int mode;
  int num_heads;
  int head_dim;
  int max_requests;
  int max_seq_len;
  int max_tree_tokens;
  int max_tokens;
  float qk_scale;
  float rope_theta;
  int out_layout;
  int rope_llama3;
  float rope_factor, rope_low_freq_factor, rope_high_freq_factor;
  int rope_original_max_pos;
  int full_precision;
} ffmi_attn_cfg;

typedef struct ffmi_attn ffmi_attn;

ffmi_status ffmi_attn_create(const ffmi_attn_cfg *cfg, ffmi_attn **out);
void ffmi_attn_destroy(ffmi_attn *h);
ffmi_status ffmi_attn_inc(ffmi_attn *h, const ffmi_batch_dev *b, const void *qkv,
                          void *out, ffmi_stream stream);
ffmi_status ffmi_attn_spec(ffmi_attn *h, const ffmi_batch_dev *b, const void *qkv,
                           void *out, ffmi_stream stream);
ffmi_status ffmi_attn_tree(ffmi_attn *h, const ffmi_batch_dev *b, const void *qkv,
                           void *out, ffmi_stream stream);
ffmi_status ffmi_attn_kv_ptrs(ffmi_attn *h, void **k, void **v, int *slots);

typedef enum {
  FFMI_EPI_NONE = 0,
  FFMI_EPI_SILU_MUL = 1
} ffmi_epilogue;

#define FFMI_X_PACKED 0x10
#define FFMI_Y_PACKED 0x20
#define FFMI_W_STREAM 0x40
size_t ffmi_packed_activation_bytes(int T, int in_dim);
ffmi_status ffmi_pack_activations(const void *X, int T, int in_dim, void *X_packed,
                                  ffmi_stream stream);

size_t ffmi_linear_packed_bytes(int out_dim, int in_dim);
ffmi_status ffmi_linear_pack_weight(const void *W, int out_dim, int in_dim,
                                    void *W_packed, ffmi_stream stream);
ffmi_status ffmi_linear_pack_gate_up(const void *Wg, const void *Wu, int out_dim,
                                     int in_dim, void *W_packed, ffmi_stream stream);
ffmi_status ffmi_linear(const void *X, const void *W_packed, void *Y, int T,
                        int out_dim, int in_dim, int epilogue, ffmi_stream stream);
ffmi_status ffmi_linear_f32(const float *X, const float *W, float *Y, int T, int out_dim,
                            int in_dim, ffmi_stream stream);
size_t ffmi_linear_workspace_bytes(int T, int out_dim, int in_dim, int epilogue);
ffmi_status ffmi_linear_ws(const void *X, const void *W_packed, void *Y, int T,
                           int out_dim, int in_dim, int epilogue, void *workspace,
                           size_t workspace_bytes, ffmi_stream stream);

ffmi_status ffmi_rmsnorm(const void *x, const void *w, void *out, int T, int H,
                         float eps, ffmi_stream stream);
ffmi_status ffmi_residual_rmsnorm(const void *x1, const void *x2, const void *w,
                                  void *residual_out, void *out, int T, int H,
                                  float eps, ffmi_stream stream);
ffmi_status ffmi_rmsnorm_ex(const void *x1, const void *x2, const void *w, void *residual_out,
                            void *out, int T, int H, float eps, int flags, ffmi_stream stream);

typedef struct ffmi_comm ffmi_comm;
#define FFMI_UNIQUE_ID_BYTES 128
ffmi_status ffmi_comm_unique_id(void *id_out );
ffmi_status ffmi_comm_create(const void *id, int nranks, int rank, ffmi_comm **out);
ffmi_status ffmi_comm_create_local(int nranks, ffmi_comm **out);
void ffmi_comm_destroy(ffmi_comm *c);
ffmi_status ffmi_allreduce(ffmi_comm *c, const void *in, void *out, size_t count,
                           int dtype, ffmi_stream stream);

size_t ffmi_vocab_shard_scratch_bytes(int nranks, int T);
ffmi_status ffmi_vocab_shard_topk(ffmi_comm *c, const void *logits, int T, int Vl, int k,
                                  int32_t *ids, float *probs, void *scratch, ffmi_stream stream);

#define FFMI_PEER_HANDLE_BYTES 64
ffmi_status ffmi_comm_create_peer(int nranks, int rank, ffmi_comm **out);
ffmi_status ffmi_comm_peer_export(ffmi_comm *c, size_t max_bytes,
                                  void *handle_out );
ffmi_status ffmi_comm_peer_attach(ffmi_comm *c, const void *handles );
ffmi_status ffmi_comm_allgather(ffmi_comm *c, const void *mine, size_t bytes, void *all);
ffmi_status ffmi_comm_peer_status(ffmi_comm *c);
ffmi_status ffmi_comm_peer_detach(ffmi_comm *c);
ffmi_status ffmi_allreduce_rmsnorm(ffmi_comm *c, const void *in, int T, int H, int col0,
                                   const void *prev, void *residual, const void *w, float eps,
                                   void *out, int flags, int *rows_out, ffmi_stream stream);

ffmi_status ffmi_embedding(const ffmi_batch_dev *b, const void *table, void *out,
                           int H, ffmi_stream stream);
ffmi_status ffmi_silu_mul(const void *a, const void *b, void *out, size_t n,
                          ffmi_stream stream);
ffmi_status ffmi_argmax(const void *logits, int T, int V, int32_t *ids,
                        float *probs, ffmi_stream stream);
ffmi_status ffmi_arg_topk(const void *logits, int T, int V, int k, int32_t *ids,
                          float *probs, ffmi_stream stream);
size_t ffmi_arg_topk_workspace_bytes(int T);
ffmi_status ffmi_arg_topk_ws(const void *logits, int T, int V, int k, int32_t *ids,
                             float *probs, void *workspace, size_t workspace_bytes,
                             ffmi_stream stream);
ffmi_status ffmi_rmsnorm_f32(const float *x, const float *w, float *out, int T, int H, float eps,
                             ffmi_stream stream);
ffmi_status ffmi_residual_rmsnorm_f32(const float *x1, const float *x2, const float *w,
                                      float *residual_out, float *out, int T, int H, float eps,
                                      ffmi_stream stream);
ffmi_status ffmi_silu_mul_f32(const float *a, const float *b, float *out, size_t n,
                              ffmi_stream stream);
ffmi_status ffmi_arg_topk_f32(const float *logits, int T, int V, int k, int32_t *ids,
                              float *probs, ffmi_stream stream);
#define FFMI_WKIND_DEPTH 0x10000
ffmi_status ffmi_fill_weight(void *dst_f16, size_t n, const char *name,
                             uint64_t seed, int kind, ffmi_stream stream);

typedef struct {
  int num_layers, vocab_size, num_heads, num_kv_heads, hidden, intermediate;
  float rms_eps, rope_theta;
  int rope_llama3;
  float rope_factor, rope_low_freq_factor, rope_high_freq_factor;
  int rope_original_max_pos;
} ffmi_llama_config;

typedef enum {
  FFMI_MODEL_INC = 0,
  FFMI_MODEL_BEAM = 1,
  FFMI_MODEL_TREE = 2
} ffmi_model_mode;

typedef struct {
  int mode;
  int tp_rank, tp_size;
  ffmi_comm *comm;
  int max_requests;
  int max_tokens;
  int max_seq_len;
  int max_tree_tokens;
  uint64_t weight_seed;
  int use_graphs;
  const char *weights_folder;
  int weight_init;
  int full_precision;
} ffmi_model_opts;

typedef struct ffmi_model ffmi_model;
ffmi_status ffmi_model_create(const ffmi_llama_config *cfg, const ffmi_model_opts *o,
                              ffmi_model **out);
void ffmi_model_destroy(ffmi_model *m);
typedef struct {
  char name[32];
  long launches;
  double total_ms;
  double bytes;
  double flops;
} ffmi_op_stat;
ffmi_status ffmi_model_set_profiling(ffmi_model *m, int level);
int ffmi_model_op_stats(ffmi_model *m, ffmi_op_stat *out, int cap);
#define FFMI_DBG_HIDDEN 0
#define FFMI_DBG_LOGITS 1
#define FFMI_DBG_ATTN_NORM 2
#define FFMI_DBG_QKV 3
#define FFMI_DBG_ATTN_OUT 4
#define FFMI_DBG_O_PROJ 5
#define FFMI_DBG_FFN_NORM 6
#define FFMI_DBG_MLP_ACT 7
#define FFMI_DBG_DOWN 8
#define FFMI_DBG_EMBED 9
ffmi_status ffmi_model_set_debug(ffmi_model *m, int enable);
long ffmi_model_debug_tensor(ffmi_model *m, int which, int layer, float *out, long cap);
long ffmi_model_debug_width(ffmi_model *m, int which);
#define FFMI_FAULT_NONE 0
#define FFMI_FAULT_ROPE_POS 1
#define FFMI_FAULT_RESID_ROUND 2
#define FFMI_FAULT_TP_HEAD_SWAP 3
#define FFMI_FAULT_TP_AR_DROP 4
ffmi_status ffmi_model_debug_fault(ffmi_model *m, int kind, int layer, int arg);
ffmi_status ffmi_set_device(int device);

typedef struct ffmi_rm ffmi_rm;
typedef struct {
  int max_requests_per_batch;
  int max_tokens_per_batch;
  int max_spec_tree_token_num;
  int max_sequence_length;
  int bos_token_id;
  const int *eos_token_ids;
  int num_eos;
  const int *spec_tree_width;
  int num_tree_width;
  int verbose;
  int spec_extensions;
} ffmi_rm_config;
#define FFMI_SPEC_EXT_WIDTH4 1
#define FFMI_SPEC_EXT_MULTI_SSM 2

ffmi_status ffmi_rm_create(const ffmi_rm_config *cfg, ffmi_rm **out);
void ffmi_rm_destroy(ffmi_rm *rm);
ffmi_status ffmi_rm_register_ssm(ffmi_rm *rm, ffmi_model *ssm);
typedef int (*ffmi_allgather_fn)(void *ctx, const void *mine, size_t bytes, void *all);
ffmi_status ffmi_rm_register_remote_ssm(ffmi_rm *rm);
ffmi_status ffmi_rm_set_ssm_exchange(ffmi_rm *rm, int nranks, int rank, ffmi_allgather_fn fn,
                                     void *ctx);
ffmi_status ffmi_rm_set_ssm_exchange_comm(ffmi_rm *rm, ffmi_comm *comm);
ffmi_status ffmi_rm_register_output_filepath(ffmi_rm *rm, const char *path);
typedef int (*ffmi_detokenize_fn)(const int *ids, int n, char *buf, int cap, void *ctx);
ffmi_status ffmi_rm_register_detokenizer(ffmi_rm *rm, ffmi_detokenize_fn fn, void *ctx);
ffmi_status ffmi_rm_set_old_llama_tokenizer(ffmi_rm *rm, int enable);
int64_t ffmi_rm_register_request(ffmi_rm *rm, const int *prompt, int n_prompt,
                                 int max_length, int max_new_tokens,
                                 int add_special_tokens);
ffmi_status ffmi_rm_serve_incr_decoding(ffmi_rm *rm, ffmi_model *llm);
ffmi_status ffmi_rm_serve_spec_infer(ffmi_rm *rm, ffmi_model *llm);
int ffmi_rm_get_output(ffmi_rm *rm, int64_t guid, int *tokens, int cap);
typedef struct {
  int llm_decoding_steps, ssm_decoding_steps;
  double start_us, finish_us, registration_us, first_token_us;
  int input_len, output_len;
} ffmi_profile;
ffmi_status ffmi_rm_get_profile(ffmi_rm *rm, int64_t guid, ffmi_profile *p);
typedef struct {
  long llm_steps, ssm_steps, tokens_committed, tree_tokens_verified;
  long request_verifies;
  double wall_us;
  double llm_us, ssm_us;
  long ssm_phases_chained;
  double ssm_exchange_us;
} ffmi_serve_stats;
ffmi_status ffmi_rm_get_stats(ffmi_rm *rm, ffmi_serve_stats *s);



ffmi_status ffmi_debug_fused_residual_linear(const void *X, const void *W_packed, void *residual,
                                             float *ss_out, int T, int out_dim, int in_dim,
                                             ffmi_stream stream);
ffmi_status ffmi_debug_fused_norm_linear(const void *residual, const float *ss_in,
                                         const void *norm_w, float eps, const void *W_packed,
                                         void *Y, int T, int out_dim, int in_dim, int epilogue,
                                         ffmi_stream stream);

long ffmi_debug_gemm_stamps(long long *dst, long max_waves);
ffmi_status ffmi_debug_gemm_plan(int T, int out_dim, int in_dim, int epilogue, int *plan );
long ffmi_debug_attn_stamps(long long *dst, long max_waves);
long ffmi_debug_markers(long long *dst, long n);

const char *ffmi_status_str(ffmi_status s);
const char *ffmi_last_error(void);
const char *ffmi_version(void);

#ifdef __cplusplus
}
#endif
#endif
```

Before: 1366 tokens/s.

## Fold next-step embedding gather and RMSNorm into SSM top-k sampling kernel

When consecutive chained SSM steps are captured in one graph, the softmax/top-k kernel of one step now also copies the next step's batch blob, gathers the next tokens' embeddings (including tree-resolved ids from its own top-k output) and applies the first-layer RMSNorm. The next step then skips its layer-0 rmsnorm launch. This removes a kernel launch and a dependency hop per chained step in the small draft model (H<=1024). It adds shared-memory use and a tail phase to the top-k kernel, plus host-side eligibility checks. A debug API and step-timing event fixes are included.

```diff
diff --git a/flexflow_amd/csrc/api.cpp b/flexflow_amd/csrc/api.cpp
--- a/flexflow_amd/csrc/api.cpp
+++ b/flexflow_amd/csrc/api.cpp
@@ -547,6 +547,53 @@
   return FFMI_OK;
 }
 
+extern "C" ffmi_status ffmi_debug_topk_gather_norm(
+    const void *logits, int T, int V, int k, int32_t *ids, float *probs, int32_t *ids_dev,
+    void *workspace, size_t workspace_bytes, ffmi_batch_dev *b, const ffmi_batch_desc *next,
+    const void *table, const void *norm_w, void *res, void *h, int H, float eps, int flags,
+    void *blob_dst, size_t *blob_bytes, int fold, ffmi_stream stream) {
+  FFMI_CHECK(logits && ids && ids_dev && b && next && table && norm_w && res && h && blob_dst &&
+                 blob_bytes,
+             FFMI_ERR_INVALID);
+  FFMI_CHECK(T > 0 && V > 0 && k >= 1 && k <= 4 && k <= V && H > 0 && H % 8 == 0 && H <= 16384,
+             FFMI_ERR_INVALID);
+  FFMI_CHECK((flags & ~FFMI_Y_PACKED) == 0, FFMI_ERR_INVALID);
+  const bool packed = (flags & FFMI_Y_PACKED) != 0;
+  FFMI_CHECK(!packed || H % 32 == 0, FFMI_ERR_UNSUPPORTED);
+  FFMI_CHECK(next->num_tokens > 0, FFMI_ERR_INVALID);
+  for (int t = 0; t < next->num_tokens; ++t) {
+    const long id = next->tokens[t].token_id;
+    FFMI_CHECK((id >= 0 && id < V) || (id < 0 && -1L - id < (long)T * k), FFMI_ERR_INVALID);
+  }
+  size_t bytes = 0;
+  const ffmi_status st = ffmi::batch_stage(b, next, &bytes);
+  if (st != FFMI_OK) return st;
+  *blob_bytes = bytes;
+  const hipStream_t s = (hipStream_t)stream;
+  if (fold) {
+    ffmi::ArgmaxNext nx;
+    nx.blob = b->host;
+    nx.tok_off = reinterpret_cast<const ffmi::BatchHeader *>(b->host)->off_tokens;
+    nx.T = next->num_tokens;
+    nx.embed = (const uint16_t *)table, nx.w = (const uint16_t *)norm_w;
+    nx.res = (uint16_t *)res, nx.h = (uint16_t *)h;
+    nx.H = H, nx.eps = eps, nx.out_packed = packed;
+    nx.blob_dst = (char *)blob_dst, nx.blob_bytes = bytes;
+    FFMI_CHECK(ffmi::argmax_can_fold((const uint16_t *)logits, T, V, nx), FFMI_ERR_UNSUPPORTED);
+    FFMI_HIP(ffmi::launch_argmax((const uint16_t *)logits, T, V, k, ids, probs, s, workspace,
+                                 workspace_bytes, ids_dev, &nx));
+  } else {
+    FFMI_HIP(ffmi::launch_argmax((const uint16_t *)logits, T, V, k, ids, probs, s, workspace,
+                                 workspace_bytes, ids_dev));
+    FFMI_HIP(ffmi::launch_rmsnorm((const uint16_t *)table, nullptr, (const uint16_t *)norm_w,
+                                  (uint16_t *)res, (uint16_t *)h, next->num_tokens, H, eps, s,
+                                  packed, ffmi::Partials(), b->host, (char *)blob_dst, bytes,
+                                  ids_dev));
+  }
+  FFMI_HIP(hipEventRecord(b->uploaded, s));
+  return FFMI_OK;
+}
+
 extern "C" ffmi_status ffmi_debug_fused_residual_linear(const void *X, const void *W_packed,
                                                         void *residual, float *ss_out, int T,
                                                         int out_dim, int in_dim,
diff --git a/flexflow_amd/csrc/ffmi_internal.h b/flexflow_amd/csrc/ffmi_internal.h
--- a/flexflow_amd/csrc/ffmi_internal.h
+++ b/flexflow_amd/csrc/ffmi_internal.h
@@ -165,9 +165,24 @@
                             uint16_t *out, int H, hipStream_t s);
 hipError_t launch_silu_mul(const uint16_t *a, const uint16_t *b, uint16_t *out,
                            size_t n, hipStream_t s);
+struct ArgmaxNext {
+  const char *blob = nullptr;
+  int tok_off = 0;
+  int T = 0;
+  const uint16_t *embed = nullptr, *w = nullptr;
+  uint16_t *res = nullptr, *h = nullptr;
+  int H = 0;
+  float eps = 0.f;
+  bool out_packed = false;
+  char *blob_dst = nullptr;
+  size_t blob_bytes = 0;
+};
+constexpr int kArgmaxNextMaxT = 256;
 hipError_t launch_argmax(const uint16_t *logits, int T, int V, int k, int32_t *ids,
                          float *probs, hipStream_t s, void *ws = nullptr, size_t ws_bytes = 0,
-                         int32_t *ids2 = nullptr);
+                         int32_t *ids2 = nullptr,
+                         const ArgmaxNext *next = nullptr);
+bool argmax_can_fold(const uint16_t *logits, int T, int V, const ArgmaxNext &next);
 size_t argmax_workspace_bytes(int T);
 hipError_t launch_vshard(const uint16_t *logits, int T, int Vl, int P, int rank, int k,
                          int phase, float *xch, int W, int32_t *ids, float *probs,
diff --git a/flexflow_amd/csrc/kernels/norm.hip b/flexflow_amd/csrc/kernels/norm.hip
--- a/flexflow_amd/csrc/kernels/norm.hip
+++ b/flexflow_amd/csrc/kernels/norm.hip
@@ -256,11 +256,21 @@
 extern "C" __device__ double __ockl_wfred_add_f64(double);
 extern "C" __device__ unsigned long long __ockl_wfred_max_u64(unsigned long long);
 
-template <int TPB, int NV, int G>
-__global__ __launch_bounds__(TPB) void softmax_topk_reg_kernel(
+struct TopkNext {
+  const char *blob;
+  const uint16_t *embed, *w;
+  uint16_t *res, *h;
+  uint4 *blob_dst;
+  int T, tok_off, H, out_packed, blob_n16;
+  float eps;
+};
+
+template <int TPB, int NV, int G, bool NEXT>
+__device__ __forceinline__ void softmax_topk_reg_body(
     const uint16_t *__restrict__ logits, int V, int k, int32_t *__restrict__ ids,
     float *__restrict__ probs, double *__restrict__ part, unsigned *__restrict__ cnt,
-    int32_t *__restrict__ ids2) {
+    int32_t *__restrict__ ids2, const TopkNext &nx) {
+  static_assert(!NEXT || TPB == 1024, "next-step gather norm: 8 groups of 128 threads");
   constexpr int NW = TPB / 64;
   constexpr int kCand = 128;
   static_assert(G == 1 || ((NV * 8) % G == 0 && NV * 8 / G >= 2),
@@ -286,6 +296,15 @@
     const int i = gv(v);
     r[v] = i < nvec ? x[i] : make_uint4(0xfc00fc00u, 0xfc00fc00u, 0xfc00fc00u, 0xfc00fc00u);
   }
+  [[maybe_unused]] const int nrows = G == 1 ? gridDim.x : gridDim.y;
+  [[maybe_unused]] int ntok = 0;
+  [[maybe_unused]] uint4 bl = make_uint4(0, 0, 0, 0);
+  [[maybe_unused]] const int bl_i = row * TPB + tid;
+  if constexpr (NEXT) {
+    if (tid < nx.T)
+      ntok = reinterpret_cast<const ffmi_token_info *>(nx.blob + nx.tok_off)[tid].token_id;
+    if (chunk == 0 && bl_i < nx.blob_n16) bl = reinterpret_cast<const uint4 *>(nx.blob)[bl_i];
+  }
   if (tid == 0) ncand = 0;
   auto elem = [&](int v, int e) -> float {
     const uint32_t w = (&r[v].x)[e >> 1];
@@ -349,6 +368,13 @@
   double sd = 0.0;
 #pragma unroll
   for (int q = 0; q < NW; ++q) sd += sh[q];
+  if constexpr (NEXT) {
+    if (chunk == 0) {
+      if (bl_i < nx.blob_n16) nx.blob_dst[bl_i] = bl;
+      const uint4 *src = reinterpret_cast<const uint4 *>(nx.blob);
+      for (int i = bl_i + nrows * TPB; i < nx.blob_n16; i += nrows * TPB) nx.blob_dst[i] = src[i];
+    }
+  }
   if constexpr (G > 1) {
     if (wv == 0) {
       unsigned before = 0;
@@ -391,10 +417,15 @@
     const uint16_t p = f2h_(__fdiv_rn(expf_ref(xv - M), S));
     return ((unsigned long long)(p + 1u) << 32) | (unsigned long long)(0xffffffffu - i);
   };
+  __shared__ int row_ids[4];
+  __shared__ int2 nwork[NEXT ? kArgmaxNextMaxT : 1];
+  __shared__ unsigned nnwork;
+  __shared__ double nsc[2][NW];
   auto emit = [&](int rd, unsigned long long b) {
     ids[(size_t)row * k + rd] = (int)(0xffffffffu - (unsigned)(b & 0xffffffffu));
     if (ids2) ids2[(size_t)row * k + rd] = (int)(0xffffffffu - (unsigned)(b & 0xffffffffu));
     if (probs) probs[(size_t)row * k + rd] = h2f_((uint16_t)((b >> 32) - 1u));
+    if constexpr (NEXT) row_ids[rd] = (int)(0xffffffffu - (unsigned)(b & 0xffffffffu));
   };
 #pragma unroll
   for (int v = 0; v < NV; ++v)
@@ -407,9 +438,12 @@
         if (slot < (unsigned)kCand) cand[slot] = key_of(xv, i);
       }
     }
+  if constexpr (NEXT)
+    if (tid == 0) nnwork = 0;
   __syncthreads();
   const unsigned n = ncand;
-  if (n <= (unsigned)kCand) {
+  const bool few = n <= (unsigned)kCand;
+  if (few) {
     if (wv == 0) {
       unsigned long long a = (unsigned)lane < n ? cand[lane] : 0ull;
       unsigned long long b = (unsigned)(lane + 64) < n ? cand[lane + 64] : 0ull;
@@ -420,9 +454,9 @@
         if (b == best) b = 0ull;
       }
     }
-    return;
-  }
-  for (int rd = 0; rd < k; ++rd) {
+    if constexpr (!NEXT) return;
+  }
+  for (int rd = 0; rd < (few ? 0 : k); ++rd) {
     unsigned long long best = 0;
 #pragma unroll
     for (int v = 0; v < NV; ++v)
@@ -457,6 +491,76 @@
         }
     }
   }
+  if constexpr (NEXT) {
+    __syncthreads();
+    if (tid < nx.T) {
+      const int e = -1 - ntok;
+      const bool mine = ntok < 0 ? e / k == row : tid % nrows == row;
+      if (mine) {
+        const unsigned slot = atomicAdd(&nnwork, 1u);
+        nwork[slot] = make_int2(tid, ntok < 0 ? row_ids[e - row * k] : ntok);
+      }
+    }
+    __syncthreads();
+    const int nw = (int)nnwork, H = nx.H, nchunk = H >> 3;
+    const int g = tid >> 7, ch = tid & 127;
+    for (int base = 0, par = 0; base < nw; base += TPB / 128, par ^= 1) {
+      const bool on = base + g < nw && ch < nchunk;
+      int t = 0;
+      uint4 xa = make_uint4(0, 0, 0, 0), wv8 = xa;
+      double ss = 0.0;
+      if (on) {
+        const int2 rec = nwork[base + g];
+        t = rec.x;
+        xa = *reinterpret_cast<const uint4 *>(nx.embed + (size_t)rec.y * H + ch * 8);
+        wv8 = *reinterpret_cast<const uint4 *>(nx.w + ch * 8);
+        *reinterpret_cast<uint4 *>(nx.res + (size_t)t * H + ch * 8) = xa;
+        const uint16_t *e = reinterpret_cast<const uint16_t *>(&xa);
+#pragma unroll
+        for (int q = 0; q < 8; ++q) {
+          const float f = h2f_(e[q]);
+          ss += (double)f * (double)f;
+        }
+      }
+#pragma unroll
+      for (int o = 32; o > 0; o >>= 1) ss += __shfl_xor(ss, o);
+      if (lane == 0) nsc[par][wv] = ss;
+      __syncthreads();
+      double rs = nsc[par][2 * g];
+      rs += nsc[par][2 * g + 1];
+      const float sum = (float)rs;
+      const float rms_f = __fdiv_rn(1.0f, sqrtf(__fadd_rn(__fdiv_rn(sum, (float)H), nx.eps)));
+      const float rms = h2f_(f2h_(rms_f));
+      if (on) {
+        const uint16_t *e = reinterpret_cast<const uint16_t *>(&xa);
+        const uint16_t *we = reinterpret_cast<const uint16_t *>(&wv8);
+        uint16_t o8[8];
+#pragma unroll
+        for (int q = 0; q < 8; ++q) {
+          float y = h2f_(f2h_(__fmul_rn(h2f_(e[q]), rms)));
+          o8[q] = f2h_(__fmul_rn(y, h2f_(we[q])));
+        }
+        uint16_t *dst = nx.out_packed ? nx.h + act_packed_off(t, ch * 8, H) : nx.h + (size_t)t * H + ch * 8;
+        *reinterpret_cast<uint4 *>(dst) = *reinterpret_cast<uint4 *>(o8);
+      }
+    }
+  }
+}
+
+template <int TPB, int NV, int G>
+__global__ __launch_bounds__(TPB) void softmax_topk_reg_kernel(
+    const uint16_t *__restrict__ logits, int V, int k, int32_t *__restrict__ ids,
+    float *__restrict__ probs, double *__restrict__ part, unsigned *__restrict__ cnt,
+    int32_t *__restrict__ ids2) {
+  softmax_topk_reg_body<TPB, NV, G, false>(logits, V, k, ids, probs, part, cnt, ids2, TopkNext{});
+}
+
+template <int NV, int G>
+__global__ __launch_bounds__(1024) void softmax_topk_next_kernel(
+    const uint16_t *__restrict__ logits, int V, int k, int32_t *__restrict__ ids,
+    float *__restrict__ probs, double *__restrict__ part, unsigned *__restrict__ cnt,
+    int32_t *__restrict__ ids2, TopkNext nx) {
+  softmax_topk_reg_body<1024, NV, G, true>(logits, V, k, ids, probs, part, cnt, ids2, nx);
 }
 
 template <int TPB>
@@ -580,10 +684,47 @@
   return T <= 0 ? 0 : kSplitPartOff + (size_t)std::min(T, kSplitRows) * 16 * 8;
 }
 
+static int topk_tpb() {
+  static const int tpb = [] {
+    const char *e = getenv("FFMI_TOPK_TPB");
+    const int v = e ? atoi(e) : 1024;
+    return v == 256 || v == 512 ? v : 1024;
+  }();
+  return tpb;
+}
+static bool topk_reg_form(const uint16_t *logits, int V, int tpb) {
+  const int nv = (V / 8 + tpb - 1) / tpb;
+  return V % 8 == 0 && ((uintptr_t)logits & 15) == 0 && nv * tpb <= 4096;
+}
+
+bool argmax_can_fold(const uint16_t *logits, int T, int V, const ArgmaxNext &nx) {
+  if (T <= 0 || topk_tpb() != 1024 || !topk_reg_form(logits, V, 1024)) return false;
+  if (!nx.blob || nx.tok_off < 0 || nx.tok_off % 8 || nx.T <= 0 || nx.T > kArgmaxNextMaxT)
+    return false;
+  if (!nx.embed || !nx.w || !nx.res || !nx.h) return false;
+  if (nx.H <= 0 || nx.H % 8 || nx.H > 1024 || (nx.out_packed && nx.H % 32)) return false;
+  if (((uintptr_t)nx.embed | (uintptr_t)nx.w | (uintptr_t)nx.res | (uintptr_t)nx.h) & 15)
+    return false;
+  if (nx.blob_dst && (nx.blob_bytes > (size_t)1 << 30 || (uintptr_t)nx.blob % 16 ||
+                      (uintptr_t)nx.blob_dst % 16))
+    return false;
+  return true;
+}
+
 hipError_t launch_argmax(const uint16_t *logits, int T, int V, int k, int32_t *ids,
-                         float *probs, hipStream_t s, void *ws, size_t ws_bytes, int32_t *ids2) {
-  if (T <= 0) return hipSuccess;
+                         float *probs, hipStream_t s, void *ws, size_t ws_bytes, int32_t *ids2,
+                         const ArgmaxNext *next) {
+  if (T <= 0) return next ? hipErrorInvalidValue : hipSuccess;
   if (k < 1 || k > 4) return hipErrorInvalidValue;
+  if (next && !argmax_can_fold(logits, T, V, *next)) return hipErrorInvalidValue;
+  TopkNext nx{};
+  if (next) {
+    nx.blob = next->blob, nx.embed = next->embed, nx.w = next->w, nx.res = next->res;
+    nx.h = next->h, nx.blob_dst = reinterpret_cast<uint4 *>(next->blob_dst);
+    nx.T = next->T, nx.tok_off = next->tok_off, nx.H = next->H;
+    nx.out_packed = next->out_packed ? 1 : 0, nx.eps = next->eps;
+    nx.blob_n16 = next->blob_dst ? (int)((next->blob_bytes + 15) / 16) : 0;
+  }
   static const int split_env = getenv("FFMI_TOPK_SPLIT") ? atoi(getenv("FFMI_TOPK_SPLIT")) : -1;
   static const bool split2 = getenv("FFMI_TOPK_SPLIT2") && atoi(getenv("FFMI_TOPK_SPLIT2"));
   int G = T <= 32 ? 8 : T <= 64 ? 4 : T <= 128 ? 2 : (T <= kSplitRows && split2) ? 2 : 1;
@@ -591,19 +732,24 @@
   if (!ws || ws_bytes < argmax_workspace_bytes(T) || T > kSplitRows) G = 1;
   unsigned *cnt = reinterpret_cast<unsigned *>(ws);
   double *part = ws ? reinterpret_cast<double *>(static_cast<char *>(ws) + kSplitPartOff) : nullptr;
-  static const int tpb = [] {
-    const char *e = getenv("FFMI_TOPK_TPB");
-    const int v = e ? atoi(e) : 1024;
-    return v == 256 || v == 512 ? v : 1024;
-  }();
+  const int tpb = topk_tpb();
   const int nv = (V / 8 + tpb - 1) / tpb;
-  if (V % 8 == 0 && ((uintptr_t)logits & 15) == 0 && nv * tpb <= 4096) {
+  if (topk_reg_form(logits, V, tpb)) {
 #define FFMI_SMR(TPB, NV)                                                                  \
   hipLaunchKernelGGL((softmax_topk_reg_kernel<TPB, NV, 1>), dim3(T), dim3(TPB), 0, s, logits, V, \
                      k, ids, probs, nullptr, nullptr, ids2)
-#define FFMI_SMG(NV, GG)                                                                     \
-  hipLaunchKernelGGL((softmax_topk_reg_kernel<1024, NV, GG>), dim3(GG, T), dim3(1024), 0, s, \
-                     logits, V, k, ids, probs, part, cnt, ids2)
+#define FFMI_SMG(NV, GG)                                                                         \
+  do {                                                                                           \
+    if (next)                                                                                    \
+      hipLaunchKernelGGL((softmax_topk_next_kernel<NV, GG>), dim3(GG, T), dim3(1024), 0, s,      \
+                         logits, V, k, ids, probs, part, cnt, ids2, nx);                         \
+    else                                                                                         \
+      hipLaunchKernelGGL((softmax_topk_reg_kernel<1024, NV, GG>), dim3(GG, T), dim3(1024), 0, s, \
+                         logits, V, k, ids, probs, part, cnt, ids2);                             \
+  } while (0)
+#define FFMI_SMN(NV)                                                                        \
+  hipLaunchKernelGGL((softmax_topk_next_kernel<NV, 1>), dim3(T), dim3(1024), 0, s, logits, V, \
+                     k, ids, probs, nullptr, nullptr, ids2, nx)
     const int gmax = 4 * std::max(1, nv);
     while (G > 1 && (G > gmax || (G & (G - 1)))) G >>= 1;
     if (tpb == 1024 && G > 1) {
@@ -628,6 +774,10 @@
       if (nv <= 2) FFMI_SMR(512, 2);
       else if (nv <= 4) FFMI_SMR(512, 4);
       else FFMI_SMR(512, 8);
+    } else if (next) {
+      if (nv <= 1) FFMI_SMN(1);
+      else if (nv <= 2) FFMI_SMN(2);
+      else FFMI_SMN(4);
     } else {
       if (nv <= 1) FFMI_SMR(1024, 1);
       else if (nv <= 2) FFMI_SMR(1024, 2);
@@ -635,6 +785,7 @@
     }
 #undef FFMI_SMR
 #undef FFMI_SMG
+#undef FFMI_SMN
   } else {
     hipLaunchKernelGGL(softmax_topk_kernel<1024>, dim3(T), dim3(1024), 0, s, logits, V, k, ids, probs,
                        ids2);
diff --git a/flexflow_amd/csrc/runtime/llama_gpu.cpp b/flexflow_amd/csrc/runtime/llama_gpu.cpp
--- a/flexflow_amd/csrc/runtime/llama_gpu.cpp
+++ b/flexflow_amd/csrc/runtime/llama_gpu.cpp
@@ -68,6 +68,7 @@
   std::vector<int> slot_map[kChain];
   hipEvent_t slot_ev[kChain] = {};
   hipEvent_t chain_t0 = nullptr;
+  hipEvent_t chain_t1 = nullptr;
   bool slot_ev_live[kChain] = {};
   int last_slot = -1;
   bool chain_ok = !getenv("FFMI_SSM_CHAIN") || atoi(getenv("FFMI_SSM_CHAIN")) != 0;
@@ -350,11 +351,15 @@
               c.hidden, kv.first, kv.second.n, kv.second.launch / kv.second.n, kv.second.gpu / kv.second.n,
               kv.second.wait / kv.second.n, kv.second.total / kv.second.n);
     }
+    if (step_timing && grouped_slots)
+      fprintf(stderr, "[ffmi step timing] H=%d grouped chain slots: %ld launched, %ld with the "
+              "gather norm folded into the previous top-k\n", c.hidden, grouped_slots, folded_slots);
     for (auto e : st_ev)
       if (e) (void)hipEventDestroy(e);
     for (auto e : slot_ev)
       if (e) (void)hipEventDestroy(e);
     if (chain_t0) (void)hipEventDestroy(chain_t0);
+    if (chain_t1) (void)hipEventDestroy(chain_t1);
     clear_graphs();
     for (auto &L : layers) ffmi_attn_destroy(L.attn);
     for (auto e : ev_pool) (void)hipEventDestroy(e);
@@ -710,19 +715,40 @@
   struct GraphKey {
     int T, W, C, k, parity, overlap, fused, max_q, slot;
     size_t bytes;
+    int fold = 0;
     bool operator<(const GraphKey &o) const {
-      return std::tie(T, W, C, k, parity, overlap, fused, max_q, slot, bytes) <
-             std::tie(o.T, o.W, o.C, o.k, o.parity, o.overlap, o.fused, o.max_q, o.slot, o.bytes);
+      return std::tie(T, W, C, k, parity, overlap, fused, max_q, slot, bytes, fold) <
+             std::tie(o.T, o.W, o.C, o.k, o.parity, o.overlap, o.fused, o.max_q, o.slot, o.bytes,
+                      o.fold);
     }
   };
   int tree_parity = 0;
   std::map<GraphKey, hipGraphExec_t> graphs;
   int chain_group = getenv("FFMI_CHAIN_GROUP") ? atoi(getenv("FFMI_CHAIN_GROUP")) : kChain - 2;
+  bool fold_gather = !getenv("FFMI_SSM_FOLD_GATHER") || atoi(getenv("FFMI_SSM_FOLD_GATHER")) != 0;
+  long grouped_slots = 0, folded_slots = 0;
   struct PendingSlot {
     int slot, T, k;
     size_t bytes;
     GraphKey key;
+    int tok_off;
   };
+  ffmi::ArgmaxNext next_block(const PendingSlot &nx) const {
+    ffmi::ArgmaxNext a;
+    a.blob = chain_batch[nx.slot]->host;
+    a.tok_off = nx.tok_off;
+    a.T = nx.T;
+    a.embed = embed, a.w = layers[0].in_norm, a.res = res, a.h = h;
+    a.H = c.hidden, a.eps = c.rms_eps, a.out_packed = packed;
+    a.blob_dst = chain_batch[nx.slot]->dev, a.blob_bytes = nx.bytes;
+    return a;
+  }
+  bool can_fold_gather(const PendingSlot &q, const PendingSlot &nx) const {
+    return fold_gather && blob_fetch && mode == FFMI_MODEL_BEAM && o.tp_size == 1 &&
+           Vl == c.vocab_size && !dbg && prof_level == 0 && nx.slot == q.slot + 1 && topk_ws &&
+           topk_ws_bytes >= ffmi::argmax_workspace_bytes(q.T) &&
+           ffmi::argmax_can_fold(logits, q.T, c.vocab_size, next_block(nx));
+  }
   std::vector<PendingSlot> pend;
   std::map<std::vector<GraphKey>, hipGraphExec_t> group_graphs;
   bool use_graphs = getenv("FFMI_NO_GRAPHS") == nullptr;
@@ -824,11 +850,15 @@
                     GraphKey{T, batch->num_work, batch->num_commits, k, tree_parity,
                              batch->commit_overlap ? 1 : 0,
                              (batch->one_item_per_req ? 1 : 0) | (batch->lds_tail ? 2 : 0),
-                             batch->max_q, slot, bytes}});
+                             batch->max_q, slot, bytes},
+                    reinterpret_cast<const ffmi::BatchHeader *>(batch->host)->off_tokens});
     return FFMI_OK;
   }
   ffmi_status flush_pending() {
     if (pend.empty()) return FFMI_OK;
+    for (size_t i = 0; i < pend.size(); ++i) pend[i].key.fold = 0;
+    for (size_t i = 0; i + 1 < pend.size(); ++i)
+      if (can_fold_gather(pend[i], pend[i + 1])) pend[i].key.fold |= 2, pend[i + 1].key.fold |= 1;
     std::vector<GraphKey> keys;
     for (const auto &q : pend) keys.push_back(q.key);
     auto it = group_graphs.find(keys);
@@ -837,10 +867,14 @@
       hipGraph_t g = nullptr;
       ffmi_status st = FFMI_OK;
       FFMI_HIP(hipStreamBeginCapture(stream, hipStreamCaptureModeThreadLocal));
-      for (const auto &q : pend) {
+      for (size_t i = 0; i < pend.size(); ++i) {
+        const PendingSlot &q = pend[i];
         cur_slot = q.slot;
         batch = chain_batch[q.slot];
-        st = enqueue(q.k, q.bytes, false, q.T);
+        ffmi::ArgmaxNext nb;
+        if (q.key.fold & 2) nb = next_block(pend[i + 1]);
+        st = enqueue(q.k, q.bytes, false, q.T, (q.key.fold & 1) != 0,
+                     (q.key.fold & 2) ? &nb : nullptr);
         if (st != FFMI_OK) break;
       }
       cur_slot = 0;
@@ -859,6 +893,7 @@
       FFMI_HIP(ie);
       it = group_graphs.emplace(keys, ex).first;
     }
+    for (const auto &k : keys) grouped_slots++, folded_slots += k.fold & 1;
     pend.clear();
     FFMI_HIP(hipGraphLaunch(it->second, stream));
     inflight = true;
@@ -897,7 +932,8 @@
     group_graphs.clear();
   }
 
-  ffmi_status enqueue(int k, size_t blob_bytes, bool record_upload, int T) {
+  ffmi_status enqueue(int k, size_t blob_bytes, bool record_upload, int T,
+                      bool gather_done = false, const ffmi::ArgmaxNext *next = nullptr) {
     const int H = c.hidden, V = c.vocab_size;
     const float eps = c.rms_eps;
     const ffmi_stream s = (ffmi_stream)stream;
@@ -937,7 +973,8 @@
         fz_qkv.wnorm = L.in_norm, fz_gu.wnorm = L.post_norm;
         fz_qkv.eps = fz_gu.eps = eps;
       }
-      if (!fz_in && !(arn && l > 0)) {
+      if (!fz_in && !(arn && l > 0) &&
+          !(l == 0 && gather_done)) {
         pr = prof_begin(on);
         FFMI_HIP(ffmi::launch_rmsnorm(l == 0 ? embed : res, l == 0 ? nullptr : proj, L.in_norm, res,
                                       h, T, H, eps, stream, packed,
@@ -1069,14 +1106,14 @@
     prof_end(pr, GEMM_LM_HEAD, gemm_bytes(T, Vl, Vl, H), 2.0 * T * Vl * H);
     mkt();
     pr = prof_begin(ptail);
-    TRY(enqueue_sampling(k, T));
+    TRY(enqueue_sampling(k, T, next));
     prof_end(pr, SAMPLING, (double)T * V * 2, 0);
     mkt();
 #undef TRY
     return FFMI_OK;
   }
 
-  ffmi_status enqueue_sampling(int k, int T) {
+  ffmi_status enqueue_sampling(int k, int T, const ffmi::ArgmaxNext *next = nullptr) {
     const int V = c.vocab_size;
     const ffmi_stream s = (ffmi_stream)stream;
     ffmi_status st;
@@ -1084,6 +1121,7 @@
   do { if ((st = (x)) != FFMI_OK) return st; } while (0)
     int32_t *ids_o = result_copy ? ids_d : ids_h + cur_slot * slot_ints();
     float *probs_o = reinterpret_cast<float *>(ids_o + (size_t)T * k);
+    FFMI_CHECK(!next || (Vl == V && mode == FFMI_MODEL_BEAM), FFMI_ERR_INVALID);
     if (Vl != V) {
       TRY(ffmi_vocab_shard_topk(o.comm, logits, T, Vl, k, ids_o, probs_o, xch, s));
     } else {
@@ -1091,7 +1129,8 @@
       FFMI_HIP(ffmi::launch_argmax(logits, T, V, k, ids_o, probs_o, stream, topk_ws, topk_ws_bytes,
                                    mode == FFMI_MODEL_BEAM
                                        ? ids_dev + (size_t)cur_slot * (slot_ints() / 2)
-                                       : nullptr));
+                                       : nullptr,
+                                   next));
     }
     if (result_copy)
       FFMI_HIP(hipMemcpyAsync(ids_h + cur_slot * slot_ints(), ids_d, (size_t)T * k * 8,
@@ -1183,6 +1222,7 @@
         getenv("FFMI_CHAIN_EVENTS") ? atoi(getenv("FFMI_CHAIN_EVENTS")) : 2;
     const bool record = slot_events == 1 || (slot_events == 2 && slot == kChain - 2);
     if (st == FFMI_OK) last_slot = slot;
+    if (st == FFMI_OK) FFMI_HIP(mark_chain_end());
     if (st == FFMI_OK && record) {
       if (!slot_ev[slot])
         FFMI_HIP(hipEventCreateWithFlags(&slot_ev[slot], step_timing ? 0 : hipEventDisableTiming));
@@ -1192,11 +1232,21 @@
     }
     return st;
   }
+  hipError_t mark_chain_end() {
+    if (!step_timing) return hipSuccess;
+    if (!chain_t1) {
+      const hipError_t e = hipEventCreate(&chain_t1);
+      if (e != hipSuccess) return e;
+    }
+    return hipEventRecord(chain_t1, stream);
+  }
   ffmi_status beam_collect_chained(int slot, BeamInferenceResult *ir) override {
     FFMI_CHECK(slot >= 0 && slot < kChain, FFMI_ERR_INVALID);
     {
+      const bool staged = !pend.empty();
       ffmi_status st = flush_pending();
       if (st != FFMI_OK) return st;
+      if (staged) FFMI_HIP(mark_chain_end());
     }
     int ev = -1;
     for (int e = slot; e < last_slot && ev < 0; ++e)
@@ -1208,9 +1258,9 @@
       ffmi_status st = forward_finish();
       if (st != FFMI_OK) return st;
       for (bool &b : slot_ev_live) b = false;
-      if (step_timing && ls > 0 && chain_t0) {
+      if (step_timing && ls > 0 && chain_t0 && chain_t1) {
         float ms = 0;
-        if (hipEventElapsedTime(&ms, chain_t0, slot_ev[ls]) == hipSuccess) {
+        if (hipEventElapsedTime(&ms, chain_t0, chain_t1) == hipSuccess) {
           StepTime &q = st_sum[-(ls + 1)];
           q.n++;
           q.gpu += ms * 1e3;
diff --git a/flexflow_amd/ffmi.py b/flexflow_amd/ffmi.py
--- a/flexflow_amd/ffmi.py
+++ b/flexflow_amd/ffmi.py
@@ -203,6 +203,11 @@
                                                  c_int, c_int, c_void_p]),
     "ffmi_debug_fused_norm_linear": (c_int, [c_void_p, c_void_p, c_void_p, c_float, c_void_p,
                                              c_void_p, c_int, c_int, c_int, c_int, c_void_p]),
+    "ffmi_debug_topk_gather_norm": (c_int, [c_void_p, c_int, c_int, c_int, c_void_p, c_void_p,
+                                            c_void_p, c_void_p, c_size_t, c_void_p,
+                                            ctypes.POINTER(BatchDesc), c_void_p, c_void_p,
+                                            c_void_p, c_void_p, c_int, c_float, c_int, c_void_p,
+                                            ctypes.POINTER(c_size_t), c_int, c_void_p]),
     "ffmi_debug_attn_stamps": (ctypes.c_long, [c_void_p, ctypes.c_long]),
     "ffmi_debug_markers": (ctypes.c_long, [c_void_p, ctypes.c_long]),
 }
@@ -239,6 +244,8 @@
                               "`python -c 'import __graft_entry__ as g; g.build()'`")
         L = ctypes.CDLL(LIB_PATH, mode=ctypes.RTLD_GLOBAL)
         for name, (res, args) in SIGNATURES.items():
+            if _VARIANT and name.startswith("ffmi_debug_") and not hasattr(L, name):
+                continue
             fn = getattr(L, name)
             fn.restype = res
             fn.argtypes = args
diff --git a/include/ffmi.h b/include/ffmi.h
--- a/include/ffmi.h
+++ b/include/ffmi.h
@@ -313,6 +313,14 @@
                                          void *Y, int T, int out_dim, int in_dim, int epilogue,
                                          ffmi_stream stream);
 
+ffmi_status ffmi_debug_topk_gather_norm(const void *logits, int T, int V, int k, int32_t *ids,
+                                        float *probs, int32_t *ids_dev, void *workspace,
+                                        size_t workspace_bytes, ffmi_batch_dev *b,
+                                        const ffmi_batch_desc *next, const void *table,
+                                        const void *norm_w, void *res, void *h, int H, float eps,
+                                        int flags, void *blob_dst, size_t *blob_bytes, int fold,
+                                        ffmi_stream stream);
+
 long ffmi_debug_gemm_stamps(long long *dst, long max_waves);
 ffmi_status ffmi_debug_gemm_plan(int T, int out_dim, int in_dim, int epilogue, int *plan );
 long ffmi_debug_attn_stamps(long long *dst, long max_waves);
```

Measured after the change: 1370 tokens/s (median of 6 runs). Within noise of the previous version (+0.2%).
